# nbip/IWAE

Hardware: AMD Instinct MI355X
Metric: images/sec (train step) IWAE k=50 batch 1024 @1/2/4/8 GPU; test LLH@k=5000 (higher is better)
Workload: dtype bf16; 1 GPU; 1-layer IWAE k=50 batch 1024 per GPU (BASELINE configs[1]; N=8 is configs[4]), objective iwae_elbo, train step = forward + backward + Adam(eps=1e-4); config_id=c1, global_batch=1024, n_samples=50, parallelism=dp1, rccl_ranks=0, settle_steps=100, full=False

## Files before the change

### iwae_amd/csrc/device_helpers.h

```cpp
#pragma once
#include <hip/hip_runtime.h>
#include <stdint.h>
#include "kernels.h"
#include "layout.h"

namespace iwae {

typedef __attribute__((ext_vector_type(8))) __bf16 bf16x8_t;
typedef __attribute__((ext_vector_type(2))) __bf16 bf16x2_t;
typedef __attribute__((ext_vector_type(4))) float f32x4;

#define LOG2PI_F 1.8378770664093453f
#define HALF_LOG_2PI_F 0.9189385332046727f

__device__ __forceinline__ uint32_t pack2(float a, float b) {
    bf16x2_t v;
    v[0] = (__bf16)a;
    v[1] = (__bf16)b;
    return __builtin_bit_cast(uint32_t, v);
}
__device__ __forceinline__ float bflo(uint32_t u) { return __uint_as_float(u << 16); }
__device__ __forceinline__ float bfhi(uint32_t u) { return __uint_as_float(u & 0xffff0000u); }
__device__ __forceinline__ float bf_at(const uint4& u, int j) {
    const uint32_t w = (j < 2) ? u.x : (j < 4) ? u.y : (j < 6) ? u.z : u.w;
    return (j & 1) ? bfhi(w) : bflo(w);
}
__device__ __forceinline__ f32x4 mfma16(const uint4& a, const uint4& b, f32x4 c) {
    return __builtin_amdgcn_mfma_f32_16x16x32_bf16(__builtin_bit_cast(bf16x8_t, a), __builtin_bit_cast(bf16x8_t, b), c, 0, 0, 0);
}
__device__ __forceinline__ float rcp_fast(float x) { return __builtin_amdgcn_rcpf(x); }
#define LOG2E_F 1.4426950408889634f
#define LN2_F 0.6931471805599453f
__device__ __forceinline__ float exp2_raw(float x) { return __builtin_amdgcn_exp2f(x); }
__device__ __forceinline__ float log2_raw(float x) { return __builtin_amdgcn_logf(x); }
__device__ __forceinline__ float tanh_fast(float x) {
    return 1.0f - 2.0f * rcp_fast(exp2_raw(x * (2.0f * LOG2E_F)) + 1.0f);
}
__device__ __forceinline__ float sigmoid_fast(float l) { return rcp_fast(1.0f + exp2_raw(-l * LOG2E_F)); }
__device__ __forceinline__ float tanh_f32(float x) {
    const float t = __expf(2.0f * fabsf(x));
    return __builtin_copysignf(1.0f - 2.0f * __builtin_amdgcn_rcpf(t + 1.0f), x);
}

__device__ __forceinline__ uint32_t lds_addr_of(const char* p) {
    return (uint32_t)(uintptr_t)(const __attribute__((address_space(3))) char*)p;
}
__device__ __forceinline__ void glds16(const char* g, uint32_t lds_wave_base) {
    uint32_t keep;
    asm volatile("s_mov_b32 %0, m0\n\ts_mov_b32 m0, %2\n\ts_nop 0\n\tglobal_load_lds_dwordx4 %1, off\n\ts_mov_b32 m0, %0"
                 : "=&s"(keep) : "v"(g), "s"(lds_wave_base) : "memory");
}

template <int NWAVES>
__device__ __forceinline__ void stage_image(const char* src, char* lds, int bytes, int wave, int lane) {
    const uint32_t base = lds_addr_of(lds);
    for (int off = wave * 1024; off < bytes; off += NWAVES * 1024)
        glds16(src + off + lane * 16, (uint32_t)__builtin_amdgcn_readfirstlane((int)(base + (uint32_t)off)));
}

__device__ __forceinline__ void wait_all_vmem() {
    __builtin_amdgcn_s_waitcnt(0x0F70);
    asm volatile("s_waitcnt vmcnt(0)" ::: "memory");
}

template <int N, int P, class RD, class USE, class SIDE>
__device__ __forceinline__ void lds_pipeline(RD rd, USE use, SIDE side) {
    uint4 av[P];
#pragma unroll
    for (int i = 0; i < P; ++i)
        if (i < N) av[i] = rd(i);
#pragma unroll
    for (int i = 0; i < N; ++i) {
        use(i, av[i % P]);
        if (i + P < N) av[i % P] = rd(i + P);
        side(i);
    }
}
template <int N, int P, class RD, class USE>
__device__ __forceinline__ void lds_pipeline(RD rd, USE use) {
    lds_pipeline<N, P>(rd, use, [](int) {});
}

__device__ __forceinline__ void philox4x32_10(uint32_t c0, uint32_t c1, uint32_t c2, uint32_t c3, uint32_t k0, uint32_t k1, uint32_t out[4]) {
#pragma unroll
    for (int r = 0; r < 10; ++r) {
        unsigned long long p0, p1;
        asm("v_mad_u64_u32 %0, vcc, %1, %2, 0" : "=v"(p0) : "v"(c0), "v"(0xD2511F53u) : "vcc");
        asm("v_mad_u64_u32 %0, vcc, %1, %2, 0" : "=v"(p1) : "v"(c2), "v"(0xCD9E8D57u) : "vcc");
        const uint32_t hi0 = (uint32_t)(p0 >> 32), lo0 = (uint32_t)p0;
        const uint32_t hi1 = (uint32_t)(p1 >> 32), lo1 = (uint32_t)p1;
        const uint32_t n0 = hi1 ^ c1 ^ k0, n1 = lo1, n2 = hi0 ^ c3 ^ k1, n3 = lo0;
        c0 = n0; c1 = n1; c2 = n2; c3 = n3;
        k0 += 0x9E3779B9u; k1 += 0xBB67AE85u;
    }
    out[0] = c0; out[1] = c1; out[2] = c2; out[3] = c3;
}
__device__ __forceinline__ void philox4x32_10_mul(uint32_t c0, uint32_t c1, uint32_t c2, uint32_t c3, uint32_t k0, uint32_t k1, uint32_t out[4]) {
#pragma unroll
    for (int r = 0; r < 10; ++r) {
        const unsigned long long p0 = (unsigned long long)c0 * 0xD2511F53ull, p1 = (unsigned long long)c2 * 0xCD9E8D57ull;
        const uint32_t hi0 = (uint32_t)(p0 >> 32), lo0 = (uint32_t)p0, hi1 = (uint32_t)(p1 >> 32), lo1 = (uint32_t)p1;
        const uint32_t n0 = hi1 ^ c1 ^ k0, n2 = hi0 ^ c3 ^ k1;
        c0 = n0; c1 = lo1; c2 = n2; c3 = lo0;
        k0 += 0x9E3779B9u; k1 += 0xBB67AE85u;
    }
    out[0] = c0; out[1] = c1; out[2] = c2; out[3] = c3;
}
__device__ __forceinline__ void box_muller4(const uint32_t (&r)[4], float n[4]) {
    const float s24 = 5.9604644775390625e-08f;
    const float u0 = ((float)(r[0] >> 8) + 0.5f) * s24, u1 = ((float)(r[1] >> 8) + 0.5f) * s24;
    const float u2 = ((float)(r[2] >> 8) + 0.5f) * s24, u3 = ((float)(r[3] >> 8) + 0.5f) * s24;
    const float ra = __builtin_amdgcn_sqrtf(-2.0f * __logf(u0)), rb = __builtin_amdgcn_sqrtf(-2.0f * __logf(u2));
    n[0] = ra * __builtin_amdgcn_cosf(u1); n[1] = ra * __builtin_amdgcn_sinf(u1);
    n[2] = rb * __builtin_amdgcn_cosf(u3); n[3] = rb * __builtin_amdgcn_sinf(u3);
}
__device__ __forceinline__ void normal4(uint64_t grow, uint32_t d4, uint32_t stream, uint32_t step, uint64_t seed, float n[4]) {
    uint32_t r[4];
    philox4x32_10((uint32_t)grow, (uint32_t)(grow >> 32), (stream << 24) | d4, step, (uint32_t)seed, (uint32_t)(seed >> 32), r);
    box_muller4(r, n);
}
__device__ __forceinline__ void normal4_mul(uint64_t grow, uint32_t d4, uint32_t stream, uint32_t step, uint64_t seed, float n[4]) {
    uint32_t r[4];
    philox4x32_10_mul((uint32_t)grow, (uint32_t)(grow >> 32), (stream << 24) | d4, step, (uint32_t)seed, (uint32_t)(seed >> 32), r);
    box_muller4(r, n);
}

__device__ __forceinline__ float rowsum16(float v) {
    v += __shfl_xor(v, 1); v += __shfl_xor(v, 2); v += __shfl_xor(v, 4); v += __shfl_xor(v, 8);
    return v;
}
__device__ __forceinline__ double rowsum16(double v) {
    v += __shfl_xor(v, 1); v += __shfl_xor(v, 2); v += __shfl_xor(v, 4); v += __shfl_xor(v, 8);
    return v;
}
__device__ __forceinline__ double tree_sum_256(double v, double* sh) {
    sh[threadIdx.x] = v;
    __syncthreads();
#pragma unroll
    for (int w = 256 / 2; w > 0; w >>= 1) {
        if ((int)threadIdx.x < w) sh[threadIdx.x] += sh[threadIdx.x + w];
        __syncthreads();
    }
    const double r = sh[0];
    __syncthreads();
    return r;
}

constexpr int WG_GEMM_THREADS = 256;

__device__ __forceinline__ void wg_gemm_f32(const float* strip, int pa, int nkb, const float* W, int ldw, int cnt, float* slab,
                                            f32x4 (&acc)[AIS_NT], int tid, int n16, int q) {
    const int gpr = 4 * cnt;
    int goff[4], soff[4];
    bool ok[4];
    float4 pre[4];
#pragma unroll
    for (int u = 0; u < 4; ++u) {
        const int g = tid + WG_GEMM_THREADS * u, r = g / gpr, cq = g - r * gpr;
        ok[u] = r < 16;
        goff[u] = r * ldw + 4 * cq;
        soff[u] = r * AIS_SLABP + 4 * cq;
        pre[u] = make_float4(0.f, 0.f, 0.f, 0.f);
        if (ok[u]) pre[u] = *(const float4*)(W + goff[u]);
    }
    for (int kb = 0; kb < nkb; ++kb) {
        __syncthreads();
#pragma unroll
        for (int u = 0; u < 4; ++u)
            if (ok[u]) *(float4*)(slab + soff[u]) = pre[u];
        __syncthreads();
        if (kb + 1 < nkb) {
#pragma unroll
            for (int u = 0; u < 4; ++u)
                if (ok[u]) pre[u] = *(const float4*)(W + (size_t)(kb + 1) * 16 * ldw + goff[u]);
        }
        const float4 av = *(const float4*)(strip + n16 * pa + 16 * kb + 4 * q);
        const float a4[4] = {av.x, av.y, av.z, av.w};
        const float* sl = slab + 4 * q * AIS_SLABP + n16;
#pragma unroll
        for (int j = 0; j < 4; ++j)
#pragma unroll
            for (int t = 0; t < AIS_NT; ++t)
                if (t < cnt) acc[t] = __builtin_amdgcn_mfma_f32_16x16x4f32(a4[j], sl[j * AIS_SLABP + 16 * t], acc[t], 0, 0, 0);
    }
}

template <class Args>
__device__ __forceinline__ void dec_row_tanh_layers(const Args& a, const float* zs, float* g1s, float* g2s, float* slab, int PZ, int PH, int dt, int ht,
                                                    f32x4 (&acc)[AIS_NT], int tid, int n16, int q) {
#pragma unroll
    for (int t = 0; t < AIS_NT; ++t) acc[t] = (f32x4){0.f, 0.f, 0.f, 0.f};
    wg_gemm_f32(zs, PZ, dt, a.W1, a.Hp, ht, slab, acc, tid, n16, q);
#pragma unroll
    for (int t = 0; t < AIS_NT; ++t) {
        if (t < ht) {
            const float b = a.b1[16 * t + n16];
#pragma unroll
            for (int r = 0; r < 4; ++r) g1s[(4 * q + r) * PH + 16 * t + n16] = tanh_f32(acc[t][r] + b);
            acc[t] = (f32x4){0.f, 0.f, 0.f, 0.f};
        }
    }
    wg_gemm_f32(g1s, PH, ht, a.W2, a.Hp, ht, slab, acc, tid, n16, q);
#pragma unroll
    for (int t = 0; t < AIS_NT; ++t) {
        if (t < ht) {
            const float b = a.b2[16 * t + n16];
#pragma unroll
            for (int r = 0; r < 4; ++r) g2s[(4 * q + r) * PH + 16 * t + n16] = tanh_f32(acc[t][r] + b);
        }
    }
}

template <class Args>
__device__ __forceinline__ void dec_row_eval(const Args& a, float* zs, float* g1s, float* g2s, float* slab, int PZ, int PH, int dt, int ht, int xt,
                                             int npass, const float* const (&xrow)[4], f32x4 (&acc)[AIS_NT], float (&lp)[4], int tid, int n16, int q) {
    f32x4 dg2[AIS_NT];
    dec_row_tanh_layers(a, zs, g1s, g2s, slab, PZ, PH, dt, ht, acc, tid, n16, q);
#pragma unroll
    for (int t = 0; t < AIS_NT; ++t) dg2[t] = (f32x4){0.f, 0.f, 0.f, 0.f};
    for (int pass = 0; pass < npass; ++pass) {
        const int c0 = 16 * AIS_TPO * pass, cnt = min(AIS_TPO, xt - AIS_TPO * pass);
#pragma unroll
        for (int t = 0; t < AIS_TPO; ++t) acc[t] = (f32x4){0.f, 0.f, 0.f, 0.f};
        wg_gemm_f32(g2s, PH, ht, a.W3 + c0, a.Xp, cnt, slab, acc, tid, n16, q);
        float s_xl[4] = {0.f, 0.f, 0.f, 0.f}, s_al[4] = {0.f, 0.f, 0.f, 0.f}, prod[4] = {1.f, 1.f, 1.f, 1.f};
#pragma unroll
        for (int t = 0; t < AIS_TPO; ++t) {
            if (t < cnt) {
                const int col = c0 + 16 * t + n16;
                const bool in = col < a.X;
                const float b = a.b3[col];
#pragma unroll
                for (int r = 0; r < 4; ++r) {
// ... 44 lines not shown
```

### iwae_amd/csrc/fp32_kernels.hip

```cpp
#include <hip/hip_runtime.h>
#include <stdint.h>
#include <type_traits>
#include <algorithm>
#include "kernels.h"
#include "device_helpers.h"

namespace iwae {

__device__ __forceinline__ float4 scale_b_quad(const GemmF32Args& a, float4 t, int gk, bool b_nfast) {
    if (b_nfast) { const float w = a.brow_scale[gk]; return make_float4(t.x * w, t.y * w, t.z * w, t.w * w); }
    return make_float4(t.x * a.brow_scale[gk], t.y * a.brow_scale[gk + 1], t.z * a.brow_scale[gk + 2], t.w * a.brow_scale[gk + 3]);
}

template <int KB>
__global__ __launch_bounds__(256) void gemm_f32_kernel(GemmF32Args a) {
    constexpr int BK = 16 * KB;
    __shared__ float sA[64][BK + 1];
    __shared__ float sB[BK][80];
    const int tid = threadIdx.x, lane = tid & 63, wave = tid >> 6;
    const int m0 = blockIdx.y * 64, n0 = blockIdx.x * 64;
    const int k_beg = blockIdx.z * a.kchunk, k_end = min(a.K, k_beg + a.kchunk);
    const int wm = wave >> 1, wn = wave & 1;
    const int r16 = lane & 15, q = lane >> 4;
    f32x4 acc[2][2];
// ... 148 lines not shown
        const float* p = a.B + (size_t)gk * a.sbk + (size_t)gn * a.sbn;
        const int lim = b_nfast ? a.N - gn : k_end - gk;
        const bool outer_ok = b_nfast ? gk < k_end : gn < a.N;
        if (outer_ok && lim >= 4 && a.bvec) { float4 t = *(const float4*)p; if (a.brow_scale) t = scale_b_quad(a, t, gk, b_nfast); return t; }
        if (outer_ok) {
#pragma unroll
            for (int e = 0; e < 4; ++e) if (e < lim) v[e] = p[e * (b_nfast ? a.sbn : a.sbk)] * (a.brow_scale ? a.brow_scale[b_nfast ? gk : gk + e] : 1.0f);
        }
        return make_float4(v[0], v[1], v[2], v[3]);
    };
    auto stash = [&](int buf, const float4 (&ra)[NA], const float4 (&rb)[NB]) {
#pragma unroll
        for (int u = 0; u < NA; ++u) {
            int lm, lk;
            if (!a_pos(u, lm, lk)) continue;
            const float av4[4] = {ra[u].x, ra[u].y, ra[u].z, ra[u].w};
#pragma unroll
            for (int e = 0; e < 4; ++e) { if (a_kfast) sA[buf][lm][lk + e] = av4[e]; else sA[buf][lm + e][lk] = av4[e]; }
        }
#pragma unroll
        for (int u = 0; u < NB; ++u) {
            int ln, lk;
            if (!b_pos(u, ln, lk)) continue;
            const float bv4[4] = {rb[u].x, rb[u].y, rb[u].z, rb[u].w};
#pragma unroll
            for (int e = 0; e < 4; ++e) { if (b_nfast) sB[buf][lk][ln + e] = bv4[e]; else sB[buf][lk + e][ln] = bv4[e]; }
        }
    };
    float4 ra[NA], rb[NB];
#pragma unroll
    for (int u = 0; u < NA; ++u) ra[u] = make_float4(0.f, 0.f, 0.f, 0.f);
#pragma unroll
    for (int u = 0; u < NB; ++u) rb[u] = make_float4(0.f, 0.f, 0.f, 0.f);
    if (k_beg < k_end) {
#pragma unroll
        for (int u = 0; u < NA; ++u) ra[u] = fetch_a(k_beg, u);
#pragma unroll
        for (int u = 0; u < NB; ++u) rb[u] = fetch_b(k_beg, u);
    }
    stash(0, ra, rb);
    __syncthreads();
    int buf = 0;
    for (int k0 = k_beg; k0 < k_end; k0 += 16) {
        const bool more = k0 + 16 < k_end;
        if (more) {
#pragma unroll
            for (int u = 0; u < NA; ++u) ra[u] = fetch_a(k0 + 16, u);
#pragma unroll
            for (int u = 0; u < NB; ++u) rb[u] = fetch_b(k0 + 16, u);
        }
#pragma unroll
        for (int kk = 0; kk < 4; ++kk) {
            float av[TM], bv[TN];
#pragma unroll
            for (int i = 0; i < TM; ++i) av[i] = sA[buf][16 * TM * wm + 16 * i + r16][4 * kk + q];
#pragma unroll
            for (int j = 0; j < TN; ++j) bv[j] = sB[buf][4 * kk + q][16 * TN * wn + 16 * j + r16];
#pragma unroll
            for (int i = 0; i < TM; ++i)
#pragma unroll
                for (int j = 0; j < TN; ++j) acc[i][j] = __builtin_amdgcn_mfma_f32_16x16x4f32(av[i], bv[j], acc[i][j], 0, 0, 0);
        }
        if (more) stash(buf ^ 1, ra, rb);
        __syncthreads();
        buf ^= 1;
    }
    if constexpr (TM == 4 && TN == 4) {
    if (a.epi == GEMM_EPI_BERN) {
        float bias4[4];
        bool nok[4];
#pragma unroll
        for (int j = 0; j < 4; ++j) {
            const int n = n0 + 64 * wn + 16 * j + r16;
            nok[j] = n < a.N;
            bias4[j] = (nok[j] && a.bias) ? a.bias[n] : 0.0f;
        }
#pragma unroll
        for (int i = 0; i < 4; ++i)
#pragma unroll
            for (int r = 0; r < 4; ++r) {
                const int m = m0 + 64 * wm + 16 * i + 4 * q + r;
                const int mc = min(m, a.M - 1);
                const float* xr = a.XB + (size_t)(mc / a.bern_k) * a.bern_X;
                float sum = 0.0f;
#pragma unroll
                for (int j = 0; j < 4; ++j) {
                    if (nok[j]) {
                        const float l = acc[i][j][r] + bias4[j];
                        const float xv = xr[n0 + 64 * wn + 16 * j + r16];
                        const float e = __expf(-fabsf(l)), ope = 1.0f + e;
                        sum += xv * l - (fmaxf(l, 0.0f) + __logf(ope));
                        if (a.C && m < a.M) a.C[(size_t)m * a.ldc + n0 + 64 * wn + 16 * j + r16] = xv - (l >= 0.0f ? 1.0f : e) * __builtin_amdgcn_rcpf(ope);
                    }
                }
                sum += __shfl_xor(sum, 1); sum += __shfl_xor(sum, 2); sum += __shfl_xor(sum, 4); sum += __shfl_xor(sum, 8);
                if (r16 == 0 && m < a.M) a.part[(size_t)(2 * blockIdx.x + wn) * a.part_stride + m] = sum;
            }
        return;
    }
    }
    float* C = a.C + (size_t)blockIdx.z * a.slab_stride;
#pragma unroll
    for (int i = 0; i < TM; ++i)
#pragma unroll
        for (int j = 0; j < TN; ++j) {
            const int n = n0 + 16 * TN * wn + 16 * j + r16;
            if (n >= a.N) continue;
            const float bias = a.bias ? a.bias[n] : 0.0f;
#pragma unroll
            for (int r = 0; r < 4; ++r) {
                const int m = m0 + 16 * TM * wm + 16 * i + 4 * q + r;
                if (m >= a.M) {
                    if (a.Cones && m == a.M) a.Cones[(size_t)blockIdx.z * a.cones_stride + n] = acc[i][j][r];
                    continue;
                }
                float v = acc[i][j][r] + bias;
                if (a.orow_scale) v *= a.orow_scale[m];
                if (a.epi == GEMM_EPI_TANH) v = tanh_f32(v);
                else if (a.epi == GEMM_EPI_EXP) v = expf(v) + 1e-6f;
                else if (a.epi == GEMM_EPI_DTANH) { const float y = a.ACT[(size_t)m * a.ldact + n]; v *= 1.0f - y * y; }
                float* dst = C + (size_t)m * a.ldc + n;
                *dst = a.accumulate ? *dst + v : v;
            }
        }
}

#ifdef IWAE_DENSE_STAMPS
#define GS_STAMP(slot)                                                                 \
    {                                                                                  \
        unsigned long long t_;                                                         \
        __builtin_amdgcn_sched_barrier(0);                                             \
        asm volatile("s_memtime %0\n\ts_waitcnt lgkmcnt(0)" : "=s"(t_)::"memory");     \
        __builtin_amdgcn_sched_barrier(0);                                             \
        gs_sum[slot] += t_ - gs_prev;                                                  \
        gs_prev = t_;                                                                  \
    }
#else
#define GS_STAMP(slot)
#endif
__device__ __forceinline__ int gemm_swz16(int row) { return (0x78 >> (2 * ((row >> 2) & 3))) & 3; }
__device__ __forceinline__ float4 gemm_f32_slow_quad(const float* base, long s_e, long s_k, int e, int k, int Ext, int k_end, bool kfast, bool ones) {
    float v[4];
#pragma unroll
    for (int t = 0; t < 4; ++t) {
        const int ee = kfast ? e : e + t, kk = kfast ? k + t : k;
        float x = 0.0f;
        if (kk < k_end) {
            if (ee < Ext) x = base[(size_t)ee * s_e + (size_t)kk * s_k];
            else if (ones && ee == Ext) x = 1.0f;
        }
        v[t] = x;
    }
    return make_float4(v[0], v[1], v[2], v[3]);
}
__device__ __forceinline__ void quad_transpose(float (&x)[4], int lane) {
    const int p = lane & 3;
    float t[4];
#pragma unroll
    for (int r = 0; r < 4; ++r) {
        const float o = __builtin_bit_cast(float, __builtin_amdgcn_mov_dpp(__builtin_bit_cast(int, x[r ^ 1]), 0xB1, 0xF, 0xF, true));
        t[r] = ((r ^ p) & 1) ? o : x[r];
    }
#pragma unroll
    for (int r = 0; r < 4; ++r) {
        const float o = __builtin_bit_cast(float, __builtin_amdgcn_mov_dpp(__builtin_bit_cast(int, t[r ^ 2]), 0x4E, 0xF, 0xF, true));
        x[r] = ((r ^ p) & 2) ? o : t[r];
    }
}
template <int TM, int TN, int WGM, int WGN, bool AK, bool BNF, int OCC = 4>
__global__ __launch_bounds__(64 * WGM * WGN, OCC) void gemm_f32_v2_kernel(GemmF32Args a) {
    constexpr int NT = 64 * WGM * WGN;
    [[maybe_unused]] constexpr int NW = WGM * WGN;
    constexpr int BM = 16 * TM * WGM, BN = 16 * TN * WGN;
    constexpr int PA = AK ? 16 : BM + 4, PB = BNF ? BN + 4 : 16;
    constexpr int SA = AK ? BM * 16 : 16 * PA, SB = BNF ? 16 * PB : BN * 16;
    constexpr int QM = BM / 4, QN = BN / 4;
    constexpr bool HOLD_A = TM <= TN;
    __shared__ __attribute__((aligned(16))) float sA[2][SA];
    __shared__ __attribute__((aligned(16))) float sB[2][SB];
    const int tid = threadIdx.x, lane = tid & 63, wave = tid >> 6;
#ifdef IWAE_DENSE_STAMPS
    unsigned long long gs_sum[8] = {0, 0, 0, 0, 0, 0, 0, 0}, gs_prev = 0;
    asm volatile("s_memtime %0\n\ts_waitcnt lgkmcnt(0)" : "=s"(gs_prev)::"memory");
#endif
    int bx = blockIdx.x, by = blockIdx.y, bz = blockIdx.z;
    {
        const int nb = gridDim.x * gridDim.y * gridDim.z;
        if (gridDim.z > 1 && (nb & 7) == 0) {
            const int L = bx + gridDim.x * (by + gridDim.y * bz), V = (L & 7) * (nb >> 3) + (L >> 3);
            bx = V % gridDim.x; by = (V / gridDim.x) % gridDim.y; bz = V / (gridDim.x * gridDim.y);
        }
    }
    const int m0 = by * BM, n0 = bx * BN;
    const int k_beg = bz * a.kchunk, k_end = min(a.K, k_beg + a.kchunk);
    const int wm = wave / WGN, wn = wave % WGN;
    const int r16 = lane & 15, q = lane >> 4;
    f32x4 acc[TM][TN];
#pragma unroll
    for (int i = 0; i < TM; ++i)
#pragma unroll
        for (int j = 0; j < TN; ++j) acc[i][j] = (f32x4){0.f, 0.f, 0.f, 0.f};
    constexpr int TPRA = QM > 32 ? 64 : QM > 16 ? 32 : 16, TPRB = QN > 32 ? 64 : QN > 16 ? 32 : 16;
    constexpr int RQ = NT / 4, KRA = NT / TPRA, KRB = NT / TPRB;
    constexpr int NA = AK ? (BM + RQ - 1) / RQ : (16 + KRA - 1) / KRA, NB = BNF ? (16 + KRB - 1) / KRB : (BN + RQ - 1) / RQ;
    const bool ones = a.Cones != nullptr;
    const int eA0 = AK ? tid >> 2 : 4 * (tid % TPRA), kA0 = AK ? 4 * (tid & 3) : tid / TPRA;
    const int eB0 = BNF ? 4 * (tid % TPRB) : tid >> 2, kB0 = BNF ? tid / TPRB : 4 * (tid & 3);
    constexpr int dEA = AK ? RQ : 0, dKA = AK ? 0 : KRA, dEB = BNF ? 0 : RQ, dKB = BNF ? KRB : 0;
    const int oA0 = AK ? eA0 * 16 + (((tid & 3) ^ gemm_swz16(eA0)) << 2) : kA0 * PA + eA0;
    const int oB0 = BNF ? kB0 * PB + eB0 : eB0 * 16 + (((tid & 3) ^ gemm_swz16(eB0)) << 2);
    constexpr int dOA = AK ? RQ * 16 : dKA * PA, dOB = BNF ? dKB * PB : RQ * 16;
    const float* pA = a.A + (size_t)(m0 + eA0) * a.sam + (size_t)(k_beg + kA0) * a.sak;
    const float* pB = a.B + (size_t)(n0 + eB0) * a.sbn + (size_t)(k_beg + kB0) * a.sbk;
    const long dPA = AK ? RQ * a.sam : (long)dKA * a.sak, dPB = BNF ? (long)dKB * a.sbk : RQ * a.sbn;
    unsigned stA = 0, stB = 0;
#pragma unroll
    for (int u = 0; u < NA; ++u) {
        const int le = eA0 + dEA * u, ge = m0 + le;
        const bool exists = AK ? le < BM : le < BM && kA0 + dKA * u < 16;
        const bool inside = AK ? ge < a.M : ge + 3 < a.M, outside = ge >= a.M + (ones ? 1 : 0);
        stA |= (unsigned)(!exists ? 3 : (inside && a.avec) ? 1 : outside ? 0 : 2) << (2 * u);
    }
#pragma unroll
    for (int u = 0; u < NB; ++u) {
        const int le = eB0 + dEB * u, ge = n0 + le;
        const bool exists = BNF ? le < BN && kB0 + dKB * u < 16 : le < BN;
        const bool inside = BNF ? ge + 3 < a.N : ge < a.N, outside = ge >= a.N;
        stB |= (unsigned)(!exists ? 3 : (inside && a.bvec) ? 1 : outside ? 0 : 2) << (2 * u);
    }
    const long stepA = 16 * a.sak, stepB = 16 * a.sbk;
    float4 ra[NA], rb[NB], rw[NB];
    auto fetch = [&](int k0, bool full) {
#pragma unroll
        for (int u = 0; u < NA; ++u) {
            const unsigned st = (stA >> (2 * u)) & 3u;
            float4 t = make_float4(0.f, 0.f, 0.f, 0.f);
            if (st == 1 && full) t = *(const float4*)(pA + u * dPA);
            else if (st == 2 || (st == 1 && !full)) t = gemm_f32_slow_quad(a.A, a.sam, a.sak, m0 + eA0 + dEA * u, k0 + kA0 + dKA * u, a.M, k_end, AK, ones);
            ra[u] = t;
        }
        pA += stepA;
#pragma unroll
        for (int u = 0; u < NB; ++u) {
            const unsigned st = (stB >> (2 * u)) & 3u;
            float4 t = make_float4(0.f, 0.f, 0.f, 0.f);
            if (st == 1 && full) t = *(const float4*)(pB + u * dPB);
            else if (st == 2 || (st == 1 && !full)) t = gemm_f32_slow_quad(a.B, a.sbn, a.sbk, n0 + eB0 + dEB * u, k0 + kB0 + dKB * u, a.N, k_end, !BNF, false);
            rb[u] = t;
            if (a.brow_scale && st != 3) {
                const int gk = k0 + kB0 + dKB * u;
                if (BNF) { const float w = gk < k_end ? a.brow_scale[gk] : 0.0f; rw[u] = make_float4(w, w, w, w); }
                else rw[u] = make_float4(gk < k_end ? a.brow_scale[gk] : 0.0f, gk + 1 < k_end ? a.brow_scale[gk + 1] : 0.0f,
                                         gk + 2 < k_end ? a.brow_scale[gk + 2] : 0.0f, gk + 3 < k_end ? a.brow_scale[gk + 3] : 0.0f);
            }
        }
        pB += stepB;
    };
    auto stash = [&](int buf) {
#pragma unroll
        for (int u = 0; u < NA; ++u) if (((stA >> (2 * u)) & 3u) != 3u) *(float4*)&sA[buf][oA0 + dOA * u] = ra[u];
#pragma unroll
        for (int u = 0; u < NB; ++u)
            if (((stB >> (2 * u)) & 3u) != 3u) {
                float4 t = rb[u];
                if (a.brow_scale) { t.x *= rw[u].x; t.y *= rw[u].y; t.z *= rw[u].z; t.w *= rw[u].w; }
                *(float4*)&sB[buf][oB0 + dOB * u] = t;
            }
    };
    const int arow = 16 * TM * wm + r16, brow = 16 * TN * wn + r16;
    const int afr = AK ? arow * 16 + ((q ^ gemm_swz16(r16)) << 2) : 4 * q * PA + arow;
    const int bfr = BNF ? 4 * q * PB + brow : brow * 16 + ((q ^ gemm_swz16(r16)) << 2);
    auto frag_a = [&](const float* As, int t, float (&v)[4]) {
        if (AK) { const float4 x = *(const float4*)(As + afr + 256 * t); v[0] = x.x; v[1] = x.y; v[2] = x.z; v[3] = x.w; }
        else {
#pragma unroll
            for (int j = 0; j < 4; ++j) v[j] = As[afr + 16 * t + j * PA];
        }
    };
    auto frag_b = [&](const float* Bs, int t, float (&v)[4]) {
        if (BNF) {
#pragma unroll
            for (int j = 0; j < 4; ++j) v[j] = Bs[bfr + 16 * t + j * PB];
        } else { const float4 x = *(const float4*)(Bs + bfr + 256 * t); v[0] = x.x; v[1] = x.y; v[2] = x.z; v[3] = x.w; }
    };
    auto compute = [&](int buf) {
        const float *As = sA[buf], *Bs = sB[buf];
        if constexpr (HOLD_A) {
            float ah[TM][4];
#pragma unroll
            for (int i = 0; i < TM; ++i) frag_a(As, i, ah[i]);
            constexpr int NG = (TN + 1) / 2;
            float cur[2][4], nxt[2][4];
            frag_b(Bs, 0, cur[0]);
            if (TN > 1) frag_b(Bs, 1, cur[1]);
#pragma unroll
            for (int g = 0; g < NG; ++g) {
                if (g + 1 < NG) { frag_b(Bs, 2 * g + 2, nxt[0]); if (2 * g + 3 < TN) frag_b(Bs, 2 * g + 3, nxt[1]); }
#pragma unroll
                for (int j = 0; j < 4; ++j)
#pragma unroll
                    for (int h = 0; h < 2; ++h)
                        if (2 * g + h < TN) {
#pragma unroll
                            for (int i = 0; i < TM; ++i) acc[i][2 * g + h] = __builtin_amdgcn_mfma_f32_16x16x4f32(ah[i][j], cur[h][j], acc[i][2 * g + h], 0, 0, 0);
                        }
#pragma unroll
                for (int h = 0; h < 2; ++h)
#pragma unroll
                    for (int j = 0; j < 4; ++j) cur[h][j] = nxt[h][j];
            }
        } else {
            float bh[TN][4];
#pragma unroll
            for (int j = 0; j < TN; ++j) frag_b(Bs, j, bh[j]);
            constexpr int NG = (TM + 1) / 2;
            float cur[2][4], nxt[2][4];
            frag_a(As, 0, cur[0]);
            if (TM > 1) frag_a(As, 1, cur[1]);
#pragma unroll
            for (int g = 0; g < NG; ++g) {
// ... 652 lines not shown
```

### iwae_amd/csrc/kernels.h

```cpp
#pragma once
#include <hip/hip_runtime.h>
#include <stdint.h>

namespace iwae {

#define IWAE_DENSE_G1_DEFAULT 29u
enum { EPI_TANH = 0, EPI_HEAD = 1, EPI_DX = 2, EPI_F32 = 3, EPI_BERN = 4, EPI_SIGMOID = 5 };
enum { OBJ_VAE_ELBO = 0, OBJ_IWAE_ELBO = 1, OBJ_IWAE_EQ14 = 2, OBJ_VAE_ELBO_KL = 3, OBJ_DREG = 4 };
enum { PB_LME = 0, PB_MEAN, PB_EQ14, PB_KL, PB_PX, PB_T1, PB_T2, PB_DREG, PB_COUNT };
enum { SC_VAE_ELBO = 0, SC_VAE_ELBO_KL, SC_IWAE_ELBO, SC_IWAE_EQ14, SC_INFERENCE_LOSS, SC_MEAN_LPXZ, SC_MEAN_T1, SC_MEAN_T2, SC_KL, SC_COUNT = 16 };


struct EpsSrc {
    const float* user = nullptr;
    const float* cache = nullptr;
    int ldC = 0;
    int B = 0;
    uint64_t seed = 0;
    uint64_t row_offset = 0;
    uint32_t step = 0;
    uint32_t stream = 0;
    int k_total = 0, s_off = 0, kc = 0;
};

// ... 82 lines not shown
    const float* Xf; int Xdim; uint16_t* XPout;
    const char *img0, *img1, *img2;
    int KT0, KT1;
    int NT1, NT2;
    int R;
    uint16_t *H1, *H2; int ldH;
    float* YF; int ldYF; int split;
    int sample; SampleArgs S;
    const char* oimg; int oXdim, oH;
    const uint16_t* oXB; int oldXB; int ok;
    uint16_t* oSP; int oldS; float* olpxz;
};
bool block_fwd_ok(const BlockFwdArgs& a);
bool block_fwd_shape_ok(const BlockFwdArgs& a);
void launch_block_fwd(const BlockFwdArgs& a, hipStream_t st);

struct Chain2FwdArgs {
    uint16_t* Z1P;
    float* lqz1x;
    const char *e_img1, *e_img2, *e_imgh;
    const char *d_img1, *d_img2, *d_imgh;
    int M, k, B, D0, D1;
    uint16_t *EH1, *EH2;
    float* EHEAD;
    uint16_t* Z2P;
    uint16_t *DH1, *DH2;
    float* DHEAD;
    const float* head1; int ldH1;
    EpsSrc eps1, eps2;
    float *lpz1z2, *lpz2, *lqz2z1;
};
bool chain2_fwd_ok(int KT0, int KTH, int KT1, int M);
void launch_chain2_fwd(const Chain2FwdArgs& a, hipStream_t st);

struct DecBwdRowsArgs {
    const uint16_t* SP; int ldS; int KTX;
    const char* imgK3; int MT3;
    const char *imgB2, *imgB1;
    int KT, NT1, NT3;
    int M;
    const uint16_t *G2, *G1; int ldH;
    const float* gx;
    uint16_t *D2P, *D1P;
    float* DZ; uint16_t* DZH; int ldDZ;
    int lse_on;
    LseArgs lse;
};
bool dec_bwd_rows_ok(const DecBwdRowsArgs& a);
void launch_dec_bwd_rows(const DecBwdRowsArgs& a, hipStream_t st, hipEvent_t done = nullptr);

struct LatentBwdArgs {
    const float* dz; int ldDZ;
    const uint16_t* dzh;
    const float* dz2; const float* dz3;
    const float* head; int ldH; int D, Dp;
    const float4* cf;
    EpsSrc eps;
    int B, Bp, k;
    float kmu, ksig;
    uint16_t* DHP;
    float* DHF;
    const float* prior_head;
    uint16_t* DHP2;
    float* DHF2;
};
void launch_latent_bwd(const LatentBwdArgs& a, hipStream_t st);
struct BlockBwdArgs {
    const uint16_t* DH; int ldDH;
    const char *imgH, *imgL2;
    int KTH, KT1, NT1;
    int R;
    const uint16_t *H2, *H1; int ldH;
    uint16_t *D2, *D1;
    int lat_on;
    LatentBwdArgs lat;
    int rows_per_wg;
};
bool block_bwd_ok(const BlockBwdArgs& a);
void launch_block_bwd(const BlockBwdArgs& a, hipStream_t st);

struct OutBwdArgs {
    const uint16_t* G2; int ldG;
    const char* img1;
    const char* img2;
    int Xdim; int Xp32;
    const float* gx;
    const uint16_t* XB; int ldXB; int k;
    int M, KT, NG;
    uint16_t* DLP;
    const uint16_t* SP;
    float* part; int gpb;
    uint16_t* DPP;
    unsigned long long* stamps;
    int dbg;
};
void launch_out_bwd(const OutBwdArgs& a, hipStream_t st, hipEvent_t done = nullptr);

struct DecBwdArgs {
    OutBwdArgs o;
    const char* imgB2;
    const uint16_t* G1;
    uint16_t* D1P;
    const char* imgB1; int MG1;
    float* DZ; int ldDZ;
    uint16_t* DZH;
    int nw;
};
bool out_bwd_has_s_mode(int KT);
void launch_dec_bwd(const DecBwdArgs& d, hipStream_t st, hipEvent_t done = nullptr);

struct GBlockBwdArgs {
    const char* imgH;
    const char *imgBh, *imgB2, *imgB1;
    const uint16_t *H2, *H1;
    const float* gx;
    int M, k, B, D;
    EpsSrc eps;
    const float* head1; int ldH1;
    const float* DZIN;
    uint16_t* DHP;
    uint16_t *D2P, *D1P;
    float* DZ2;
    uint16_t* DZD;
    const float* DZDEC;
    int ldDZDEC;
    uint16_t* DZOUT;
};
bool gblock_bwd_ok(int KT0, int KTH, int KT1, int M);
void launch_gblock_bwd(int mode, const GBlockBwdArgs& a, hipStream_t st, hipEvent_t done = nullptr);

struct GaussBwdArgs {
    int mode;
    const float* G;
    const float* head; int ldH; int D, Dp;
    const float* zhead; int ldZH; int Dzp;
    const float* dz_in; float* dz_direct; int ldDZ;
    EpsSrc eps;
    int M, Mp, k;
    uint16_t* DHP;
    float* DHF;
};
void launch_gauss_bwd(const GaussBwdArgs& a, hipStream_t st);

struct WgradPArgs {
    const uint16_t* X; int ldX; int IT;
    const uint16_t* G; int ldG; int JT;
    int M, rows_per_split;
    float* slabW;
    float* slabB;
    const char* zero;
    const float* rowscale;
    int dbg;
    unsigned long long* stamps;
};
void launch_wgradp(const WgradPArgs& a, int nsplit, int shape, hipStream_t st, hipEvent_t done = nullptr);
int wgradp_strip(int shape);
struct WgradPGroup {
    WgradPArgs a[3];
    int n;
    int gx[3], gy[3];
    int zbeg[4];
};
void launch_wgradp_group(const WgradPGroup& g, hipStream_t st);
void launch_wgradws_group(const WgradPGroup& g, hipStream_t st);

struct LayerDesc {
    int Kin, Nout, joff;
    size_t offW, offb;
    char* imgF; int KT_F;
    char* imgB; int KT_B; int MT_B; int imgB_kmajor;
    const float* slabW; const float* slabB; int nsplit; int slab_ld; size_t slab_stride;
    size_t slabB_stride;
    int block_begin;
    int rblock_begin;
};
void launch_reduce_grads(const LayerDesc* layers, int nlayers, int first_block, int nblocks, float* grad, float* param, float* mom, float* vel,
                         float alpha, float beta1, float beta2, float eps, int fuse_adam, const float* per_b, int B, float beta, float* scalars, hipStream_t st,
                         int first_block2 = 0, int nblocks2 = 0, hipEvent_t done = nullptr);
void launch_scalars(const float* per_b, int B, float beta, float* out, hipStream_t st);
void launch_adam(const LayerDesc* layers, int nlayers, int nblocks, float* param, const float* grad, float* mom, float* vel,
                 float alpha, float gscale, float beta1, float beta2, float eps, int do_update, hipStream_t st, int first_block = 0, hipEvent_t done = nullptr);

#define WGR_MAX_JOBS 6
struct WgradRowsJob {
    const uint16_t* X; int ldX;
    const uint16_t* G; int ldG;
    int R;
    const float* rowscale;
    int sub0, sub1, split;
    int ib, jb, wg_begin;
};
void launch_wgrad_rows(const WgradRowsJob* jobs, int njobs, const LayerDesc* layers, float* grad, float* param, float* mom, float* vel, float alpha,
                       float beta1, float beta2, float eps, int fuse_adam, const float* per_b, int B, float beta, float* scalars, const char* zero, hipStream_t st);

enum { GEMM_EPI_NONE = 0, GEMM_EPI_TANH = 1, GEMM_EPI_EXP = 2, GEMM_EPI_DTANH = 3, GEMM_EPI_BERN = 4 };
struct GemmF32Args {
    const float* A; long sam, sak;
    const float* B; long sbk, sbn;
    float* C; long ldc;
    int M, N, K;
    const float* bias;
    int epi;
    const float* ACT; long ldact;
    int accumulate;
    int kchunk; size_t slab_stride;
    int avec, bvec;
    int cvec;
    const float* XB; int bern_k, bern_X;
    float* part; size_t part_stride;
    const float* brow_scale;
    const float* orow_scale;
    float* Cones; size_t cones_stride;
    unsigned long long* stamps;
    int tile_mode;
    int dbg;
};
struct DecFwdF32Args {
    const float* Z; int ldz; int Din;
    int M, H, X;
    const float *W1, *b1, *W2, *b2, *W3, *b3;
    float *G1, *G2; int ldg;
    float* S; int ldS;
    const float* XB; int k;
    float* lpxz;
    const char* zero;
    unsigned long long* stamps;
};
bool dec_fwd_f32_ok(const DecFwdF32Args& a);
void launch_dec_fwd_f32(const DecFwdF32Args& a, hipStream_t st);
struct GemmF32Opts {
    bool v2 = true;
    bool w8 = true;
    bool v2_small = true;
    bool ksplit = true;
    int ksplit_min_tiles = 1;
    int v2_small_min = 1;
    int dbg = 0;
};
long gemm_f32_tiles(const GemmF32Opts& o, int M, int N, int tile_mode = 0);
bool gemm_f32_takes_big(int M, int N, int nsplit);
void launch_gemm_f32(const GemmF32Opts& o, const GemmF32Args& a, int nsplit, hipStream_t st);
int gemm_f32_fewrows_split(const GemmF32Opts& o, int M, int N, int K);
void launch_gemm_f32_fewrows(const GemmF32Opts& o, const GemmF32Args& a, float* slabs, hipStream_t st);
int gemm_f32_slots(const GemmF32Opts& o, int M, int N, int tile_mode = 0);
void launch_reduce_slabs_f32(const float* slabs, size_t stride, int nsplit, size_t n, float* out, hipStream_t st);
#define REDUCE_SLABS_MAX_JOBS 40
struct ReduceSlabsJob { const float* slabs; size_t stride; size_t n; float* out; int nsplit; int block_begin; };
struct ReduceSlabsJobs { ReduceSlabsJob job[REDUCE_SLABS_MAX_JOBS]; int n; };
void launch_reduce_slabs_multi_f32(ReduceSlabsJobs& jobs, hipStream_t st);
void launch_bern_f32(const float* logits, size_t ld, const float* x, int X, int M, int k, float* lpxz, hipStream_t st);
void launch_dl_f32(float* logits, size_t ld, const float* x, int X, int M, int k, const float* gx, hipStream_t st);
void launch_sigmoid_f32(float* v, size_t n, hipStream_t st);
void launch_export_mat(const float* in, int B, int k, int X, float* out, hipStream_t st);
void launch_concat_f32(const float* a, int na, const float* b, int nb, int rows, float* out, hipStream_t st);

#define GRID_D_MAX 4
#define GRID_XP_MAX 800
#define GRID_RANGE 1024
enum { GRID_ST = 18, GRID_S1 = 2, GRID_S2 = 6, GRID_Q = 16, GRID_A = 17 };
__host__ __device__ inline int grid_tri(int d, int e) { return d * GRID_D_MAX - d * (d - 1) / 2 + (e - d); }
struct GridPrepArgs {
    const float* logits; int ldl;
    const float* z; const float* lw;
    int Gc, Gcp, X, Xp, D;
    uint16_t *Lhi, *Llo;
    float* c; float4* zc; float* w;
};
struct GridScoreArgs {
    const uint16_t* XB; int Xp;
    const uint16_t *Lhi, *Llo; const float* c; const float4* zc; const float* w;
    const float* head; int ldh, soff;
    int N, Gc, nsplit;
    float* part;
    float* log_joint; long ldlj; long lj_col;
};
struct GridMergeArgs {
    const float* part; int nsplit, N, D;
    double* run;
    int first, last;
    const float* head; int ldh;
    double* log_px; float *mean, *cov, *qmass, *kl;
};
void launch_grid_prep_x(const float* x, int N, int X, int Np, int Xp, uint16_t* XB, int* nonbinary, hipStream_t st);
void launch_grid_prep(const GridPrepArgs& a, hipStream_t st);
void launch_grid_score(const GridScoreArgs& a, int D, hipStream_t st);
void launch_grid_merge(const GridMergeArgs& a, hipStream_t st);

#define ACT_BLOCK 128
struct ActChainArgs {
    const char *img1, *img2, *imgh;
    const float* head1; int ldH1;
    EpsSrc eps1;
    int kn, D0, D1;
    float* part; int nblk;
    int img0, blk0;
};
struct ActPartialArgs {
    const float* head; int ldh;
    int nb, kn, D1;
    float* part; int nblk, img0, blk0;
};
struct ActStatsArgs {
    const float* src; long ld_img; int ld_blk, nblk;
    double kdiv;
    int N, D;
    float* post_mean; int ldpm, col;
    double *activity, *data_mean;
// ... 208 lines not shown
```

### iwae_amd/csrc/kernels.hip

```cpp
#include <hip/hip_runtime.h>
#include <hip/hip_ext.h>
#include <stdint.h>
#include <string.h>
#include <type_traits>
#include "kernels.h"
#include "layout.h"
#include "device_helpers.h"
#include "step_helpers.h"

namespace iwae {
template <bool MASKED, bool KEEP>
__device__ __forceinline__ float bern8(const f32x4& a0, const f32x4& a1, const uint4& xb, int f0, int Xdim, uint4& sp) {
    float s_xl = 0.0f, s_al = 0.0f, prod = 1.0f, sv[8];
#pragma unroll
    for (int j = 0; j < 8; ++j) {
        const float l = (j < 4) ? a0[j & 3] : a1[j & 3];
        const float xm = bf_at(xb, j) - 0.5f;
        const float ope = 1.0f + exp2_raw(-fabsf(l * LOG2E_F));
        const bool in = !MASKED || (f0 + 16 * (j >> 2) + (j & 3) < Xdim);
        prod *= in ? ope : 1.0f;
        s_al += fabsf(l);
        s_xl = fmaf(xm, l, s_xl);
        if (KEEP) {
            const float h = __builtin_copysignf(rcp_fast(ope) - 0.5f, l);
// ... 2589 lines not shown
                        dsg[i] += t * e[u][i] + cf[u].w * rsg[i];
                        dpm[i] -= cf[u].y * up * prs[i];
                        dps[i] -= cf[u].y * (up * up - 1.0f) * prs[i];
                    }
                }
            }
        }
    }
#pragma unroll
    for (int i = 0; i < 4; ++i) { red[threadIdx.x][i] = dmu[i]; red[threadIdx.x][4 + i] = dsg[i]; }
    __syncthreads();
    if (sg == 0 && act) {
        for (int g = 1; g < SG; ++g)
#pragma unroll
            for (int i = 0; i < 4; ++i) { dmu[i] += red[g * nf4 + f4][i]; dsg[i] += red[g * nf4 + f4][4 + i]; }
#pragma unroll
        for (int i = 0; i < 4; ++i) {
            if (f0 + i < a.D) {
                dmu[i] += a.kmu * mu[i];
                dsg[i] += a.ksig * (sgm[i] - 1.0f / sgm[i]);
                dsg[i] *= (sgm[i] - 1e-6f);
            } else { dmu[i] = 0.0f; dsg[i] = 0.0f; }
        }
    }
    if (sg == 0 && b < a.B) {
        if (a.DHP) {
            *(uint2*)(a.DHP + (size_t)b * (2 * a.Dp) + p_pos(f0)) = make_uint2(pack2(dmu[0], dmu[1]), pack2(dmu[2], dmu[3]));
            *(uint2*)(a.DHP + (size_t)b * (2 * a.Dp) + p_pos(a.Dp + f0)) = make_uint2(pack2(dsg[0], dsg[1]), pack2(dsg[2], dsg[3]));
        }
        if (a.DHF) {
            *(float4*)(a.DHF + (size_t)b * (2 * a.Dp) + f0) = make_float4(dmu[0], dmu[1], dmu[2], dmu[3]);
            *(float4*)(a.DHF + (size_t)b * (2 * a.Dp) + a.Dp + f0) = make_float4(dsg[0], dsg[1], dsg[2], dsg[3]);
        }
    }
    if (FAST || !a.prior_head) return;
    __syncthreads();
#pragma unroll
    for (int i = 0; i < 4; ++i) { red[threadIdx.x][i] = dpm[i]; red[threadIdx.x][4 + i] = dps[i]; }
    __syncthreads();
    if (sg != 0 || b >= a.B) return;
    if (act) {
        for (int g = 1; g < SG; ++g)
#pragma unroll
            for (int i = 0; i < 4; ++i) { dpm[i] += red[g * nf4 + f4][i]; dps[i] += red[g * nf4 + f4][4 + i]; }
#pragma unroll
        for (int i = 0; i < 4; ++i) {
            if (f0 + i < a.D) dps[i] *= (sigp_of(a, b, f0 + i) - 1e-6f);
            else { dpm[i] = 0.0f; dps[i] = 0.0f; }
        }
    }
    if (a.DHP2) {
        *(uint2*)(a.DHP2 + (size_t)b * (2 * a.Dp) + p_pos(f0)) = make_uint2(pack2(dpm[0], dpm[1]), pack2(dpm[2], dpm[3]));
        *(uint2*)(a.DHP2 + (size_t)b * (2 * a.Dp) + p_pos(a.Dp + f0)) = make_uint2(pack2(dps[0], dps[1]), pack2(dps[2], dps[3]));
    }
    if (a.DHF2) {
        *(float4*)(a.DHF2 + (size_t)b * (2 * a.Dp) + f0) = make_float4(dpm[0], dpm[1], dpm[2], dpm[3]);
        *(float4*)(a.DHF2 + (size_t)b * (2 * a.Dp) + a.Dp + f0) = make_float4(dps[0], dps[1], dps[2], dps[3]);
    }
}

__global__ void gauss_bwd_kernel(GaussBwdArgs a) {
    const int idx = blockIdx.x * blockDim.x + threadIdx.x;
    const int nf4 = a.Dp / 4;
    const int row = idx / nf4, f4 = idx % nf4;
    if (row >= a.Mp) return;
    const bool valid = row < a.M;
    const int f0 = 4 * f4;
    float dm[4] = {0, 0, 0, 0}, ds[4] = {0, 0, 0, 0}, dzd[4] = {0, 0, 0, 0};
    if (valid && f0 < a.D) {
        const int b = row / a.k, s = row - b * a.k;
        const float G = a.G[row];
        const float* hp = a.head + (size_t)row * a.ldH;
        float e[4];
        eps4(a.eps, b, s, row, f4, a.D, e);
        const float4 mu4 = *(const float4*)(hp + f0), sg4 = *(const float4*)(hp + a.Dp + f0);
        const float muv[4] = {mu4.x, mu4.y, mu4.z, mu4.w}, sgv[4] = {sg4.x, sg4.y, sg4.z, sg4.w};
        float4 a4 = make_float4(0.f, 0.f, 0.f, 0.f), b4 = a4;
        if (a.mode == 0) {
            const float* hz = a.zhead + (size_t)b * a.ldZH;
            a4 = *(const float4*)(hz + f0); b4 = *(const float4*)(hz + a.Dzp + f0);
        } else {
            a4 = *(const float4*)(a.dz_in + (size_t)row * a.ldDZ + f0);
        }
        const float av[4] = {a4.x, a4.y, a4.z, a4.w}, bv[4] = {b4.x, b4.y, b4.z, b4.w};
#pragma unroll
        for (int i = 0; i < 4; ++i) {
            if (f0 + i < a.D) {
                const float mu = muv[i], sg = sgv[i], rs = __builtin_amdgcn_rcpf(sg);
                if (a.mode == 0) {
                    const float z = av[i] + bv[i] * e[i];
                    const float u = (z - mu) * rs;
                    dm[i] = G * u * rs;
                    ds[i] = G * (u * u - 1.0f) * rs * (sg - 1e-6f);
                    dzd[i] = -dm[i];
                } else {
                    const float z = mu + sg * e[i];
                    const float d = av[i] - G * z;
                    dm[i] = d;
                    ds[i] = (d * e[i] + G * rs) * (sg - 1e-6f);
                }
            }
        }
    }
    if (valid) {
        if (a.DHP) {
            *(uint2*)(a.DHP + (size_t)row * (2 * a.Dp) + p_pos(f0)) = make_uint2(pack2(dm[0], dm[1]), pack2(dm[2], dm[3]));
            *(uint2*)(a.DHP + (size_t)row * (2 * a.Dp) + p_pos(a.Dp + f0)) = make_uint2(pack2(ds[0], ds[1]), pack2(ds[2], ds[3]));
        }
        if (a.DHF) {
            *(float4*)(a.DHF + (size_t)row * (2 * a.Dp) + f0) = make_float4(dm[0], dm[1], dm[2], dm[3]);
            *(float4*)(a.DHF + (size_t)row * (2 * a.Dp) + a.Dp + f0) = make_float4(ds[0], ds[1], ds[2], ds[3]);
        }
        if (a.mode == 0) *(float4*)(a.dz_direct + (size_t)row * a.ldDZ + f0) = make_float4(dzd[0], dzd[1], dzd[2], dzd[3]);
    }
}


struct AdamCoef { float alpha, gscale, beta1, beta2, eps; int on; };

__device__ __forceinline__ void adam_math(float& w, float& m, float& v, float g, const AdamCoef& c) {
    g *= c.gscale;
    m = __builtin_fmaf(c.beta1, m, (1.0f - c.beta1) * g);
    v = __builtin_fmaf(c.beta2, v, ((1.0f - c.beta2) * g) * g);
    const float q = (c.alpha * m) / (sqrtf(v) + c.eps);
    w = w - q;
}
__device__ __forceinline__ void image_refresh(const LayerDesc& L, bool is_bias, int i, int j, float w) {
    if (is_bias) {
        *(float*)(L.imgF + img_mg_bias_byte(L.joff + j, L.KT_F)) = w;
    } else {
        const uint16_t h = (uint16_t)(pack2(w, 0.0f) & 0xffffu);
        *(uint16_t*)(L.imgF + img_mg_byte(L.joff + j, i, L.KT_F)) = h;
        if (L.imgB) {
            if (L.imgB_kmajor) *(uint16_t*)(L.imgB + img_k_byte(i, L.joff + j, L.MT_B)) = h;
            else *(uint16_t*)(L.imgB + img_mg_byte(i, L.joff + j, L.KT_B)) = h;
        }
    }
}
__device__ __forceinline__ void adam_element(const LayerDesc& L, bool is_bias, int i, int j, size_t idx, float g, bool update,
                                             float* param, float* mom, float* vel, const AdamCoef& c) {
    float w = param[idx];
    if (update) {
        float m = mom[idx], v = vel[idx];
        adam_math(w, m, v, g, c);
        mom[idx] = m;
        vel[idx] = v;
        param[idx] = w;
    }
    image_refresh(L, is_bias, i, j, w);
}

struct MeansArgs { const float* per_b; int B; float beta; float* out; };

__global__ __launch_bounds__(256) void reduce_grads_kernel(const LayerDesc* layers, int nlayers, float* grad, float* param, float* mom,
                                                           float* vel, AdamCoef c, MeansArgs mn, int first_block, int n1, int first_block2) {
    if (mn.per_b && blockIdx.x == gridDim.x - 1) {
        batch_means_block(mn.per_b, mn.B, mn.beta, mn.out);
        return;
    }
    const int bid = (int)blockIdx.x < n1 ? (int)blockIdx.x + first_block : (int)blockIdx.x - n1 + first_block2;
    __shared__ float4 red[4][64];
    int l = 0;
    while (l + 1 < nlayers && bid >= layers[l + 1].rblock_begin) ++l;
    const LayerDesc L = layers[l];
    const int n4 = (L.Nout + 3) >> 2;
    const int g = (bid - L.rblock_begin) * 64 + (threadIdx.x & 63);
    const int sg = threadIdx.x >> 6;
    const int ngroups = (L.Kin + 1) * n4;
    float4 s = make_float4(0.f, 0.f, 0.f, 0.f);
    int i = 0, j = 0;
    const bool ok = g < ngroups;
    if (ok) {
        i = g / n4;
        j = (g - i * n4) * 4;
        const bool is_b = i == L.Kin;
        const float* p = is_b ? (L.slabB + L.joff + j) : (L.slabW + (size_t)i * L.slab_ld + L.joff + j);
        const size_t stride = is_b ? (L.slabB_stride ? L.slabB_stride : (size_t)L.slab_ld) : L.slab_stride;
        if (L.nsplit <= 16) {
#pragma unroll 4
            for (int sp = sg; sp < L.nsplit; sp += 4) {
                const float4 v = *(const float4*)(p + (size_t)sp * stride);
                s.x += v.x; s.y += v.y; s.z += v.z; s.w += v.w;
            }
        } else
        for (int sp0 = sg; sp0 < L.nsplit; sp0 += 32) {
            float4 v[8];
#pragma unroll
            for (int u = 0; u < 8; ++u) {
                const int sp = sp0 + 4 * u;
                v[u] = *(const float4*)(p + (size_t)(sp < L.nsplit ? sp : sg) * stride);
            }
#pragma unroll
            for (int u = 0; u < 8; ++u)
                if (sp0 + 4 * u < L.nsplit) { s.x += v[u].x; s.y += v[u].y; s.z += v[u].z; s.w += v[u].w; }
        }
    }
    red[sg][threadIdx.x & 63] = s;
    __syncthreads();
    if (sg == 0 && ok) {
        const int t = threadIdx.x;
        float r[4] = {red[0][t].x + red[1][t].x + red[2][t].x + red[3][t].x, red[0][t].y + red[1][t].y + red[2][t].y + red[3][t].y,
                      red[0][t].z + red[1][t].z + red[2][t].z + red[3][t].z, red[0][t].w + red[1][t].w + red[2][t].w + red[3][t].w};
        float* dst = (i == L.Kin) ? (grad + L.offb + j) : (grad + L.offW + (size_t)i * L.Nout + j);
#pragma unroll
        for (int e = 0; e < 4; ++e) {
            if (j + e < L.Nout) {
                dst[e] = r[e];
                if (c.on) adam_element(L, i == L.Kin, i, j + e, (size_t)(dst - grad) + e, r[e], true, param, mom, vel, c);
            }
        }
    }
}

__global__ void adam_kernel(const LayerDesc* layers, int nlayers, float* param, const float* grad, float* mom, float* vel, AdamCoef c, int first_block) {
    const int bid = (int)blockIdx.x + first_block;
    int l = 0;
    while (l + 1 < nlayers && bid >= layers[l + 1].block_begin) ++l;
    const LayerDesc L = layers[l];
    const int e = (bid - L.block_begin) * blockDim.x + threadIdx.x;
    const int nW = L.Kin * L.Nout;
    if (e >= nW + L.Nout) return;
    const bool is_b = e >= nW;
    const size_t idx = is_b ? (L.offb + (e - nW)) : (L.offW + e);
    adam_element(L, is_b, is_b ? 0 : e / L.Nout, is_b ? e - nW : e % L.Nout, idx, c.on ? grad[idx] : 0.0f, c.on != 0, param, mom, vel, c);
}
struct WgradRowsArgs {
    WgradRowsJob job[WGR_MAX_JOBS];
    int njobs;
    const LayerDesc* layers;
    float *grad, *param, *mom, *vel;
    AdamCoef c;
    MeansArgs mn;
    const char* zero;
};
#define WGR_NST 4
#define WGR_STAGE 8192
__global__ __launch_bounds__(256, 1) void wgrad_rows_kernel(WgradRowsArgs a) {
    extern __shared__ __attribute__((aligned(1024))) char smem[];
    typedef __attribute__((ext_vector_type(4))) short v4s;
    if (a.mn.per_b && blockIdx.x == gridDim.x - 1) {
        batch_means_block(a.mn.per_b, a.mn.B, a.mn.beta, a.mn.out);
        return;
    }
    int jn = 0;
#pragma unroll
    for (int t = 1; t < WGR_MAX_JOBS; ++t)
        if (t < a.njobs && (int)blockIdx.x >= a.job[t].wg_begin) jn = t;
    const WgradRowsJob J = a.job[jn];
    const int wl = (int)blockIdx.x - J.wg_begin;
    const int bi = wl / J.jb, bj = wl - bi * J.jb;
    const int tid = threadIdx.x, lane = tid & 63, wave = __builtin_amdgcn_readfirstlane(tid >> 6);
    const int q = lane >> 4, l16 = lane & 15, qp = l16 >> 2, p = l16 & 3;
    const int RW = ((J.R + 3) / 4 + 31) & ~31;
    const int rbeg = wave * RW, rend = min(J.R, rbeg + RW);
    const int nstage = rend > rbeg ? (rend - rbeg + 31) / 32 : 0;
    char* ring = smem + wave * (WGR_NST * WGR_STAGE);
    auto swz = [](int r) { return ((r >> 1) & 1) << 2; };
    const int prl = lane >> 3, psl = lane & 7;
    const char* zsrc = a.zero + lane * 16;
    const char* xsrc[4]; const char* gsrc[4]; int xlim[4], glim[4];
#pragma unroll
    for (int pc = 0; pc < 4; ++pc) {
        const int rl = 8 * pc + prl;
        const int cx = bi * 64 + ((psl ^ swz(rl)) * 8), cg = bj * 64 + ((psl ^ swz(rl)) * 8);
        xsrc[pc] = (const char*)J.X + ((size_t)(rbeg + rl) * J.ldX + cx) * 2;
        gsrc[pc] = (const char*)J.G + ((size_t)(rbeg + rl) * J.ldG + cg) * 2;
        xlim[pc] = cx < J.ldX ? rend - rbeg - rl : -(1 << 30);
        glim[pc] = cg < J.ldG ? rend - rbeg - rl : -(1 << 30);
    }
    const size_t xstride = (size_t)32 * J.ldX * 2, gstride = (size_t)32 * J.ldG * 2;
    auto issue = [&](int c) {
        const uint32_t base = lds_addr_of(ring + (c % WGR_NST) * WGR_STAGE);
#pragma unroll
        for (int pc = 0; pc < 4; ++pc)
            glds16(32 * c < xlim[pc] ? xsrc[pc] + (size_t)c * xstride : zsrc, (uint32_t)__builtin_amdgcn_readfirstlane((int)(base + (uint32_t)pc * 1024u)));
#pragma unroll
        for (int pc = 0; pc < 4; ++pc)
            glds16(32 * c < glim[pc] ? gsrc[pc] + (size_t)c * gstride : zsrc, (uint32_t)__builtin_amdgcn_readfirstlane((int)(base + 4096u + (uint32_t)pc * 1024u)));
    };
    f32x4 acc[4][4], accb[4];
#pragma unroll
    for (int u = 0; u < 4; ++u) {
        accb[u] = (f32x4){0.0f, 0.0f, 0.0f, 0.0f};
#pragma unroll
        for (int t = 0; t < 4; ++t) acc[t][u] = (f32x4){0.0f, 0.0f, 0.0f, 0.0f};
    }
    const uint4 ones = make_uint4(0x3F803F80u, 0x3F803F80u, 0x3F803F80u, 0x3F803F80u);
    const bool do_bias = bi == 0;
    for (int c = 0; c < min(nstage, WGR_NST - 1); ++c) issue(c);
    const int row_off = (4 * q + qp) * 128;
    for (int c = 0; c < nstage; ++c) {
        wait_vmem_but_ws(8 * min(WGR_NST - 2, nstage - 1 - c));
        if (c + WGR_NST - 1 < nstage) issue(c + WGR_NST - 1);
        const char* xb = ring + (c % WGR_NST) * WGR_STAGE + row_off;
        const char* gb = xb + 4096;
        auto frag = [&](const char* base, int t) {
            const char* p0 = base + ((((4 * (t >> 1)) ^ swz(qp)) + p) * 16) + 8 * (t & 1);
            const v4s r0 = __builtin_amdgcn_ds_read_tr16_b64_v4i16((__attribute__((address_space(3))) v4s*)p0);
            const v4s r1 = __builtin_amdgcn_ds_read_tr16_b64_v4i16((__attribute__((address_space(3))) v4s*)(p0 + 16 * 128));
            const uint2 lo = __builtin_bit_cast(uint2, r0), hi = __builtin_bit_cast(uint2, r1);
            return make_uint4(lo.x, lo.y, hi.x, hi.y);
        };
        uint4 g[4];
#pragma unroll
        for (int u = 0; u < 4; ++u) g[u] = frag(gb, u);
        if (J.rowscale) {
            const float* rs = J.rowscale + rbeg + 32 * c + 4 * q;
            const float4 s0 = *(const float4*)rs, s1 = *(const float4*)(rs + 16);
#pragma unroll
            for (int u = 0; u < 4; ++u)
                g[u] = make_uint4(pack2(bflo(g[u].x) * s0.x, bfhi(g[u].x) * s0.y), pack2(bflo(g[u].y) * s0.z, bfhi(g[u].y) * s0.w),
                                  pack2(bflo(g[u].z) * s1.x, bfhi(g[u].z) * s1.y), pack2(bflo(g[u].w) * s1.z, bfhi(g[u].w) * s1.w));
        }
#pragma unroll
        for (int t = 0; t < 4; ++t) {
            const uint4 av = frag(xb, t);
#pragma unroll
            for (int u = 0; u < 4; ++u) acc[t][u] = mfma16(av, g[u], acc[t][u]);
        }
        if (do_bias) {
#pragma unroll
            for (int u = 0; u < 4; ++u) accb[u] = mfma16(ones, g[u], accb[u]);
        }
    }
    asm volatile("s_waitcnt vmcnt(0)" ::: "memory");
#pragma unroll
    for (int t = 0; t < 4; ++t)
#pragma unroll
        for (int u = 0; u < 4; ++u) *(f32x4*)(ring + ((t * 4 + u) * 64 + lane) * 16) = acc[t][u];
    if (q == 0) {
#pragma unroll
        for (int u = 0; u < 4; ++u) *(float*)(ring + 16384 + (u * 16 + l16) * 4) = accb[u][0];
    }
    __syncthreads();
    const int jg = bj * 64;
    const LayerDesc L0 = a.layers[J.sub0];
    const LayerDesc L1 = a.layers[J.sub1 >= 0 ? J.sub1 : J.sub0];
    const int s2 = wave >> 1, u0 = 2 * (wave & 1);
    float gsum[16], pw[16], pm[16], pv[16];
    size_t eidx[16];
    bool eok[16];
    char* tileB = smem + 20480;
    constexpr int TB_PITCH = 144;
#pragma unroll
    for (int uu = 0; uu < 2; ++uu) {
        const int u = u0 + uu;
        const bool second = J.sub1 >= 0 && jg + 16 * u >= J.split;
        const int joff = second ? L1.joff : L0.joff, Nout = second ? L1.Nout : L0.Nout, Kin = second ? L1.Kin : L0.Kin;
        const size_t offW = second ? L1.offW : L0.offW;
        const int jj = jg + 16 * u + l16 - joff;
#pragma unroll
        for (int tt = 0; tt < 2; ++tt) {
            const int n = (2 * s2 + tt) * 4 + u;
            f32x4 v = *(const f32x4*)(smem + (n * 64 + lane) * 16);
#pragma unroll
            for (int w = 1; w < 4; ++w) {
// ... 98 lines not shown
    if (a.M < 8192 || !((a.g1_mask >> epi) & 1u)) return false;
    if (a.KT == 7 && epi == EPI_TANH) {
        LAUNCH_EV(done, (dense_kernel<EPI_TANH, 7, 1, 16>), dim3((a.M + 255) / 256, grid.y), dim3(1024), lds, st, a);
        return true;
    }
    if (a.KT == 7) {
        switch (epi) {
            case EPI_DX: LAUNCH_EV(done, (dense_kernel<EPI_DX, 7, 1>), grid, dim3(512), lds, st, a); return true;
            case EPI_F32: LAUNCH_EV(done, (dense_kernel<EPI_F32, 7, 1>), grid, dim3(512), lds, st, a); return true;
            case EPI_BERN: LAUNCH_EV(done, (dense_kernel<EPI_BERN, 7, 1>), grid, dim3(512), lds, st, a); return true;
            default: return false;
        }
    }
    if (a.KT == 4 && epi == EPI_TANH) { LAUNCH_EV(done, (dense_kernel<EPI_TANH, 4, 1>), grid, dim3(512), lds, st, a); return true; }
    return false;
}
bool block_fwd_ok(const BlockFwdArgs& a) {
    if (a.sample && !a.S.ZP) return false;
    if (a.oimg && (!a.oXB || !a.olpxz)) return false;
    return block_fwd_shape_ok(a);
}
bool block_fwd_shape_ok(const BlockFwdArgs& a) {
    if (a.sample && (a.S.Dp != 32 * a.KT0 || a.KT0 > 15 || a.S.ZF || a.S.M != a.R)) return false;
    if (a.oimg && (a.NT2 != 0 || a.oH < 1 || a.ok < 1)) return false;
    return a.R <= 4096 && a.KT1 <= BLOCKFWD_MAX_KT && a.NT1 <= 16 && a.NT2 <= 16 && a.NT1 == 2 * a.KT1 &&
           (size_t)(a.KT0 + 2 * a.KT1) * 1024 <= 150 * 1024;
}
bool dec_bwd_rows_ok(const DecBwdRowsArgs& a) {
    return a.KT <= BLOCKFWD_MAX_KT && a.NT1 <= 16 && a.NT1 == 2 * a.KT && a.NT3 <= 16 && (size_t)(a.KTX + 2 * a.KT) * 1024 <= 150 * 1024;
}
void launch_dec_bwd_rows(const DecBwdRowsArgs& a, hipStream_t st, hipEvent_t done) {
    const size_t lds = (size_t)(a.KTX + 2 * a.KT) * 1024 + 64;
    if (a.M <= 512 && a.KTX > 8) LAUNCH_EV(done, (dec_bwd_rows_kernel<13>), dim3((a.M + 15) / 16), dim3(1024), lds, st, a);
    else LAUNCH_EV(done, (dec_bwd_rows_kernel<6>), dim3((a.M + 15) / 16), dim3(1024), lds, st, a);
}
bool block_bwd_ok(const BlockBwdArgs& a) {
    return a.R <= 4096 && a.KTH <= BLOCKFWD_MAX_KT && a.KT1 <= BLOCKFWD_MAX_KT && a.NT1 <= 16 && a.NT1 == 2 * a.KT1;
}
void launch_block_bwd(const BlockBwdArgs& a, hipStream_t st) {
    if (a.rows_per_wg == 4) hipLaunchKernelGGL(block_bwd_kernel<4>, dim3((a.R + 3) / 4), dim3(1024), (size_t)(a.KTH + a.KT1) * 1024 + 16384, st, a);
    else hipLaunchKernelGGL(block_bwd_kernel<16>, dim3((a.R + 15) / 16), dim3(1024), (size_t)(a.KTH + a.KT1) * 1024, st, a);
}
void launch_block_fwd(const BlockFwdArgs& a, hipStream_t st) {
    const size_t lds = (size_t)(a.KT0 + 2 * a.KT1) * 1024 + (a.sample ? (size_t)a.KT0 * 768 : 0);
    if (a.oimg) { hipLaunchKernelGGL((block_fwd_kernel<6, true>), dim3((a.R + 15) / 16), dim3(1024), lds, st, a); return; }
    if (a.R <= 512 && a.KT0 > 8) hipLaunchKernelGGL((block_fwd_kernel<13>), dim3((a.R + 15) / 16), dim3(1024), lds, st, a);
    else hipLaunchKernelGGL((block_fwd_kernel<6>), dim3((a.R + 15) / 16), dim3(1024), lds, st, a);
}
bool bern_pipe_ok(const DenseArgs& a) {
    if (a.pre_img1 && (a.pre_KT1 < 1 || a.pre_KT1 > 4)) return false;
    return a.KT == 7 && a.M >= 8192 && a.mg_per_block >= a.MG && !a.logits_out && a.lpxz_stride == 0 &&
           (126 + a.k) / a.k + 1 <= BERN_XIMG_MAX && (a.Np32 >> 5) >= 2 && (a.Np32 >> 5) <= 2 * a.MG &&
           2 * (7 * 4096 + 1024) + (size_t)BERN_XIMG_MAX * a.ldXB * 4 + 128 <= 80 * 1024;
}
bool bern_lse_ok(const DenseArgs& a) {
    return bern_pipe_ok(a) && a.pre_img1 && a.pipe >= 2 && (198 + a.k) / a.k + 1 <= 8 && a.k >= 13 && 200 % a.k == 0 &&
           (!a.zhead || (a.lse.term[1] == a.zlp && a.lse.term[2] == a.zlq && (!a.lse.lq_dreg || a.lse.lq_dreg == a.zlq_dreg))) && a.lse.n_px_part <= 1;
}
void launch_dense(int epi, const DenseArgs& a, hipStream_t st, hipEvent_t done) {
    dim3 grid((a.M + 127) / 128, (a.MG + a.mg_per_block - 1) / a.mg_per_block);
    const size_t lds = 2 * DENSE_UNIT;
    if (epi == EPI_BERN && a.pipe && bern_pipe_ok(a)) {
        const size_t ldsb = 2 * (7 * 4096 + 1024) + (size_t)BERN_XIMG_MAX * a.ldXB * 4 + 128;
        if (a.pre_img1 && a.pipe >= 2 && (198 + a.k) / a.k + 1 <= 8) {
            const size_t ldsq = 2 * (7 * 4096 + 1024) + (size_t)8 * a.ldXB * 4 + 128 + 4096 + 2 * 7 * 1024 + 4096 + 1024
                                + (a.zhead ? (size_t)8 * 3 * a.zDp * 4 + 256 : 0);
            if (a.YP) LAUNCH_EV(done, (bern_pipe_kernel<7, true, true, true>), dim3((a.M + 199) / 200), dim3(1024), ldsq, st, a);
            else LAUNCH_EV(done, (bern_pipe_kernel<7, false, true, true>), dim3((a.M + 199) / 200), dim3(1024), ldsq, st, a);
        } else if (a.pre_img1) {
            if (a.YP) LAUNCH_EV(done, (bern_pipe_kernel<7, true, true>), dim3(grid.x), dim3(512), ldsb, st, a);
            else LAUNCH_EV(done, (bern_pipe_kernel<7, false, true>), dim3(grid.x), dim3(512), ldsb, st, a);
        } else if (a.YP) LAUNCH_EV(done, (bern_pipe_kernel<7, true, false>), dim3(grid.x), dim3(512), ldsb, st, a);
        else LAUNCH_EV(done, (bern_pipe_kernel<7, false, false>), dim3(grid.x), dim3(512), ldsb, st, a);
        return;
    }
    if (launch_dense_g1(epi, a, grid, lds, st, done)) return;
    switch (a.KT) {
        case 2: launch_dense_k<2>(epi, a, grid, lds, st, done); break;
        case 4: launch_dense_k<4>(epi, a, grid, lds, st, done); break;
        case 7: launch_dense_k<7>(epi, a, grid, lds, st, done); break;
        case 8: launch_dense_k<8>(epi, a, grid, lds, st, done); break;
        default: launch_dense_k<0>(epi, a, grid, a.stage_all ? 4 * DENSE_UNIT : lds, st, done); break;
    }
}
bool chain2_fwd_ok(int KT0, int KTH, int KT1, int M) { return KT0 == 4 && KTH == 4 && KT1 == 2 && M >= 8192; }
void launch_chain2_fwd(const Chain2FwdArgs& a, hipStream_t st) {
    hipLaunchKernelGGL((chain2_fwd_kernel<4, 4, 2>), dim3((a.M + 127) / 128), dim3(512), 2 * (4 * 4096 + 1024), st, a);
}
bool gblock_bwd_ok(int KT0, int KTH, int KT1, int M) { return KT0 == 4 && KTH == 4 && KT1 == 2 && M >= 8192; }
void launch_gblock_bwd(int mode, const GBlockBwdArgs& a, hipStream_t st, hipEvent_t done) {
    dim3 grid((a.M + 127) / 128);
    if (mode == 0) LAUNCH_EV(done, (gblock_bwd_kernel<0, 2, 4, 4>), grid, dim3(512), 2 * (8 * 4096 + 1024), st, a);
    else LAUNCH_EV(done, (gblock_bwd_kernel<1, 4, 4, 2>), grid, dim3(512), 2 * (4 * 4096 + 1024), st, a);
}
bool out_bwd_has_s_mode(int KT) { return KT == 7 || KT == 4 || KT == 2; }
void launch_dec_bwd(const DecBwdArgs& d, hipStream_t st, hipEvent_t done) {
    const size_t lds = 2 * ((size_t)d.o.KT * 4096 + 1024);
    dim3 grid((d.o.M + 127) / 128);
    if (d.nw == 8 && d.o.KT == 7) { LAUNCH_EV(done, (dec_bwd_kernel<7, 8, 1>), grid, dim3(512), lds, st, d); return; }
    switch (d.o.KT) {
        case 7: LAUNCH_EV(done, dec_bwd_kernel<7>, grid, dim3(256), lds, st, d); break;
        case 4: LAUNCH_EV(done, dec_bwd_kernel<4>, grid, dim3(256), lds, st, d); break;
        case 2: LAUNCH_EV(done, dec_bwd_kernel<2>, grid, dim3(256), lds, st, d); break;
        default: break;
    }
}
void launch_out_bwd(const OutBwdArgs& a, hipStream_t st, hipEvent_t done) {
    if (a.SP) {
        const size_t lds = 2 * ((size_t)a.KT * 4096 + 1024);
        const int nparts = a.part ? (a.NG + a.gpb - 1) / a.gpb : 1;
        dim3 grid((a.M + 127) / 128, nparts);
        const hipEvent_t done_s = a.part ? nullptr : done;
        switch (a.KT) {
            case 7: LAUNCH_EV(done_s, out_bwd_s_kernel<7>, grid, dim3(256), lds, st, a); break;
            case 4: LAUNCH_EV(done_s, out_bwd_s_kernel<4>, grid, dim3(256), lds, st, a); break;
            case 2: LAUNCH_EV(done_s, out_bwd_s_kernel<2>, grid, dim3(256), lds, st, a); break;
            default: return;
        }
        if (a.part) {
            LAUNCH_EV(done, out_bwd_finish_kernel, grid1((size_t)a.M * (a.ldG / 8), 256), dim3(256), 0, st, a, nparts);
        }
        return;
    }
    constexpr int PAIRS = 2;
    const size_t ldsp = 2 * ((size_t)a.KT * 4096 + 1024) + (size_t)PAIRS * 4096;
    dim3 gridp((a.M + PAIRS * 32 - 1) / (PAIRS * 32));
#ifdef IWAE_DIAG
    if (a.stamps) {
        LAUNCH_EV(done, (out_bwd_pair_kernel<7, PAIRS, true>), gridp, dim3(PAIRS * 128), 2 * ((size_t)7 * 4096 + 1024) + (size_t)PAIRS * 4096, st, a);
        return;
    }
#endif
    switch (a.KT) {
        case 7: LAUNCH_EV(done, (out_bwd_pair_kernel<7, PAIRS, false>), gridp, dim3(PAIRS * 128), ldsp, st, a); break;
        case 4: LAUNCH_EV(done, (out_bwd_pair_kernel<4, PAIRS, false>), gridp, dim3(PAIRS * 128), ldsp, st, a); break;
        case 2: LAUNCH_EV(done, (out_bwd_pair_kernel<2, PAIRS, false>), gridp, dim3(PAIRS * 128), ldsp, st, a); break;
        default: {
            const size_t lds = 2 * ((size_t)a.KT * 8192 + 1024);
            LAUNCH_EV(done, (out_bwd_kernel<0, false>), dim3((a.M + 127) / 128), dim3(256), lds, st, a);
        }
    }
}
void launch_latent_bwd(const LatentBwdArgs& a, hipStream_t st) {
    if (a.dzh && !a.dz2 && a.eps.cache && !a.prior_head) hipLaunchKernelGGL(latent_bwd_kernel<1>, dim3(a.Bp), dim3(256), 0, st, a);
    else if (!a.dzh && a.dz && a.dz2 && a.dz3 && a.eps.cache && !a.prior_head) hipLaunchKernelGGL(latent_bwd_kernel<2>, dim3(a.Bp), dim3(256), 0, st, a);
    else hipLaunchKernelGGL(latent_bwd_kernel<0>, dim3(a.Bp), dim3(256), 0, st, a);
}
void launch_gauss_bwd(const GaussBwdArgs& a, hipStream_t st) {
    hipLaunchKernelGGL(gauss_bwd_kernel, grid1((size_t)a.Mp * (a.Dp / 4), 256), dim3(256), 0, st, a);
}
void launch_reduce_grads(const LayerDesc* layers, int nlayers, int first_block, int nblocks, float* grad, float* param, float* mom, float* vel,
                         float alpha, float beta1, float beta2, float eps, int fuse_adam, const float* per_b, int B, float beta, float* scalars, hipStream_t st,
                         int first_block2, int nblocks2, hipEvent_t done) {
    const AdamCoef c = {alpha, 1.0f, beta1, beta2, eps, fuse_adam};
    const MeansArgs mn = {per_b, B, beta, scalars};
    LAUNCH_EV(done, reduce_grads_kernel, dim3(nblocks + nblocks2 + (per_b ? 1 : 0)), dim3(256), 0, st, layers, nlayers, grad, param, mom, vel, c, mn, first_block, nblocks,
              first_block2);
}
void launch_scalars(const float* per_b, int B, float beta, float* out, hipStream_t st) {
    hipLaunchKernelGGL(scalars_kernel, dim3(1), dim3(256), 0, st, per_b, B, beta, out);
}
void launch_adam(const LayerDesc* layers, int nlayers, int nblocks, float* param, const float* grad, float* mom, float* vel,
                 float alpha, float gscale, float beta1, float beta2, float eps, int do_update, hipStream_t st, int first_block, hipEvent_t done) {
    const AdamCoef c = {alpha, gscale, beta1, beta2, eps, do_update};
    LAUNCH_EV(done, adam_kernel, dim3(nblocks), dim3(256), 0, st, layers, nlayers, param, grad, mom, vel, c, first_block);
}
void launch_wgrad_rows(const WgradRowsJob* jobs, int njobs, const LayerDesc* layers, float* grad, float* param, float* mom, float* vel, float alpha,
                       float beta1, float beta2, float eps, int fuse_adam, const float* per_b, int B, float beta, float* scalars, const char* zero, hipStream_t st) {
    WgradRowsArgs a;
    memset(&a, 0, sizeof(a));
    int wgs = 0;
    for (int i = 0; i < njobs && i < WGR_MAX_JOBS; ++i) {
        a.job[i] = jobs[i];
        a.job[i].ib = (jobs[i].ldX + 63) / 64;
        a.job[i].jb = (jobs[i].ldG + 63) / 64;
        a.job[i].wg_begin = wgs;
        wgs += a.job[i].ib * a.job[i].jb;
    }
    a.njobs = njobs;
    a.layers = layers; a.grad = grad; a.param = param; a.mom = mom; a.vel = vel;
    a.c = AdamCoef{alpha, 1.0f, beta1, beta2, eps, fuse_adam};
    a.mn = MeansArgs{per_b, B, beta, scalars};
    a.zero = zero;
    hipLaunchKernelGGL(wgrad_rows_kernel, dim3(wgs + (per_b ? 1 : 0)), dim3(256), (size_t)4 * WGR_NST * WGR_STAGE, st, a);
}

}
```

### iwae_amd/csrc/model.h

```cpp
#pragma once
#include <hip/hip_runtime.h>
#include <stddef.h>
#include <stdint.h>
#include <string>
#include <type_traits>
#include <vector>
#include <rccl/rccl.h>
#include "../../include/iwae_amd.h"
#include "kernels.h"

#pragma GCC visibility push(hidden)

int fail(int code, const std::string& msg);
#define HIPCHK(expr)                                                                                   \
    do {                                                                                               \
        hipError_t e_ = (expr);                                                                        \
        if (e_ != hipSuccess)                                                                          \
            return fail(e_ == hipErrorOutOfMemory ? IWAE_ERR_NOMEM : IWAE_ERR_HIP,                     \
                        std::string(#expr) + ": " + hipGetErrorString(e_));                            \
    } while (0)
#define CHK(expr) do { int rc_ = (expr); if (rc_ != IWAE_OK) return rc_; } while (0)

struct DevBuf { void* p = nullptr; size_t cap = 0; };
struct KerasLayer { std::string name; int Kin, Nout; size_t offW, offb; };

struct Linear {
    int Kin = 0, Nspace = 0;
    int Kp32 = 0, Np32 = 0, KT = 0, MG = 0;
    int nsub = 0, sub[2] = {0, 0}, joff[2] = {0, 0};
    char* imgF = nullptr; size_t imgF_bytes = 0;
    char* imgB = nullptr; size_t imgB_bytes = 0; int KT_B = 0, MG_B = 0, MT_B = 0, kmajor = 0;
    DevBuf slabW, slabB;
    int IT = 0, JT = 0, nsplit = 1;
};

struct BlockWs { DevBuf h1P, h2P, head, dheadP, d2P, d1P, dx; };
struct MlpWs {
    DevBuf g1P, g2P, dlP, d2P, d1P, dz;
    DevBuf g2wP;
};

void free_buf(DevBuf& b);
template <class Ws> void free_all(Ws& ws) {
    static_assert(std::is_standard_layout<Ws>::value && std::is_trivially_destructible<Ws>::value && sizeof(Ws) % sizeof(DevBuf) == 0, "a workspace struct holds DevBufs only");
    DevBuf* b = reinterpret_cast<DevBuf*>(&ws);
    for (size_t i = 0; i < sizeof(Ws) / sizeof(DevBuf); ++i) free_buf(b[i]);
}

enum TimedKernel { T_OUT_BWD = 0, T_DEC_FWD, T_WGRAD_OUT, T_DX_HID, T_DX_LAT, T_WGRAD_HID, T_WGRAD_LAT, T_LATENT_BWD, T_ENC_FWD, T_REDUCE, T_DEC_BWD, T_AR_ENC, T_AR_DEC, T_AIS_CHAIN, T_LOCAL_Q, T_IMPUTE, T_POSTERIOR, T_COUNT };

struct FwdCall {
    uint32_t batch_offset = 0;
    int cond_row0 = 0;
    int k_total = 0, s_off = 0;
    bool log_w_only = false;
    bool no_ksplit = false;
};

struct StepOptions {
    bool allow_s_mode = true;
    bool allow_zin = true;
    bool allow_zin_eval = false;
    bool allow_eps_multi = true;
    int eps_blocks = 512;
    bool allow_block_fused = true;
    bool allow_out_in_block = true;
    bool allow_dec_fused = true;
    bool allow_bern_pipe = true;
    bool bern_qw = true;
    bool bern_qw_force = false;
    bool allow_lse_fused = true;
    bool allow_lse_dup = true;
    bool allow_lse_in_bwd = true;
    bool allow_early_wout = true;
    bool allow_g2w = false;
    bool allow_chain2 = true;
    bool allow_chain2_bwd = true;
    unsigned dense_g1_mask = IWAE_DENSE_G1_DEFAULT;
    bool allow_dec_bwd = true;
    bool small_dec_bwd = true; int small_rows = 8191;
    int dec_rows_max = 1024;
    int dec_bwd_nw = 8;
    bool allow_dz_half = true;
    bool allow_wg3 = true;
    bool allow_dec_rows = true;
    bool allow_wgrad_rows = true;
    bool allow_lat_rows4 = false;
    bool allow_lat_in_block = true;
    bool use_side2 = true;
    bool allow_wg_group = false;
    int wout_split = 0, wout_wg1 = 56, wout_wg2 = 128;
    bool defer_split = false;
    bool allow_defer = true;
    bool allow_defer2 = true;
    bool allow_defer2_split = true;
    int wg_target16 = 0;
    int wg_target16_1 = 64;
    int wg_target8 = 128;
    int wg_target8_few = 32;
    int wg_shape9 = 0;
    bool allow_wg7 = true;
    bool dp_concurrent = false;
    iwae::GemmF32Opts gemm_f32;
    bool allow_f32_multi_reduce = true;
    bool allow_f32_side = true, f32_wout_first = true;
    int f32_dw_last = 0;
    int f32_dw_min_rows = 32;
    int f32_dw_tiles = 1024;
    bool f32_dec_fused_train = false;
    bool allow_f32_dec_fused = true;
    bool allow_f32_bern_fused = true;
    int eval_rows = 0;
    int grid_chunk = 0;
    int ais_t_chunk = 0;
    int local_t_chunk = 0;
    int impute_rows = 0;
};

enum ZFrom { Z_SAMPLE = 0, Z_DENSE_ZIN, Z_DEC_PROLOGUE, Z_BLOCK, Z_CHAIN2 };
enum DecFwd { DEC_DENSE = 0, DEC_BLOCK2, DEC_BLOCK_OUT, DEC_PIPE };
enum LseAt { LSE_FWD = 0, LSE_DECODER, LSE_BWD_ROWS };
enum DxPath { DX_THREE = 0, DX_DEC_BWD, DX_ROWS };
enum OnStream { ON_MAIN = 0, ON_SIDE, ON_SIDE2 };
struct StepPlan {
    bool zin_eval = false;
    bool keep_eps = false;
    bool eps_multi = false;
    bool enc_takes_f32 = false;
    ZFrom z_from = Z_SAMPLE;
    bool chain = false;
    bool chain2_bwd = false;
    DecFwd dec_fwd = DEC_DENSE;
    iwae::DenseArgs bern;
    iwae::BlockFwdArgs dec_blk;
    int px_parts = 1;
    bool s_mode = false;
    bool early_wout = false;
    bool lse_fused = false;
    bool lse_dup = false;
    bool g2w = false;
    LseAt lse_at = LSE_FWD;
    bool want_dreg = false;
    OnStream draw_on = ON_SIDE;
    bool dec_rows = false;
    DxPath dx = DX_THREE;
    iwae::DecBwdRowsArgs rows;
    bool out_parts = false;
    bool dz_half = false;
    bool lat_fuse = false;
    bool rows_enc = false;
    bool group3 = false;
    bool wout_two_part = false;
    bool hid_group = false;
    OnStream hid_on = ON_SIDE;
    OnStream tail = ON_SIDE;
};

enum F32DecFwd { F32_DEC_GEMMS = 0, F32_DEC_ONE_LAUNCH };
enum F32PxFrom { F32_PX_BERN_PASS = 0, F32_PX_GEMM_EPILOGUE, F32_PX_DEC_KERNEL };
enum F32DwOrder {
    F32_DW_ONE_STREAM = 0,
    F32_DW_WOUT_FIRST,
    F32_DW_WOUT_LAST,
    F32_DW_BEHIND_DX
};
struct F32Plan {
    const float* x = nullptr;
    F32DecFwd dec_fwd = F32_DEC_GEMMS;
    F32PxFrom px_from = F32_PX_BERN_PASS;
    int px_parts = 1;
    bool keeps_s = false;
    bool want_dreg = false;
    bool lme_only = false;
    F32DwOrder dw_order = F32_DW_ONE_STREAM;
    int dw_tile_mode = 0;
    bool side() const { return dw_order != F32_DW_ONE_STREAM; }
};

enum StepEnd {
    END_GRAD = 0,
    END_GRAD_SPLIT,
    END_GRAD_SPLIT_HELD,
    END_UPDATE
};
struct BlockRange { int first = 0, count = 0; };
struct TableBounds {
    struct At { int r = 0, e = 0; };
    At enc1_end, enc2, dec2;
    At dec1, dec1_out, dec1_end;
    At end;
};
struct StepLeft {
    bool dec = false;
    bool dec2 = false;
    BlockRange held;
    size_t split_offset = 0;
    OnStream on = ON_SIDE;
    bool z_pending = false;
};
enum EndCase { ENDS_JOINED = 0, ENDS_DEC_ROWS, ENDS_EARLY, ENDS_EARLY_SPLIT, ENDS_EARLY_HELD, ENDS_DEFER, ENDS_SPLIT_UPD, ENDS_DEFER2, ENDS_DEFER2_SPLIT };
enum SideWait { WAIT_NONE = 0, WAIT_FORK2, WAIT_SIDE };
struct SideSum { OnStream on = ON_SIDE; BlockRange a, b; SideWait behind = WAIT_NONE; bool second_event = false; };
struct StepEndPlan {
    EndCase how = ENDS_JOINED;
    bool update = false;
    bool join_both = false;
    BlockRange main_a, main_b;
    int nside = 0;
    SideSum side[2];
    StepLeft left;
};

struct iwae_model {
    iwae_config cfg;
    int X, Xp32;
    int C = 0, Xinp = 0;
    DevBuf cond; int cond_n = 0;
    int H[2], D[2], Hp[2], Dp[2];
    hipStream_t stream = nullptr;
    bool own_stream = false;
    std::vector<KerasLayer> klayers;
    size_t nparam = 0;
    Linear enc1[3], enc2[3], dec2[3], dec1[3];
    Linear prior[3];
    bool has_prior = false;
    DevBuf condP;
    float *param = nullptr, *grad = nullptr, *mom = nullptr, *vel = nullptr;
    int64_t adam_t = 0;
    struct F32Block { DevBuf h1, h2, dhead, d2, d1, dx; };
    struct F32State { F32Block enc1, enc2, dec2, prior; DevBuf z[2], g1, g2, logits, d2, d1, slab, bpart, xcat, kslab; } f32;
    struct F32Pending { size_t off; size_t stride; size_t n; float* out; int nsplit; int seg; };
    std::vector<F32Pending> f32_pending; size_t f32_slab_used = 0;
    bool bf16_side_used = false;
    size_t f32_slab_want = 0, f32_slab_want_step = 0;
    struct EvalWs { DevBuf x, xP, head; } ev;
    DevBuf eval_lme;
    int eval_precision = IWAE_PREC_FP32;
    struct GridWs { DevBuf xb, flag, z, lw, zP, h1, h2, logits, lhi, llo, c, zc, w, part, run, lpx, mean, cov, qmass, kl, lj; } grid;
    struct ActWs { DevBuf eps, z, rows, part, pm, act, dm; BlockWs blk; F32Block f32; } act;
    struct MomWs { DevBuf mean, m2; } mom_ws;
    struct AggWs { DevBuf eps, mu, inv, invd, nls, nls_sum, zT, shT, dim_part, jmax, jsum, lqz, lqzdT, lqzd, part, out; } agg;
    struct AisWs { DevBuf wpad, betas, e, logw, h, nacc, z0, mom, unif, dH, acc, rate, z, lpx, ess; } ais;
    struct LocalWs { DevBuf st, acc, alpha, mu0, sg0, eps, qmu, qsg, mu, sg, elbo, iwae, bound, grad, logw; } loc;
    struct ImputeWs { DevBuf xin, mask, eps, logw, wstat, part, lpx, ess, xhat; } imp;
    struct PosteriorWs { DevBuf part, cdf, unif, mean, cov, idx, z, u; } post;
    bool fwd_was_f32 = false;
    ncclComm_t comm_main = nullptr, comm_side = nullptr;
    int comm_world = 1, comm_rank = 0;
    float adam_b1 = 0.9f, adam_b2 = 0.999f, adam_eps = 1e-4f;
    uint32_t noise_step = 0, batch_offset = 0;
    std::vector<iwae::LayerDesc> descs;
    iwae::LayerDesc* d_descs = nullptr;
    TableBounds tb;
    bool descs_dirty = true;
// ... 113 lines not shown
```

### iwae_amd/csrc/model.hip

```cpp
#include <math.h>
#include <stdio.h>
#include <string.h>
#include <stddef.h>
#include <stdlib.h>
#include <algorithm>
#include <random>
#include <memory>
#include <dlfcn.h>
#include "model.h"
#include "layout.h"

using namespace iwae;

static_assert(sizeof(iwae_config) == 64 && offsetof(iwae_config, struct_size) == 0 && offsetof(iwae_config, seed) == 32 && offsetof(iwae_config, cond_dim) == 48 &&
              offsetof(iwae_config, cond_prior) == 52 && offsetof(iwae_config, precision) == 56, "iwae_config layout is part of the ABI (iwae_amd/_capi.py)");
static_assert(sizeof(iwae_scalars) == 64 && sizeof(iwae_tensors) == 12 * sizeof(void*), "ABI struct layout");
static_assert(sizeof(iwae_ais_options) == 72 && offsetof(iwae_ais_options, betas) == 16 && offsetof(iwae_ais_options, step_size) == 24 && offsetof(iwae_ais_options, z0) == 40 &&
              offsetof(iwae_ais_options, unif) == 64 && sizeof(iwae_ais_outputs) == 10 * sizeof(void*), "iwae_ais_options / iwae_ais_outputs layout is part of the ABI (iwae_amd/_capi.py)");
static_assert(sizeof(iwae_local_options) == 64 && offsetof(iwae_local_options, objective) == 16 && offsetof(iwae_local_options, lr) == 20 && offsetof(iwae_local_options, epsilon) == 32 &&
              offsetof(iwae_local_options, mu0) == 40 && offsetof(iwae_local_options, eps) == 56 && sizeof(iwae_local_outputs) == 9 * sizeof(void*), "iwae_local_options / iwae_local_outputs layout is part of the ABI (iwae_amd/_capi.py)");
static_assert(sizeof(iwae_impute_options) == 24 && offsetof(iwae_impute_options, k) == 4 && offsetof(iwae_impute_options, mask) == 8 && offsetof(iwae_impute_options, eps) == 16 &&
              sizeof(iwae_impute_outputs) == 6 * sizeof(void*), "iwae_impute_options / iwae_impute_outputs layout is part of the ABI (iwae_amd/_capi.py)");
static_assert(sizeof(iwae_posterior_options) == 40 && offsetof(iwae_posterior_options, k) == 4 && offsetof(iwae_posterior_options, R) == 8 && offsetof(iwae_posterior_options, reserved) == 12 &&
              offsetof(iwae_posterior_options, mask) == 16 && offsetof(iwae_posterior_options, eps) == 24 && offsetof(iwae_posterior_options, unif) == 32 &&
// ... 52 lines not shown
void init_linear(Linear& L, int Kin, int Nspace, bool need_B, bool kmajor) {
    L.Kin = Kin;
    L.Nspace = Nspace;
    L.Kp32 = round_up(Kin, 32);
    L.Np32 = round_up(Nspace, 32);
    L.KT = L.Kp32 / 32;
    L.MG = (L.Np32 + 63) / 64;
    L.imgF_bytes = (size_t)L.MG * img_mg_group_bytes(L.KT);
    L.kmajor = kmajor ? 1 : 0;
    if (need_B) {
        if (kmajor) {
            L.MT_B = L.Kp32 / 16;
            L.imgB_bytes = (size_t)L.MG * 2 * L.MT_B * 1024;
        } else {
            L.KT_B = L.Np32 / 32;
            L.MG_B = (L.Kp32 + 63) / 64;
            L.imgB_bytes = (size_t)L.MG_B * img_mg_group_bytes(L.KT_B);
        }
    }
    L.IT = L.Kp32 / 16;
    L.JT = L.Np32 / 16;
}

int alloc_linear(Linear& L) {
    HIPCHK(hipMalloc((void**)&L.imgF, L.imgF_bytes));
    HIPCHK(hipMemset(L.imgF, 0, L.imgF_bytes));
    if (L.imgB_bytes) {
        HIPCHK(hipMalloc((void**)&L.imgB, L.imgB_bytes));
        HIPCHK(hipMemset(L.imgB, 0, L.imgB_bytes));
    }
    return IWAE_OK;
}

void free_linear(Linear& L) {
    if (L.imgF) (void)hipFree(L.imgF);
    if (L.imgB) (void)hipFree(L.imgB);
    free_buf(L.slabW);
    free_buf(L.slabB);
}

void add_block(iwae_model* m, Linear* blk, const char* prefix, int Kin, int H, int D, bool need_dx_first) {
    const int base = (int)m->klayers.size();
    const char* nm[4] = {"l1", "l2", "lmu", "lstd"};
    const int kin[4] = {Kin, H, H, H}, nout[4] = {H, H, D, D};
    for (int i = 0; i < 4; ++i) {
        KerasLayer kl;
        kl.name = std::string(prefix) + "." + nm[i];
        kl.Kin = kin[i];
        kl.Nout = nout[i];
        kl.offW = m->nparam;
        m->nparam += (size_t)kin[i] * nout[i];
        kl.offb = m->nparam;
        m->nparam += nout[i];
        m->klayers.push_back(kl);
    }
    const int Dp = round_up(D, 32);
    init_linear(blk[0], Kin, H, need_dx_first, false);
    blk[0].nsub = 1; blk[0].sub[0] = base;
    init_linear(blk[1], H, H, true, false);
    blk[1].nsub = 1; blk[1].sub[0] = base + 1;
    init_linear(blk[2], H, 2 * Dp, true, false);
    blk[2].nsub = 2; blk[2].sub[0] = base + 2; blk[2].sub[1] = base + 3; blk[2].joff[1] = Dp;
}

void add_mlp3(iwae_model* m, Linear* mlp, const char* prefix, int D, int H, int X) {
    const int base = (int)m->klayers.size();
    const char* nm[3] = {"d1", "d2", "out"};
    const int kin[3] = {D, H, H}, nout[3] = {H, H, X};
    for (int i = 0; i < 3; ++i) {
        KerasLayer kl;
        kl.name = std::string(prefix) + "." + nm[i];
        kl.Kin = kin[i];
        kl.Nout = nout[i];
        kl.offW = m->nparam;
        m->nparam += (size_t)kin[i] * nout[i];
        kl.offb = m->nparam;
        m->nparam += nout[i];
        m->klayers.push_back(kl);
    }
    init_linear(mlp[0], D, H, true, false);
    mlp[0].nsub = 1; mlp[0].sub[0] = base;
    init_linear(mlp[1], H, H, true, false);
    mlp[1].nsub = 1; mlp[1].sub[0] = base + 1;
    init_linear(mlp[2], H, X, true, true);
    mlp[2].nsub = 1; mlp[2].sub[0] = base + 2;
}

std::vector<Linear*> all_linears(iwae_model* m) {
    std::vector<Linear*> v;
    for (int i = 0; i < 3; ++i) v.push_back(&m->enc1[i]);
    if (m->cfg.n_layers == 2) {
        for (int i = 0; i < 3; ++i) v.push_back(&m->enc2[i]);
        for (int i = 0; i < 3; ++i) v.push_back(&m->dec2[i]);
    }
    for (int i = 0; i < 3; ++i) v.push_back(&m->dec1[i]);
    if (m->has_prior) for (int i = 0; i < 3; ++i) v.push_back(&m->prior[i]);
    return v;
}

bool dec_layers_last(const iwae_model* m) {
    const int d0 = m->dec1[0].sub[0];
    return m->dec1[0].nsub == 1 && m->dec1[1].nsub == 1 && m->dec1[2].nsub == 1 && m->dec1[1].sub[0] == d0 + 1 && m->dec1[2].sub[0] == d0 + 2 && d0 + 3 == (int)m->klayers.size();
}
bool side_layers_from_enc2(const iwae_model* m) { return m->cfg.n_layers == 2 && m->enc2[0].nsub >= 1; }

}
int build_descs(iwae_model* m) {
    m->descs.assign(m->klayers.size(), LayerDesc());
    for (Linear* L : all_linears(m)) {
        for (int s = 0; s < L->nsub; ++s) {
            const KerasLayer& kl = m->klayers[L->sub[s]];
            LayerDesc& d = m->descs[L->sub[s]];
            d.Kin = kl.Kin; d.Nout = kl.Nout; d.joff = L->joff[s];
            d.offW = kl.offW; d.offb = kl.offb;
            d.imgF = L->imgF; d.KT_F = L->KT;
            d.imgB = L->imgB; d.KT_B = L->KT_B; d.MT_B = L->MT_B; d.imgB_kmajor = L->kmajor;
            d.slabW = ptr<float>(L->slabW); d.slabB = ptr<float>(L->slabB);
            d.nsplit = L->nsplit; d.slab_ld = L->JT * 16; d.slab_stride = (size_t)L->IT * 16 * L->JT * 16;
            d.slabB_stride = 0;
            if (m->plan.g2w && L == &m->dec1[2]) {
                d.slabB = ptr<float>(L->slabW) + (size_t)kl.Kin * d.slab_ld;
                d.slabB_stride = d.slab_stride;
            }
        }
    }
    int blocks = 0, rblocks = 0;
    for (auto& d : m->descs) {
        d.block_begin = blocks;
        d.rblock_begin = rblocks;
        blocks += (d.Kin * d.Nout + d.Nout + 255) / 256;
        rblocks += ((d.Kin + 1) * ((d.Nout + 3) / 4) + 63) / 64;
    }
    auto at = [&](int i) { return i < (int)m->descs.size() ? TableBounds::At{m->descs[i].rblock_begin, m->descs[i].block_begin} : TableBounds::At{rblocks, blocks}; };
    const bool two = m->cfg.n_layers == 2;
    TableBounds& t = m->tb;
    t.enc1_end = at(m->enc1[2].sub[m->enc1[2].nsub - 1] + 1);
    t.enc2 = two ? at(m->enc2[0].sub[0]) : t.enc1_end;
    t.dec2 = two ? at(m->dec2[0].sub[0]) : t.enc1_end;
    t.dec1 = at(m->dec1[0].sub[0]); t.dec1_out = at(m->dec1[2].sub[0]); t.dec1_end = at(m->dec1[2].sub[0] + 1);
    t.end = at((int)m->descs.size());
    if (!m->d_descs) HIPCHK(hipMalloc((void**)&m->d_descs, sizeof(LayerDesc) * m->descs.size()));
    HIPCHK(hipMemcpyAsync(m->d_descs, m->descs.data(), sizeof(LayerDesc) * m->descs.size(), hipMemcpyHostToDevice, m->stream));
    HIPCHK(hipStreamSynchronize(m->stream));
    if (m->side) HIPCHK(hipStreamSynchronize(m->side));
    if (m->side2) HIPCHK(hipStreamSynchronize(m->side2));
    m->descs_dirty = false;
    m->g2w_descs = m->plan.g2w;
    return IWAE_OK;
}
namespace {

void reduce_blocks(iwae_model* m, hipStream_t st, BlockRange a, BlockRange b, float alpha, bool update, hipEvent_t done, bool with_means) {
    const float* per_b = with_means ? ptr<float>(m->per_b) : nullptr;
    launch_reduce_grads(m->d_descs, (int)m->descs.size(), a.first, a.count, m->grad, m->param, m->mom, m->vel, alpha, m->adam_b1, m->adam_b2, m->adam_eps, update ? 1 : 0,
                        per_b, per_b ? m->B : 0, !per_b ? 0.f : m->cfg.n_layers == 2 ? 1.f : m->beta, per_b ? m->d_scalars : nullptr, st, b.first, b.count, done);
}
}
void adam_blocks(iwae_model* m, hipStream_t st, int first, int count, float alpha, float grad_scale, hipEvent_t done, bool update) {
    launch_adam(m->d_descs, (int)m->descs.size(), count, m->param, m->grad, m->mom, m->vel, alpha, grad_scale, m->adam_b1, m->adam_b2, m->adam_eps, update ? 1 : 0, st, first, done);
}
namespace {

int refresh_images(iwae_model* m) {
    if (m->descs_dirty) CHK(build_descs(m));
    adam_blocks(m, m->stream, 0, m->tb.end.e, 0.f, 1.f, nullptr, false);
    HIPCHK(hipGetLastError());
    return IWAE_OK;
}

static inline int eps_ld(const iwae_model* m, int layer) { return 4 * ((m->D[layer] + 3) / 4); }
}
EpsSrc eps_src(iwae_model* m, int layer) {
    EpsSrc e;
    e.user = nullptr;
    e.cache = m->epsc_ptr[layer];
    e.ldC = eps_ld(m, layer);
    if (m->user_eps) e.user = ptr<float>(m->epsbuf) + (layer == 0 ? 0 : (size_t)m->k * m->B * m->D[0]);
    e.B = m->B;
    e.seed = m->cfg.seed;
    e.row_offset = (uint64_t)m->call.batch_offset * (uint64_t)m->k;
    e.step = m->noise_step;
    e.stream = (uint32_t)layer;
    if (m->call.k_total > 0) {
        e.k_total = m->call.k_total; e.s_off = m->call.s_off; e.kc = m->k;
        e.row_offset = (uint64_t)m->call.batch_offset * (uint64_t)m->call.k_total;
    }
    return e;
}
namespace {

int attach_dense_stamps(iwae_model* m, int epi, DenseArgs& a) {
    if (m->dstamp_epi != epi || m->dstamp_kt != a.KT || (a.M < 4096 && a.KT <= 8)) return IWAE_OK;
    m->dstamp_waves = std::max(((a.M + 127) / 128) * ((a.MG + a.mg_per_block - 1) / a.mg_per_block) * 4, epi == EPI_BERN ? ((a.M + 127) / 128) * 16 : 0);
    CHK(ensure(m->dstamps, (size_t)m->dstamp_waves * 64, m->stream));
    a.stamps = ptr<unsigned long long>(m->dstamps);
    return IWAE_OK;
}

bool block_fwd_shape(const iwae_model* m, const Linear* blk, int R, BlockFwdArgs& a) {
    memset(&a, 0, sizeof(a));
    a.ldX = blk[0].Kp32; a.img0 = blk[0].imgF; a.img1 = blk[1].imgF; a.img2 = blk[2].imgF;
    a.KT0 = blk[0].KT; a.KT1 = blk[1].KT; a.NT1 = blk[0].Np32 / 16; a.NT2 = blk[2].Np32 / 16; a.R = R;
    a.ldH = blk[0].Np32; a.ldYF = blk[2].Np32; a.split = (blk[2].nsub == 2) ? blk[2].joff[1] : (1 << 30);
    return m->opt.allow_block_fused && blk[1].Np32 == blk[0].Np32 && blk[2].KT == blk[1].KT && blk[1].Kp32 == blk[0].Np32 && block_fwd_ok(a);
}

void wgradp_shape(const iwae_model* m, const Linear& L, int rows, int& nsplit, int& nw, int& cps) {
    const int chunks = (rows + 63) / 64;
    nw = (L.JT > 8 && chunks >= 128) ? 16 : 8;
    if (nw == 16 && L.IT <= 14 && m->opt.allow_wg7) nw = (m->opt.wg_shape9 & (L.JT > 16 ? 1 : 2)) ? 9 : 7;
    const int blocks = ((L.JT + wgradp_strip(nw) - 1) / wgradp_strip(nw)) * ((L.IT + 15) / 16);
    const int target16 = m->opt.wg_target16 > 0 ? m->opt.wg_target16 : (m->cfg.n_layers == 2 ? 64 : 96);
    const int target = (nw != 8) ? (blocks == 1 ? m->opt.wg_target16_1 : target16) : (chunks < 128 ? m->opt.wg_target8_few : m->opt.wg_target8);
    nsplit = std::max(1, std::min(chunks, target / std::max(1, blocks)));
    cps = (chunks + nsplit - 1) / nsplit;
    nsplit = (chunks + cps - 1) / cps;
}
int wgradp_plan(iwae_model* m, Linear& L, const uint16_t* XP, const uint16_t* GP, int rows, WgradPArgs& a, int& nsplit, int& nw) {
    int cps;
    wgradp_shape(m, L, rows, nsplit, nw, cps);
    const size_t needW = (size_t)nsplit * L.IT * 16 * L.JT * 16 * 4, needB = (size_t)nsplit * L.JT * 16 * 4;
    void* oldW = L.slabW.p; void* oldB = L.slabB.p;
    CHK(ensure(L.slabW, needW, m->stream));
    CHK(ensure(L.slabB, needB, m->stream));
    if (oldW != L.slabW.p || oldB != L.slabB.p || nsplit != L.nsplit) { L.nsplit = nsplit; m->descs_dirty = true; }
    a.X = XP; a.ldX = L.Kp32; a.IT = L.IT; a.G = GP; a.ldG = L.Np32; a.JT = L.JT; a.M = rows; a.rows_per_split = cps * 64;
    a.slabW = ptr<float>(L.slabW); a.slabB = ptr<float>(L.slabB); a.zero = m->d_zero; a.rowscale = nullptr;
    a.dbg = m->wg_debug;
    a.stamps = nullptr;
    return IWAE_OK;
}

int wgradp(iwae_model* m, Linear& L, const uint16_t* XP, const uint16_t* GP, int rows, hipStream_t st = nullptr,
           const float* rowscale = nullptr, hipEvent_t done = nullptr) {
    WgradPArgs a;
    int nsplit = 1, nw = 8;
    CHK(wgradp_plan(m, L, XP, GP, rows, a, nsplit, nw));
    a.rowscale = rowscale;
    if (rowscale && (m->fake_s & 2)) a.dbg |= 32;
#ifdef IWAE_DENSE_STAMPS
    if (m->dstamp_epi == 10 && rowscale && nw == 7) {
        m->dstamp_waves = ((L.JT + 15) / 16) * nsplit * 12;
        CHK(ensure(m->dstamps, (size_t)m->dstamp_waves * 64, m->stream));
        a.stamps = ptr<unsigned long long>(m->dstamps);
    }
#endif
    launch_wgradp(a, nsplit, nw, st ? st : m->stream, done);
    HIPCHK(hipGetLastError());
    return IWAE_OK;
}

int wgradp_two_plan(iwae_model* m, Linear& L, const uint16_t* XP, const uint16_t* GP, int rows, const float* rowscale, WgradPArgs& a1, int& n1, WgradPArgs& a2, int& n2) {
    const int blocks = (L.JT + 15) / 16;
    const int chunks = (rows + 63) / 64;
    const int c1 = std::min(chunks - 1, std::max(1, (int)((long)chunks * m->opt.wout_split / 100)));
    const int c2 = chunks - c1;
    auto split = [&](int ch, int target, int& n, int& cps) { n = std::max(1, std::min(ch, target / std::max(1, blocks))); cps = (ch + n - 1) / n; n = (ch + cps - 1) / cps; };
    int cps1, cps2;
    split(c1, m->opt.wout_wg1, n1, cps1);
    split(c2, m->opt.wout_wg2, n2, cps2);
    const int ns = n1 + n2;
    const size_t stride = (size_t)L.IT * 16 * L.JT * 16;
    void* oldW = L.slabW.p; void* oldB = L.slabB.p;
    CHK(ensure(L.slabW, (size_t)ns * stride * 4, m->stream));
    CHK(ensure(L.slabB, (size_t)ns * L.JT * 16 * 4, m->stream));
    if (oldW != L.slabW.p || oldB != L.slabB.p || ns != L.nsplit) { L.nsplit = ns; m->descs_dirty = true; }
    const int R1 = c1 * 64;
    memset(&a1, 0, sizeof(a1));
    a1.X = XP; a1.ldX = L.Kp32; a1.IT = L.IT; a1.G = GP; a1.ldG = L.Np32; a1.JT = L.JT; a1.M = R1; a1.rows_per_split = cps1 * 64;
    a1.slabW = ptr<float>(L.slabW); a1.slabB = ptr<float>(L.slabB); a1.zero = m->d_zero; a1.rowscale = rowscale;
    a2 = a1;
    a2.X = XP + (size_t)R1 * L.Kp32; a2.G = GP + (size_t)R1 * L.Np32; a2.M = rows - R1; a2.rows_per_split = cps2 * 64;
    a2.slabW = a1.slabW + (size_t)n1 * stride; a2.slabB = a1.slabB + (size_t)n1 * L.JT * 16; a2.rowscale = rowscale + R1;
    return IWAE_OK;
}

int dense_dx(iwae_model* m, Linear& L, const uint16_t* GP, int rows, const uint16_t* ACT, uint16_t* YP, float* YF, hipEvent_t done = nullptr) {
    DenseArgs a;
    memset(&a, 0, sizeof(a));
    a.X = GP; a.ldX = L.Np32; a.img = L.imgB;
    a.split = 1 << 30;
    a.M = rows; a.KT = L.KT_B; a.MG = L.MG_B; a.mg_per_block = (rows <= 8192) ? 1 : L.MG_B; a.Np32 = L.Kp32; a.g1_mask = m->opt.dense_g1_mask;
    a.YP = YP; a.ldYP = L.Kp32; a.YF = YF; a.ldYF = L.Kp32;
    a.ACT = ACT; a.ldACT = L.Kp32;
    CHK(attach_dense_stamps(m, ACT ? EPI_DX : EPI_F32, a));
    launch_dense(ACT ? EPI_DX : EPI_F32, a, m->stream, done);
    HIPCHK(hipGetLastError());
    return IWAE_OK;
}

bool block_bwd_shape(const iwae_model* m, const Linear* blk, int R, BlockBwdArgs& b) {
    memset(&b, 0, sizeof(b));
    b.ldDH = blk[2].Np32; b.imgH = blk[2].imgB; b.imgL2 = blk[1].imgB;
    b.KTH = blk[2].KT_B; b.KT1 = blk[1].KT_B; b.NT1 = blk[0].Np32 / 16; b.R = R; b.ldH = blk[0].Np32;
    return m->opt.allow_block_fused && !blk[2].kmajor && !blk[1].kmajor && blk[1].Np32 == blk[0].Np32 && blk[1].Kp32 == blk[0].Np32 && blk[2].Kp32 == blk[0].Np32 && block_bwd_ok(b);
}
bool lat_in_block_ok(const Linear* blk, int Dp, bool prior, bool f32_rows) { return Dp <= 128 && Dp == blk[2].Np32 / 2 && !prior && !f32_rows; }
int block_bwd(iwae_model* m, Linear* blk, BlockWs& w, const uint16_t* inP, int R, bool need_dx, bool wgrad_on_side, bool dx_done = false, hipStream_t side_st = nullptr,
              bool skip_wgrad = false, const LatentBwdArgs* lat = nullptr) {
    bool chain_fused = dx_done;
    if (dx_done) need_dx = false;
    BlockBwdArgs b;
    if (!dx_done && block_bwd_shape(m, blk, R, b)) {
        b.DH = ptr<uint16_t>(w.dheadP); b.H2 = ptr<uint16_t>(w.h2P); b.H1 = ptr<uint16_t>(w.h1P);
        b.D2 = ptr<uint16_t>(w.d2P); b.D1 = ptr<uint16_t>(w.d1P);
        if (lat) {
            if (!lat_in_block_ok(blk, lat->Dp, lat->prior_head != nullptr, lat->DHF != nullptr)) return fail(IWAE_ERR_STATE, "block_bwd: latent sums on a shape block_bwd_kernel does not cover");
            b.lat_on = 1; b.lat = *lat;
            b.rows_per_wg = lat->k > 16 ? 4 : 16;
        }
        launch_block_bwd(b, m->stream); chain_fused = true;
    } else if (lat) return fail(IWAE_ERR_STATE, "block_bwd: latent sums on a shape block_bwd_kernel does not cover");
    if (!chain_fused) {
        CHK(dense_dx(m, blk[2], ptr<uint16_t>(w.dheadP), R, ptr<uint16_t>(w.h2P), ptr<uint16_t>(w.d2P), nullptr));
        CHK(dense_dx(m, blk[1], ptr<uint16_t>(w.d2P), R, ptr<uint16_t>(w.h1P), ptr<uint16_t>(w.d1P), nullptr));
    }
    if (need_dx) CHK(dense_dx(m, blk[0], ptr<uint16_t>(w.d1P), R, nullptr, nullptr, ptr<float>(w.dx)));
    if (skip_wgrad) { HIPCHK(hipGetLastError()); return IWAE_OK; }
    const uint16_t* xs[3] = {ptr<uint16_t>(w.h2P), ptr<uint16_t>(w.h1P), inP};
    const uint16_t* gs[3] = {ptr<uint16_t>(w.dheadP), ptr<uint16_t>(w.d2P), ptr<uint16_t>(w.d1P)};
    Linear* ls[3] = {&blk[2], &blk[1], &blk[0]};
    hipStream_t ws = m->stream;
    if (wgrad_on_side) {
        ws = side_st ? side_st : m->side;
        if (!dx_done) HIPCHK(hipEventRecord(m->ev_blk, m->stream));
        HIPCHK(hipStreamWaitEvent(ws, m->ev_blk, 0));
    }
    WgradPGroup g;
    memset(&g, 0, sizeof(g));
    int nsplit[3], nw[3];
    bool small = true;
    for (int i = 0; i < 3; ++i) {
        CHK(wgradp_plan(m, *ls[i], xs[i], gs[i], R, g.a[i], nsplit[i], nw[i]));
        small = small && nw[i] == 8;
    }
    if (small) {
        g.n = 3;
        for (int i = 0; i < 3; ++i) {
            g.gx[i] = (ls[i]->JT + 7) / 8; g.gy[i] = (ls[i]->IT + 15) / 16;
            g.zbeg[i + 1] = g.zbeg[i] + nsplit[i];
        }
        launch_wgradp_group(g, ws);
    } else {
        for (int i = 0; i < 3; ++i) launch_wgradp(g.a[i], nsplit[i], nw[i], ws);
    }
    HIPCHK(hipGetLastError());
    return IWAE_OK;
}

bool wgrad_rows_ok(const iwae_model* m, const Linear* blk, int R) {
    return m->opt.allow_wgrad_rows && R <= 2048 && blk[0].nsub == 1 && blk[1].nsub == 1 && blk[2].nsub <= 2 && !blk[0].kmajor && !blk[1].kmajor && !blk[2].kmajor;
}
bool dec_rows_step(const iwae_model* m, int M, int B) {
    return m->opt.allow_dec_rows && m->cfg.n_layers == 1 && M <= 2048 && wgrad_rows_ok(m, m->enc1, B) && m->dec1[0].nsub == 1 && m->dec1[1].nsub == 1 &&
           m->dec1[2].nsub == 1 && !m->dec1[0].kmajor && !m->dec1[1].kmajor;
}
int block_wgrad_rows(iwae_model* m, Linear* blk, BlockWs& w, const uint16_t* inP, int R, float alpha, bool fuse, bool with_means, bool with_decoder = false) {
    if (m->descs_dirty) CHK(build_descs(m));
    const uint16_t* xs[6] = {ptr<uint16_t>(w.h2P), ptr<uint16_t>(w.h1P), inP, ptr<uint16_t>(m->wdec1.g2P), ptr<uint16_t>(m->wdec1.g1P), ptr<uint16_t>(m->zP[0])};
    const uint16_t* gs[6] = {ptr<uint16_t>(w.dheadP), ptr<uint16_t>(w.d2P), ptr<uint16_t>(w.d1P), ptr<uint16_t>(m->wdec1.dlP), ptr<uint16_t>(m->wdec1.d2P), ptr<uint16_t>(m->wdec1.d1P)};
    Linear* ls[6] = {&blk[2], &blk[1], &blk[0], &m->dec1[2], &m->dec1[1], &m->dec1[0]};
    const int njobs = with_decoder ? 6 : 3;
    WgradRowsJob jobs[6];
    memset(jobs, 0, sizeof(jobs));
    for (int i = 0; i < njobs; ++i) {
        jobs[i].X = xs[i]; jobs[i].ldX = ls[i]->Kp32; jobs[i].G = gs[i]; jobs[i].ldG = ls[i]->Np32; jobs[i].R = i < 3 ? R : m->M;
        jobs[i].sub0 = ls[i]->sub[0];
        jobs[i].sub1 = ls[i]->nsub == 2 ? ls[i]->sub[1] : -1;
        jobs[i].split = ls[i]->nsub == 2 ? ls[i]->joff[1] : (1 << 30);
    }
    if (with_decoder && m->plan.s_mode) jobs[3].rowscale = ptr<float>(m->gx);
    const bool two = m->cfg.n_layers == 2;
    launch_wgrad_rows(jobs, njobs, m->d_descs, m->grad, m->param, m->mom, m->vel, alpha, m->adam_b1, m->adam_b2, m->adam_eps, fuse ? 1 : 0,
                      with_means ? ptr<float>(m->per_b) : nullptr, m->B, two ? 1.f : m->beta, m->d_scalars, m->d_zero, m->stream);
    HIPCHK(hipGetLastError());
    return IWAE_OK;
}

}
int draw_eps(iwae_model* m, int par, uint32_t step, int M, hipStream_t gs, int max_blocks) {
    const int Mp = round_up(M, 128);
    iwae_model::EpsTag& tg = m->eps_tag[par];
    tg.valid = false;
    for (int l = 0; l < m->cfg.n_layers; ++l) {
        CHK(ensure(m->epsc[par][l], (size_t)Mp * m->Dp[l] * 4, m->stream));
        EpsSrc e = eps_src(m, l);
        e.user = nullptr; e.cache = nullptr; e.step = step;
        if (!(m->abl_skip & 16)) launch_eps_gen(e, M, m->D[l], eps_ld(m, l), ptr<float>(m->epsc[par][l]), gs, max_blocks);
    }
    HIPCHK(hipGetLastError());
    tg.valid = true; tg.step = step; tg.row_offset = (uint64_t)m->call.batch_offset * (uint64_t)m->k; tg.M = M;
    return IWAE_OK;
}
namespace {

#define EPSM_STEPS 8
int draw_eps_multi(iwae_model* m, int buf, uint32_t step0, int M, hipStream_t gs) {
    const int Mp = round_up(M, 128);
    iwae_model::EpsMTag& tg = m->epsm_tag[buf];
    tg.valid = false;
    for (int l = 0; l < m->cfg.n_layers; ++l) {
        const size_t stride = (size_t)Mp * eps_ld(m, l);
        CHK(ensure(m->epsm[buf][l], (size_t)EPSM_STEPS * stride * 4, m->stream));
        EpsSrc e = eps_src(m, l);
        e.user = nullptr; e.cache = nullptr; e.step = step0;
        launch_eps_gen_multi(e, M, m->D[l], eps_ld(m, l), ptr<float>(m->epsm[buf][l]), EPSM_STEPS, stride, gs);
    }
    HIPCHK(hipGetLastError());
    tg.valid = true; tg.step0 = step0; tg.row_offset = (uint64_t)m->call.batch_offset * (uint64_t)m->k; tg.M = M;
    return IWAE_OK;
}
int epsm_find(const iwae_model* m, uint32_t step, int M) {
    const uint64_t ro = (uint64_t)m->call.batch_offset * (uint64_t)m->k;
    for (int i = 0; i < 2; ++i) {
        const iwae_model::EpsMTag& t = m->epsm_tag[i];
        if (t.valid && t.M == M && t.row_offset == ro && step - t.step0 < (uint32_t)EPSM_STEPS) return i;
    }
    return -1;
}

inline hipStream_t on_stream(const iwae_model* m, OnStream s) { return s == ON_SIDE2 ? m->side2 : s == ON_SIDE ? m->side : m->stream; }

StepPlan plan_step(const iwae_model* m, int B, int k, int objective, bool bwd, const FwdCall& call, const iwae_tensors* want, bool host_eps) {
    const StepOptions& o = m->opt;
    StepPlan p = StepPlan();
    const bool two = m->cfg.n_layers == 2;
    const int M = B * k, Mp = round_up(M, 128), X = m->X, Xp = m->Xp32;
    const Linear* d1 = m->dec1;
    const Linear& L = m->dec1[2];
    BlockFwdArgs bf;
    p.enc_takes_f32 = m->C == 0 && block_fwd_shape(m, m->enc1, B, bf);
    p.dec_rows = bwd && dec_rows_step(m, M, B);
    p.want_dreg = !two && (objective == OBJ_DREG || (!bwd && !call.log_w_only));
    p.zin_eval = !bwd && !two && m->C == 0 && o.allow_zin && o.allow_zin_eval && (int64_t)B * k >= 8192 && o.allow_dec_fused && o.allow_bern_pipe;
    p.keep_eps = !host_eps && (bwd || two || p.zin_eval);
    p.eps_multi = p.keep_eps && bwd && !two && o.allow_eps_multi && call.k_total == 0 && p.dec_rows;
    const bool fuse_z = o.allow_zin && !two && m->C == 0 && (bwd || p.zin_eval) && p.keep_eps && M >= 8192 && (d1[0].KT == 4 || d1[0].KT == 2) && d1[0].Kp32 == m->Dp[0];
    const bool sample_in_block = o.allow_block_fused && o.allow_zin && !two && !fuse_z && M <= 4096 && d1[0].Kp32 == m->Dp[0];
    if (two) {
        const Linear *e2 = m->enc2, *d2 = m->dec2;
        p.chain = o.allow_chain2 && chain2_fwd_ok(e2[0].KT, e2[1].KT, d2[0].KT, M) && e2[0].Kp32 == m->Dp[0] && e2[0].Np32 == 32 * e2[1].KT &&
                  e2[1].Np32 == e2[0].Np32 && e2[2].KT == e2[1].KT && e2[2].Np32 == 2 * m->Dp[1] && d2[0].Kp32 == m->Dp[1] && d2[0].Np32 == e2[0].Np32 &&
                  d2[1].KT == e2[1].KT && d2[1].Np32 == d2[0].Np32 && d2[2].KT == e2[1].KT && d2[2].Np32 == 2 * m->Dp[0];
        p.chain2_bwd = p.chain && bwd && o.allow_chain2_bwd && gblock_bwd_ok(e2[0].KT, e2[1].KT, d2[0].KT, M) && e2[0].imgB && d2[0].imgB;
    }
    DenseArgs& a = p.bern;
    a.ldX = L.Kp32; a.img = L.imgF;
    a.split = 1 << 30;
    a.M = M; a.KT = L.KT; a.MG = L.MG; a.mg_per_block = L.MG; a.Np32 = L.Np32; a.g1_mask = o.dense_g1_mask;
    const bool out_in_block = o.allow_block_fused && o.allow_out_in_block && !fuse_z && M <= 4096 && !(want && want->logits) && !m->want_stamps &&
                              d1[1].Np32 == d1[0].Np32 && d1[1].Kp32 == d1[0].Np32 && L.Kp32 == d1[1].Np32 && L.KT == d1[1].KT && L.KT <= 8;
    if (M < 8192 && L.MG > 1 && !out_in_block) { a.mg_per_block = 1; p.px_parts = L.MG; }
    a.ldXB = m->Xinp; a.k = k; a.B = B; a.Xdim = X;
    a.lpxz_stride = p.px_parts > 1 ? (size_t)Mp : 0;
    p.s_mode = bwd && o.allow_s_mode && out_bwd_has_s_mode(L.KT);
    if (p.s_mode) {
        a.ldYP = Xp;
        if (m->fake_s & 4) a.dbg = 32;
        if (m->fake_s & 16) a.dbg |= 64;
        if (m->fake_s & 32) a.dbg |= 128;
        if (m->fake_s & 64) a.dbg |= 256;
        if (m->fake_s & 128) a.dbg |= 512;
    }
    a.pipe = o.allow_bern_pipe ? 1 : 0;
    if (a.pipe && o.bern_qw) {
        const int nwg = (M + 199) / 200, ncu = std::max(1, m->num_cus);
        const int rounds = (nwg + ncu - 1) / ncu;
        if ((double)nwg >= 0.9 * (double)rounds * ncu || o.bern_qw_force) a.pipe = 2;
    }
    if (o.allow_dec_fused && a.pipe && m->C == 0 && d1[0].KT <= 4 && d1[0].Kp32 == m->Dp[0] && d1[0].Np32 == L.Kp32 && d1[1].Kp32 == L.Kp32 && d1[1].Np32 == L.Kp32) {
        DenseArgs pre = a;
        pre.pre_img1 = d1[0].imgF; pre.pre_KT1 = d1[0].KT; pre.pre_img2 = d1[1].imgF;
        pre.logits_out = want ? want->logits : nullptr;
        if (bern_pipe_ok(pre)) { a = pre; p.dec_fwd = DEC_PIPE; }
    }
    if (p.dec_fwd != DEC_PIPE && o.allow_block_fused && !fuse_z && M <= 4096 && d1[1].Np32 == d1[0].Np32 && d1[1].Kp32 == d1[0].Np32) {
        BlockFwdArgs& b = p.dec_blk;
        b.ldX = d1[0].Kp32; b.img0 = d1[0].imgF; b.img1 = d1[1].imgF; b.img2 = d1[1].imgF;
        b.KT0 = d1[0].KT; b.KT1 = d1[1].KT; b.NT1 = d1[0].Np32 / 16; b.NT2 = 0; b.R = M;
        b.ldH = d1[0].Np32; b.split = 1 << 30;
        if (sample_in_block) { b.sample = 1; b.S.Dp = m->Dp[0]; b.S.M = M; }
        if (out_in_block) { b.oimg = L.imgF; b.oXdim = X; b.oH = L.Np32 >> 5; b.oldXB = m->Xinp; b.ok = k; b.oldS = Xp; }
        if (block_fwd_shape_ok(b)) p.dec_fwd = out_in_block ? DEC_BLOCK_OUT : DEC_BLOCK2;
    }
    const bool in_block = p.dec_fwd == DEC_BLOCK2 || p.dec_fwd == DEC_BLOCK_OUT;
    p.z_from = p.chain ? Z_CHAIN2 : (fuse_z && p.dec_fwd == DEC_PIPE) ? Z_DEC_PROLOGUE : (fuse_z && !p.want_dreg) ? Z_DENSE_ZIN : (sample_in_block && in_block) ? Z_BLOCK : Z_SAMPLE;
    p.early_wout = bwd && p.s_mode && o.allow_early_wout && !p.dec_rows;
    if (p.dec_fwd == DEC_PIPE && o.allow_lse_fused && !m->want_stamps) {
        DenseArgs lse = a;
        lse.lse_on = 1; lse.lse.n_px_part = 1;
        if (bern_lse_ok(lse)) { a.lse_on = 1; p.lse_fused = true; }
    }
    p.g2w = p.lse_fused && p.early_wout && o.allow_g2w && p.s_mode && L.Kin < L.Kp32 && !two;
    if (p.g2w) a.g2w_feat = L.Kin;
    p.lse_dup = p.early_wout && o.allow_lse_dup && p.px_parts == 1 && p.dec_fwd != DEC_BLOCK_OUT && !p.lse_fused;
    if (p.lse_fused) p.lse_at = LSE_DECODER;
    if (!bwd) return p;

    const bool small_fused = o.small_dec_bwd && o.allow_dec_bwd && p.s_mode && M <= o.small_rows && out_bwd_has_s_mode(L.KT) && !m->want_stamps;
    p.out_parts = p.s_mode && M < 8192 && L.MG > 1 && !small_fused;
    const bool fused_dx = o.allow_dec_bwd && p.s_mode && !p.out_parts && (M >= 8192 || small_fused) && !(m->want_stamps && L.KT == 7) && L.kmajor && L.imgB &&
                          d1[1].KT_B == L.KT && d1[1].MG_B == (L.KT + 1) / 2 && d1[0].KT_B == L.KT && d1[1].Kp32 == L.Kp32 && d1[0].Np32 == L.Kp32;
    p.dz_half = fused_dx && !two && o.allow_dz_half;
    DecBwdRowsArgs& r = p.rows;
    r.ldS = Xp; r.KTX = Xp / 32; r.imgK3 = L.imgB; r.MT3 = L.MT_B;
    r.imgB2 = d1[1].imgB; r.imgB1 = d1[0].imgB; r.KT = L.KT; r.NT1 = L.Kp32 / 16; r.NT3 = d1[0].Kp32 / 16; r.M = M;
    r.ldH = L.Kp32; r.ldDZ = d1[0].Kp32;
    p.dx = !fused_dx ? DX_THREE : (M <= o.dec_rows_max && o.allow_block_fused && dec_bwd_rows_ok(r)) ? DX_ROWS : DX_DEC_BWD;
    if (!p.lse_fused && o.allow_lse_in_bwd && !p.lse_dup && !p.early_wout && p.dx == DX_ROWS && small_fused && !two) { p.lse_at = LSE_BWD_ROWS; r.lse_on = 1; }
    const bool few_side2 = p.early_wout && o.allow_wg3 && o.use_side2 && M <= 4096;
    int ns[3], nw[3], cps;
    for (int i = 0; i < 3; ++i) wgradp_shape(m, d1[i], M, ns[i], nw[i], cps);
    p.group3 = few_side2 && fused_dx && nw[0] == 8 && nw[1] == 8 && nw[2] == 8;
    p.wout_two_part = !p.dec_rows && !p.group3 && o.wout_split > 0 && p.s_mode && !p.g2w && p.early_wout && o.use_side2 && fused_dx && M >= 8192 && L.IT <= 14 && o.allow_wg7 && !(m->abl_skip & 1);
    p.hid_on = p.dec_rows ? ON_MAIN : (p.group3 || (p.early_wout && o.use_side2)) ? ON_SIDE2 : ON_SIDE;
    p.hid_group = nw[1] == 7 && nw[0] == 7 && o.allow_wg_group && (p.early_wout || fused_dx);
    p.tail = p.dec_rows ? ON_SIDE : p.hid_on;
    p.draw_on = p.dec_rows ? ON_MAIN : few_side2 ? ON_SIDE2 : ON_SIDE;
    BlockBwdArgs bb;
    p.lat_fuse = o.allow_lat_in_block && B <= 1024 && (k <= 16 || (o.allow_lat_rows4 && B >= 64)) && block_bwd_shape(m, m->enc1, B, bb) &&
                 lat_in_block_ok(m->enc1, m->Dp[0], m->has_prior, false);
    p.rows_enc = wgrad_rows_ok(m, m->enc1, B);
    return p;
}

void plan_step_end(const iwae_model* m, const StepPlan& p, StepEnd mode, StepEndPlan& e) {
    const StepOptions& o = m->opt;
    const TableBounds& t = m->tb;
    const bool two = m->cfg.n_layers == 2;
    const bool fuse = mode == END_UPDATE, split = mode == END_GRAD_SPLIT || mode == END_GRAD_SPLIT_HELD;
    const bool dec_own = !two && !p.dec_rows && dec_layers_last(m);
    const bool defer = fuse && o.allow_defer && dec_own;
    const bool split_upd = defer && o.defer_split && p.hid_on == ON_SIDE2 && !p.group3 && p.early_wout;
    const bool early = !fuse && dec_own;
    const bool defer2 = fuse && two && o.allow_defer && o.allow_defer2 && side_layers_from_enc2(m) && p.chain2_bwd && p.early_wout && o.use_side2 && !split;
    const bool defer2_split = defer2 && p.tail == ON_SIDE2 && o.allow_defer2_split && m->dec2[0].nsub == 1 && m->dec1[0].nsub == 1 && m->dec1[2].nsub == 1;
    e = StepEndPlan();
    e.update = fuse;
    e.how = early ? (mode == END_GRAD_SPLIT_HELD ? ENDS_EARLY_HELD : split ? ENDS_EARLY_SPLIT : ENDS_EARLY) : defer2 ? (defer2_split ? ENDS_DEFER2_SPLIT : ENDS_DEFER2) :
            p.dec_rows ? ENDS_DEC_ROWS : defer ? (split_upd ? ENDS_SPLIT_UPD : ENDS_DEFER) : ENDS_JOINED;
    e.join_both = e.how == ENDS_JOINED && two && p.tail != ON_SIDE;
    const int lo = p.rows_enc ? t.enc1_end.r : 0, hi = (defer || early) ? t.dec1.r : defer2 ? t.enc2.r : t.end.r;
    const int d0 = p.dec_rows ? t.dec1.r : hi, d1 = p.dec_rows ? t.dec1_end.r : hi;
    e.main_a = BlockRange{lo, std::max(0, std::min(d0, hi) - lo)};
    e.main_b = BlockRange{d1, std::max(0, hi - d1)};
    e.left.split_offset = early && split ? m->klayers[m->dec1[0].sub[0]].offW : m->nparam;
    e.left.on = p.tail;
    if (e.how == ENDS_JOINED || e.how == ENDS_DEC_ROWS) return;
    auto sum = [&](OnStream on, TableBounds::At a0, TableBounds::At a1, TableBounds::At b0, TableBounds::At b1, SideWait behind = WAIT_NONE, bool second = false) {
        e.side[e.nside++] = SideSum{on, BlockRange{a0.r, a1.r - a0.r}, BlockRange{b0.r, b1.r - b0.r}, behind, second};
    };
    if (e.how == ENDS_DEFER2_SPLIT) {
        sum(ON_SIDE2, t.enc2, t.dec2, t.dec1, t.dec1_out);
        sum(ON_SIDE, t.dec2, t.dec1, t.dec1_out, t.end, WAIT_NONE, true);
    } else if (e.how == ENDS_DEFER2) {
        sum(p.tail, t.enc2, t.end, t.end, t.end, p.tail != ON_SIDE ? WAIT_SIDE : WAIT_NONE);
    } else if (e.how == ENDS_SPLIT_UPD) {
        sum(ON_SIDE, t.dec1_out, t.end, t.end, t.end, WAIT_FORK2, true);
        sum(ON_SIDE2, t.dec1, t.dec1_out, t.end, t.end);
    } else {
        sum(p.tail, t.dec1, t.end, t.end, t.end);
        if (e.how == ENDS_EARLY_HELD) e.left.held = e.side[0].a;
    }
    e.left.dec = e.how != ENDS_EARLY;
    e.left.dec2 = e.nside == 2;
}

void lse_args(iwae_model* m, int objective, bool bwd, const iwae_tensors* want, LseArgs& a) {
    const bool two = m->cfg.n_layers == 2;
    float* lpxz = ptr<float>(m->rows[0]);
    memset(&a, 0, sizeof(a));
    if (!two) {
        a.term[0] = lpxz; a.coef[0] = 1.f;
        a.term[1] = ptr<float>(m->rows[1]); a.coef[1] = m->beta;
        a.term[2] = ptr<float>(m->rows[2]); a.coef[2] = -m->beta;
        a.head = ptr<float>(m->wenc1.head); a.ldH = 2 * m->Dp[0]; a.D = m->D[0]; a.Dp = m->Dp[0];
        a.cz_on = 1.f;
    } else {
        a.term[0] = lpxz; a.coef[0] = 1.f;
        a.term[1] = ptr<float>(m->rows[1]); a.coef[1] = 1.f;
        a.term[2] = ptr<float>(m->rows[2]); a.coef[2] = 1.f;
        a.term[3] = ptr<float>(m->rows[3]); a.coef[3] = -1.f;
        a.term[4] = ptr<float>(m->rows[4]); a.coef[4] = -1.f;
        a.head = nullptr;
        a.cz_on = 0.f;
    }
    a.lq_dreg = m->plan.want_dreg ? ptr<float>(m->rows[5]) : nullptr;
    a.B = m->B; a.k = m->k; a.beta = two ? 1.f : m->beta; a.objective = objective;
    a.lme_only = (!bwd && m->call.log_w_only && !want) ? 1 : 0;
    a.logw = ptr<float>(m->logw); a.wn = ptr<float>(m->wn); a.gx = ptr<float>(m->gx);
    a.cf = ptr<float4>(m->cf); a.per_b = ptr<float>(m->per_b);
    a.n_px_part = 1; a.px_stride = (size_t)m->Mp; a.term0_out = lpxz;
}
void lse_args_parts(iwae_model* m, int objective, bool bwd, const iwae_tensors* want, LseArgs& a) {
    lse_args(m, objective, bwd, want, a);
    if (m->plan.px_parts > 1) a.term[0] = ptr<float>(m->px_part);
    a.n_px_part = m->plan.px_parts;
}
int lse_alloc(iwae_model* m) {
    hipStream_t st = m->stream;
    CHK(ensure(m->logw, (size_t)m->Mp * 4, st));
    CHK(ensure(m->wn, (size_t)m->Mp * 4, st));
    {
        const void* before = m->gx.p;
        CHK(ensure(m->gx, (size_t)m->Mp * 4, st));
        if (m->gx.p != before) HIPCHK(hipMemsetAsync(m->gx.p, 0, m->gx.cap, st));
    }
    CHK(ensure(m->cf, (size_t)m->Mp * 16, st));
    CHK(ensure(m->per_b, (size_t)PB_COUNT * m->B * 4, st));
    return IWAE_OK;
}

}
int begin_forward(iwae_model* m, const float* x, int B, int k, float beta, const FwdCall& call, const float** cond) {
    const bool from_ds = m->ds_start >= 0;
    if ((!x && !from_ds) || B <= 0 || k <= 0) return fail(IWAE_ERR_ARG, "forward: need x, B > 0, k > 0");
    if ((int64_t)B * k > (int64_t)1 << 30) return fail(IWAE_ERR_ARG, "forward: B*k too large");
    const int row0 = from_ds ? 0 : call.cond_row0;
    *cond = nullptr;
    if (m->C > 0) {
        if (from_ds) {
            if (!m->ds_has_labels) return fail(IWAE_ERR_STATE, "conditional model on the resident dataset: call iwae_dataset_set_labels first");
            CHK(ensure(m->cond, (size_t)B * m->C * 4, m->stream));
            m->cond_n = B;
        }
        if (row0 + B > m->cond_n) return fail(IWAE_ERR_STATE, "conditional model: call iwae_set_condition with y for these images first");
        *cond = ptr<float>(m->cond) + (size_t)row0 * m->C;
    }
    m->call = call; m->call.cond_row0 = row0;
    m->B = B; m->k = k; m->M = B * k; m->beta = beta;
    m->Mp = round_up(m->M, 128); m->Bp = round_up(B, 128);
    return IWAE_OK;
}

int stage_input(iwae_model* m, const float* x, int B, bool keep_f32, const float** xd) {
    *xd = x;
    if (m->ds_start >= 0) {
        CHK(ensure(m->xP, (size_t)m->Bp * m->Xinp * 2, m->stream));
        if (keep_f32) CHK(ensure(m->xin, (size_t)B * m->X * 4, m->stream));
        float* xf = keep_f32 ? ptr<float>(m->xin) : nullptr;
        launch_gather_binarize(ptr<uint8_t>(m->ds_data), ptr<int32_t>(m->ds_order), m->ds_start, m->ds_N, B, m->X, m->Xinp, m->Bp, m->cfg.seed, m->ds_epoch,
                               ptr<uint16_t>(m->xP), xf, m->stream, m->C > 0 ? ptr<uint8_t>(m->ds_labels) : nullptr, m->C, m->C > 0 ? ptr<float>(m->cond) : nullptr);
        m->ds_start = -1;
        *xd = xf;
    } else CHK(staged_in(m, x, m->xin, (size_t)B * m->X * 4, xd));
    return IWAE_OK;
}
namespace {

int forward_impl(iwae_model* m, const float* x, int B, int k, float beta, const float* eps, int objective, bool bwd,
                 const iwae_tensors* want, const FwdCall& call) {
    const float* cond;
    CHK(begin_forward(m, x, B, k, beta, call, &cond));
    m->plan = plan_step(m, B, k, objective, bwd, call, want, eps != nullptr);
    const StepPlan& p = m->plan;
    const bool two = m->cfg.n_layers == 2;
    m->bf16_side_used = true;
    if (m->left.z_pending) { HIPCHK(hipStreamWaitEvent(m->stream, m->ev_join, 0)); m->left.z_pending = false; }
    m->time_this = m->timing > 0 && (m->timing_calls++ % m->timing) == 0;
    const int M = m->M, Mp = m->Mp, Bp = m->Bp, X = m->X, Xp = m->Xp32, Xinp = m->Xinp;
    hipStream_t st = m->stream;
    m->user_eps = eps != nullptr;
    m->epsc_ptr[0] = m->epsc_ptr[1] = nullptr;
    if (p.eps_multi) {
        int bi = epsm_find(m, m->noise_step, M);
        if (bi < 0) {
            bi = (m->epsm_tag[0].valid && !m->epsm_tag[1].valid) ? 1 : 0;
            CHK(draw_eps_multi(m, bi, m->noise_step, M, st));
        }
// ... 868 lines not shown
}
int iwae_set_output_bias(iwae_handle m, const float* bias, size_t n) {
    if (!m || !bias || n != (size_t)m->X) return fail(IWAE_ERR_ARG, "set_output_bias: need x_dim values");
    CHK(join_side(m));
    HIPCHK(hipMemcpyAsync(m->param + m->klayers[m->dec1[2].sub[0]].offb, bias, n * 4, hipMemcpyDefault, m->stream));
    CHK(refresh_images(m));
    HIPCHK(hipStreamSynchronize(m->stream));
    return IWAE_OK;
}
int iwae_get_grads(iwae_handle m, float* flat, size_t n) {
    if (!m || !flat || n != m->nparam) return fail(IWAE_ERR_ARG, "get_grads: size mismatch");
    CHK(join_side(m));
    HIPCHK(hipMemcpyAsync(flat, m->grad, n * 4, hipMemcpyDefault, m->stream));
    HIPCHK(hipStreamSynchronize(m->stream));
    return IWAE_OK;
}
int iwae_get_adam_state(iwae_handle m, float* mo, float* ve, size_t n, int64_t* step) {
    if (!m || n != m->nparam) return fail(IWAE_ERR_ARG, "get_adam_state: size mismatch");
    CHK(join_side(m));
    if (mo) HIPCHK(hipMemcpyAsync(mo, m->mom, n * 4, hipMemcpyDefault, m->stream));
    if (ve) HIPCHK(hipMemcpyAsync(ve, m->vel, n * 4, hipMemcpyDefault, m->stream));
    HIPCHK(hipStreamSynchronize(m->stream));
    if (step) *step = m->adam_t;
    return IWAE_OK;
}
int iwae_set_adam_state(iwae_handle m, const float* mo, const float* ve, size_t n, int64_t step) {
    if (!m || !mo || !ve || n != m->nparam || step < 0) return fail(IWAE_ERR_ARG, "set_adam_state: bad argument");
    CHK(join_side(m));
    HIPCHK(hipMemcpyAsync(m->mom, mo, n * 4, hipMemcpyDefault, m->stream));
    HIPCHK(hipMemcpyAsync(m->vel, ve, n * 4, hipMemcpyDefault, m->stream));
    HIPCHK(hipStreamSynchronize(m->stream));
    m->adam_t = step;
    return IWAE_OK;
}

int iwae_forward(iwae_handle m, const float* x, int32_t B, int32_t k, float beta, const float* eps, iwae_scalars* scalars,
                 const iwae_tensors* want) {
    if (!m) return fail(IWAE_ERR_ARG, "null handle");
    HIPCHK(hipSetDevice(m->cfg.device));
    if (m->cfg.precision == IWAE_PREC_FP32) CHK(forward_f32(m, x, B, k, beta, eps, OBJ_IWAE_ELBO, false, want, FwdCall{m->batch_offset}));
    else CHK(forward_impl(m, x, B, k, beta, eps, OBJ_IWAE_ELBO, false, want, FwdCall{m->batch_offset}));
    CHK(fetch_outputs(m, scalars, want));
    m->noise_step += 1;
    return IWAE_OK;
}

int iwae_forward_backward(iwae_handle m, const float* x, int32_t B, int32_t k, float beta, int32_t objective, const float* eps,
                          iwae_scalars* scalars, const iwae_tensors* want) {
    if (!m) return fail(IWAE_ERR_ARG, "null handle");
    HIPCHK(hipSetDevice(m->cfg.device));
    CHK(check_objective(m, objective));
    if (m->cfg.precision == IWAE_PREC_FP32) {
        CHK(forward_f32(m, x, B, k, beta, eps, objective, true, want, FwdCall{m->batch_offset}));
        CHK(backward_f32(m, objective, END_GRAD));
    } else {
        CHK(forward_impl(m, x, B, k, beta, eps, objective, true, want, FwdCall{m->batch_offset}));
        CHK(backward_impl(m, objective, END_GRAD));
    }
    CHK(fetch_outputs(m, scalars, want));
    m->noise_step += 1;
    return IWAE_OK;
}

int iwae_forward_backward_split(iwae_handle m, const float* x, int32_t B, int32_t k, float beta, int32_t objective, const float* eps,
                                void** side_stream, size_t* side_offset) {
    if (!m || !side_stream || !side_offset) return fail(IWAE_ERR_ARG, "null argument");
    HIPCHK(hipSetDevice(m->cfg.device));
    CHK(check_objective(m, objective));
    if (m->cfg.precision == IWAE_PREC_FP32) {
        CHK(forward_f32(m, x, B, k, beta, eps, objective, true, nullptr, FwdCall{m->batch_offset}));
        CHK(backward_f32(m, objective, END_GRAD_SPLIT));
        CHK(join_side(m));
    } else {
        CHK(forward_impl(m, x, B, k, beta, eps, objective, true, nullptr, FwdCall{m->batch_offset}));
        CHK(backward_impl(m, objective, END_GRAD_SPLIT));
    }
    *side_stream = (void*)on_stream(m, m->left.on);
    *side_offset = m->left.split_offset;
    m->noise_step += 1;
    return IWAE_OK;
}

int iwae_grad_devptr(iwae_handle m, void** p, size_t* n) {
    if (!m || !p || !n) return fail(IWAE_ERR_ARG, "null argument");
    CHK(join_side(m));
    *p = m->grad;
    *n = m->nparam;
    return IWAE_OK;
}

int iwae_adam_step(iwae_handle m, float lr, float grad_scale) {
    if (!m) return fail(IWAE_ERR_ARG, "null handle");
    HIPCHK(hipSetDevice(m->cfg.device));
    CHK(join_side(m));
    return adam_impl(m, lr, grad_scale);
}

int iwae_set_option(iwae_handle m, const char* name, int64_t value) {
    if (!m || !name) return fail(IWAE_ERR_ARG, "set_option: null argument");
    HIPCHK(hipSetDevice(m->cfg.device));
    CHK(join_side(m));
    HIPCHK(hipStreamSynchronize(m->stream));
    if (m->side) HIPCHK(hipStreamSynchronize(m->side));
    if (m->side2) HIPCHK(hipStreamSynchronize(m->side2));
    m->have_forward = false;
    const bool on = value != 0;
    const int iv = (int)value;
    const std::string n(name);
    if (n == "out_recompute") m->opt.allow_s_mode = !on;
    else if (n == "no_defer") m->opt.allow_defer = !on;
    else if (n == "wout_split") m->opt.wout_split = std::max(0, std::min(95, iv));
    else if (n == "wout_wg1") m->opt.wout_wg1 = std::max(1, iv);
    else if (n == "wout_wg2") m->opt.wout_wg2 = std::max(1, iv);
    else if (n == "defer_split") m->opt.defer_split = on;
    else if (n == "no_eps_multi") m->opt.allow_eps_multi = !on;
    else if (n == "no_zin") m->opt.allow_zin = !on;
    else if (n == "zin_eval") m->opt.allow_zin_eval = on;
    else if (n == "no_chain2_bwd") m->opt.allow_chain2_bwd = !on;
    else if (n == "no_chain2") m->opt.allow_chain2 = !on;
    else if (n == "no_dec_bwd") m->opt.allow_dec_bwd = !on;
    else if (n == "no_defer2_split") m->opt.allow_defer2_split = !on;
    else if (n == "no_defer2") m->opt.allow_defer2 = !on;
    else if (n == "f32_dw_tiles") m->opt.f32_dw_tiles = std::max(1, iv);
    else if (n == "f32_dw_min_rows") m->opt.f32_dw_min_rows = std::max(16, iv);
    else if (n == "f32_gemm_dbg") m->opt.gemm_f32.dbg = iv;
    else if (n == "f32_gemm_small_min") m->opt.gemm_f32.v2_small_min = std::max(1, iv);
    else if (n == "f32_ksplit_min_tiles") m->opt.gemm_f32.ksplit_min_tiles = std::max(1, iv);
    else if (n == "f32_no_ksplit") m->opt.gemm_f32.ksplit = !on;
    else if (n == "f32_gemm_small_v1") m->opt.gemm_f32.v2_small = !on;
    else if (n == "f32_gemm_w4") m->opt.gemm_f32.w8 = !on;
    else if (n == "f32_gemm_v1") m->opt.gemm_f32.v2 = !on;
    else if (n == "no_f32_side") m->opt.allow_f32_side = !on;
    else if (n == "f32_dw_last") m->opt.f32_dw_last = iv;
    else if (n == "f32_wout_last") m->opt.f32_wout_first = !on;
    else if (n == "no_f32_multi_reduce") m->opt.allow_f32_multi_reduce = !on;
    else if (n == "f32_dec_fused_train") m->opt.f32_dec_fused_train = on;
    else if (n == "no_f32_dec_fused") m->opt.allow_f32_dec_fused = !on;
    else if (n == "no_f32_bern_fused") m->opt.allow_f32_bern_fused = !on;
    else if (n == "no_dec_rows") m->opt.allow_dec_rows = !on;
    else if (n == "no_wgrad_rows") m->opt.allow_wgrad_rows = !on;
    else if (n == "no_wg3") m->opt.allow_wg3 = !on;
    else if (n == "g2w") m->opt.allow_g2w = on;
    else if (n == "lat_rows4") m->opt.allow_lat_rows4 = on;
    else if (n == "no_lat_in_block") m->opt.allow_lat_in_block = !on;
    else if (n == "no_lse_in_bwd") m->opt.allow_lse_in_bwd = !on;
    else if (n == "no_lse_fused") m->opt.allow_lse_fused = !on;
    else if (n == "no_lse_dup") m->opt.allow_lse_dup = !on;
    else if (n == "dz_f32") m->opt.allow_dz_half = !on;
    else if (n == "no_small_dec_bwd") m->opt.small_dec_bwd = !on;
    else if (n == "small_rows") m->opt.small_rows = iv;
    else if (n == "dec_rows") m->opt.dec_rows_max = iv;
    else if (n == "no_wg7") m->opt.allow_wg7 = !on;
    else if (n == "wg9") m->opt.wg_shape9 = iv;
    else if (n == "grid_chunk") m->opt.grid_chunk = iv > 0 ? std::max(16, iv) : 0;
    else if (n == "ais_t_chunk") m->opt.ais_t_chunk = iv > 0 ? iv : 0;
    else if (n == "local_t_chunk") m->opt.local_t_chunk = iv > 0 ? iv : 0;
    else if (n == "impute_rows") m->opt.impute_rows = iv > 0 ? iv : 0;
    else if (n == "eval_rows") m->opt.eval_rows = iv > 0 ? std::max(64, iv) : 0;
    else if (n == "no_bern_pipe") m->opt.allow_bern_pipe = !on;
    else if (n == "no_block_fused") m->opt.allow_block_fused = !on;
    else if (n == "no_out_in_block") m->opt.allow_out_in_block = !on;
    else if (n == "no_dec_fused") m->opt.allow_dec_fused = !on;
    else if (n == "no_bern_qw") m->opt.bern_qw = !on;
    else if (n == "bern_qw_force") m->opt.bern_qw_force = on;
    else if (n == "dense_g1") m->opt.dense_g1_mask = (unsigned)iv;
    else if (n == "wg8") m->opt.wg_target8 = std::max(1, iv);
    else if (n == "wg8_few") m->opt.wg_target8_few = std::max(1, iv);
    else if (n == "wg16") m->opt.wg_target16 = std::max(1, iv);
    else if (n == "wg16_1") m->opt.wg_target16_1 = std::max(1, iv);
    else if (n == "eps_blocks") m->opt.eps_blocks = std::max(0, iv);
    else if (n == "dec_bwd_nw") m->opt.dec_bwd_nw = iv == 8 ? 8 : 4;
    else if (n == "no_side2") m->opt.use_side2 = !on;
    else if (n == "wg_group") m->opt.allow_wg_group = on;
    else if (n == "no_early_wout") m->opt.allow_early_wout = !on;
    else if (n == "dp_concurrent") m->opt.dp_concurrent = on;
#ifdef IWAE_DIAG
    else if (n == "stamps") { m->want_stamps = on; if (on) { m->opt.allow_s_mode = false; m->opt.allow_bern_pipe = false; m->opt.allow_block_fused = false; m->opt.allow_dec_fused = false; } }
    else if (n == "dense_stamps_epi") m->dstamp_epi = iv;
    else if (n == "dense_stamps_kt") m->dstamp_kt = iv;
    else if (n == "wg_debug") m->wg_debug = iv;
    else if (n == "abl_skip") m->abl_skip = iv;
    else if (n == "fake_s") m->fake_s = iv;
#endif
    else return fail(IWAE_ERR_ARG, "set_option: unknown option '" + n + "'");
    return IWAE_OK;
}

int iwae_set_eval_precision(iwae_handle m, int32_t precision) {
    if (!m) return fail(IWAE_ERR_ARG, "null handle");
    if (precision != IWAE_PREC_BF16 && precision != IWAE_PREC_FP32) return fail(IWAE_ERR_ARG, "precision must be IWAE_PREC_BF16 or IWAE_PREC_FP32");
    m->eval_precision = precision;
    return IWAE_OK;
}

int iwae_set_adam(iwae_handle m, float beta1, float beta2, float epsilon) {
    if (!m) return fail(IWAE_ERR_ARG, "null handle");
    if (!(beta1 >= 0.f && beta1 < 1.f) || !(beta2 >= 0.f && beta2 < 1.f) || !(epsilon > 0.f)) return fail(IWAE_ERR_ARG, "set_adam: need 0 <= beta < 1, epsilon > 0");
    m->adam_b1 = beta1; m->adam_b2 = beta2; m->adam_eps = epsilon;
    return IWAE_OK;
}

int iwae_train_step(iwae_handle m, const float* x, int32_t B, int32_t k, float beta, float lr, int32_t objective, const float* eps,
                    iwae_scalars* scalars, const iwae_tensors* want) {
    if (!m) return fail(IWAE_ERR_ARG, "null handle");
    HIPCHK(hipSetDevice(m->cfg.device));
    CHK(check_objective(m, objective));
    if (m->cfg.precision == IWAE_PREC_FP32) {
        CHK(forward_f32(m, x, B, k, beta, eps, objective, true, want, FwdCall{m->batch_offset}));
        if (m->comm_main || want) {
            CHK(backward_f32(m, objective, m->comm_main ? END_GRAD_SPLIT_HELD : END_GRAD));
            if (want) CHK(fetch_outputs(m, nullptr, want));
            if (m->comm_main) CHK(dp_finish(m, lr));
            else { CHK(join_side(m)); CHK(adam_impl(m, lr, 1.0f)); }
        } else {
            CHK(backward_f32(m, objective, END_UPDATE, lr));
        }
        CHK(fetch_outputs(m, scalars, nullptr));
        m->noise_step += 1;
        return IWAE_OK;
    }
    CHK(forward_impl(m, x, B, k, beta, eps, objective, true, want, FwdCall{m->batch_offset}));
    if (m->comm_main) {
        CHK(backward_impl(m, objective, END_GRAD_SPLIT_HELD));
        if (want) CHK(fetch_outputs(m, nullptr, want));
        CHK(dp_finish(m, lr));
    } else if (want) {
        CHK(backward_impl(m, objective, END_GRAD));
        CHK(fetch_outputs(m, nullptr, want));
        CHK(adam_impl(m, lr, 1.0f));
    } else {
        CHK(backward_impl(m, objective, END_UPDATE, lr));
    }
    CHK(fetch_outputs(m, scalars, nullptr));
    m->noise_step += 1;
    return IWAE_OK;
}

int iwae_comm_unique_id(void* id_out, size_t cap, size_t* id_bytes) {
    if (!id_out || !id_bytes || cap < 2 * sizeof(ncclUniqueId)) return fail(IWAE_ERR_ARG, "comm_unique_id: need a buffer of >= 256 bytes");
    CHK(load_rccl());
    ncclUniqueId ids[2];
    NCCLCHK(g_rccl.GetUniqueId(&ids[0]));
    NCCLCHK(g_rccl.GetUniqueId(&ids[1]));
    memcpy(id_out, ids, sizeof(ids));
    *id_bytes = sizeof(ids);
    return IWAE_OK;
}

int iwae_comm_preflight(iwae_handle m, const void* unique_id, size_t id_bytes, int32_t world_size, int32_t rank) {
    if (!m || !unique_id || id_bytes != 2 * sizeof(ncclUniqueId)) return fail(IWAE_ERR_ARG, "comm_init: bad id blob (iwae_comm_unique_id makes it)");
    if (world_size < 1 || rank < 0 || rank >= world_size) return fail(IWAE_ERR_ARG, "comm_init: need 0 <= rank < world_size");
    if (world_size != m->cfg.world_size || rank != m->cfg.rank)
        return fail(IWAE_ERR_ARG, "comm_init: world_size / rank differ from the iwae_config this handle was created with");
    if (m->comm_main) return fail(IWAE_ERR_STATE, "comm_init: communicators already exist (iwae_comm_destroy first)");
    CHK(load_rccl());
    return IWAE_OK;
}

int iwae_comm_init(iwae_handle m, const void* unique_id, size_t id_bytes, int32_t world_size, int32_t rank) {
    CHK(iwae_comm_preflight(m, unique_id, id_bytes, world_size, rank));
    HIPCHK(hipSetDevice(m->cfg.device));
    CHK(join_side(m));
    HIPCHK(hipStreamSynchronize(m->stream));
    ncclUniqueId ids[2];
    memcpy(ids, unique_id, sizeof(ids));
    if (!m->ev_ar) HIPCHK(hipEventCreateWithFlags(&m->ev_ar, hipEventDisableTiming));
    ncclComm_t cm = nullptr, cs = nullptr;
    ncclResult_t r1 = g_rccl.CommInitRank(&cm, world_size, ids[0], rank);
    ncclResult_t r2 = r1 == ncclSuccess ? g_rccl.CommInitRank(&cs, world_size, ids[1], rank) : r1;
    if (r1 != ncclSuccess || r2 != ncclSuccess) {
        if (r1 == ncclSuccess && cm) (void)g_rccl.CommDestroy(cm);
        return fail(IWAE_ERR_HIP, std::string("ncclCommInitRank: ") + g_rccl.GetErrorString(r1 != ncclSuccess ? r1 : r2));
    }
    m->comm_main = cm; m->comm_side = cs;
    m->comm_world = world_size; m->comm_rank = rank;
    return IWAE_OK;
}

int iwae_comm_destroy(iwae_handle m) {
    if (!m) return fail(IWAE_ERR_ARG, "null handle");
    CHK(join_side(m));
    HIPCHK(hipStreamSynchronize(m->stream));
    if (m->side) HIPCHK(hipStreamSynchronize(m->side));
    if (m->side2) HIPCHK(hipStreamSynchronize(m->side2));
    if (m->comm_main) { NCCLCHK(g_rccl.CommDestroy(m->comm_main)); m->comm_main = nullptr; }
    if (m->comm_side) { NCCLCHK(g_rccl.CommDestroy(m->comm_side)); m->comm_side = nullptr; }
    m->comm_world = 1; m->comm_rank = 0;
    return IWAE_OK;
}

int iwae_comm_info(iwae_handle m, int32_t* world_size, int32_t* rank) {
    if (!m || !world_size || !rank) return fail(IWAE_ERR_ARG, "comm_info: null argument");
    *world_size = 0; *rank = -1;
    if (!m->comm_main) return IWAE_OK;
    int n = 0, r = -1, n2 = 0;
    NCCLCHK(g_rccl.CommCount(m->comm_main, &n));
    NCCLCHK(g_rccl.CommUserRank(m->comm_main, &r));
    NCCLCHK(g_rccl.CommCount(m->comm_side, &n2));
    if (n2 != n) return fail(IWAE_ERR_STATE, "comm_info: the two communicators disagree about the world size");
    *world_size = n; *rank = r;
    return IWAE_OK;
}

int iwae_set_condition(iwae_handle m, const float* y, int32_t n) {
    if (!m || !y || n <= 0) return fail(IWAE_ERR_ARG, "set_condition: bad argument");
    if (m->C <= 0) return fail(IWAE_ERR_STATE, "set_condition: the model was created with cond_dim = 0");
// ... 386 lines not shown
```

### iwae_amd/csrc/wgrad_kernels.hip

```cpp
#include <hip/hip_runtime.h>
#include <hip/hip_ext.h>
#include <stdint.h>
#include <algorithm>
#include "kernels.h"
#include "layout.h"
#include "device_helpers.h"
#include "step_helpers.h"

namespace iwae {
__device__ __forceinline__ void wait_vmem_but(int n) {
    switch (n) {
        case 0: asm volatile("s_waitcnt vmcnt(0)" ::: "memory"); break;
        case 1: asm volatile("s_waitcnt vmcnt(1)" ::: "memory"); break;
        case 2: asm volatile("s_waitcnt vmcnt(2)" ::: "memory"); break;
        case 3: asm volatile("s_waitcnt vmcnt(3)" ::: "memory"); break;
        case 4: asm volatile("s_waitcnt vmcnt(4)" ::: "memory"); break;
        case 5: asm volatile("s_waitcnt vmcnt(5)" ::: "memory"); break;
        case 6: asm volatile("s_waitcnt vmcnt(6)" ::: "memory"); break;
        case 7: asm volatile("s_waitcnt vmcnt(7)" ::: "memory"); break;
        case 8: asm volatile("s_waitcnt vmcnt(8)" ::: "memory"); break;
        case 9: asm volatile("s_waitcnt vmcnt(9)" ::: "memory"); break;
        case 10: asm volatile("s_waitcnt vmcnt(10)" ::: "memory"); break;
        case 11: asm volatile("s_waitcnt vmcnt(11)" ::: "memory"); break;
        default: asm volatile("s_waitcnt vmcnt(12)" ::: "memory"); break;
// ... 43 lines not shown
        } else if (SC && pc == XP + GP) {
            pbase[idx] = (const char*)(a.rowscale + rbeg) + (lane & 7) * 16;
            plim[idx] = lane < WG_SR / 4 ? (1 << 30) : -(1 << 30);
            pstride[idx] = WG_SR * 4;
        } else if (pc < NPC) {
            constexpr int SPR = GROW / 16, RPP = 1024 / GROW;
            const int rl = RPP * (pc - XP) + lane / SPR, sl = lane % SPR;
            const int col = gcol0 + (sl ^ ((rl & 3) << 2)) * 8;
            pbase[idx] = (const char*)a.G + ((size_t)(rbeg + rl) * a.ldG + col) * 2;
            plim[idx] = col < a.ldG ? rend - rbeg - rl : -(1 << 30);
            pstride[idx] = WG_SR * a.ldG * 2;
        }
    }
    auto dma_piece = [&](int c, int idx) {
        const int pc = wave + NW * idx;
        if (pc >= NPC) return;
        const char* src = (c * WG_SR < plim[idx]) ? pbase[idx] + (size_t)c * (size_t)pstride[idx] : zsrc;
        glds16(src, (uint32_t)__builtin_amdgcn_readfirstlane((int)(lds_addr_of(smem + (c % WG_NST) * BUF) + (uint32_t)pc * 1024u)));
    };

    f32x4 acc[AI][BJ];
#pragma unroll
    for (int t = 0; t < AI; ++t)
#pragma unroll
        for (int u = 0; u < BJ; ++u) acc[t][u] = (f32x4){0.0f, 0.0f, 0.0f, 0.0f};
    float bsum[BJ];
#pragma unroll
    for (int u = 0; u < BJ; ++u) bsum[u] = 0.0f;
    for (int c = 0; c < min(nstage, WG_NST - 1); ++c) {
#pragma unroll
        for (int idx = 0; idx < NIDX; ++idx) dma_piece(c, idx);
    }
    const int xrow_off = (4 * q + qp) * 512, grow_off = (4 * q + qp) * GROW;

    for (int c = 0; c < nstage; ++c) {
        const int buf = c % WG_NST;
        wait_vmem_but(my_pieces * min(WG_NST - 2, nstage - 1 - c));
        __syncthreads();
        const bool more = c + WG_NST - 1 < nstage && !WG_DBG(a, 1);
        int dma_idx = 0;
        auto dma_next = [&]() {
            if (more && dma_idx < NIDX) dma_piece(c + WG_NST - 1, dma_idx);
            ++dma_idx;
        };
        const char* xb = smem + buf * BUF + xrow_off + p * 16;
        const char* gbase = smem + buf * BUF + XT_BYTES + grow_off;
        {
            uint4 g[BJ];
#pragma unroll
            for (int u = 0; u < BJ; ++u) {
                const int jl = jg * BJ + u;
                const char* gb = gbase + ((((4 * (jl >> 1)) ^ (qp << 2)) + p) * 16) + 8 * (jl & 1);
                const v4s g0 = __builtin_amdgcn_ds_read_tr16_b64_v4i16((__attribute__((address_space(3))) v4s*)gb);
                const v4s g1 = __builtin_amdgcn_ds_read_tr16_b64_v4i16((__attribute__((address_space(3))) v4s*)(gb + 16 * GROW));
                const uint2 glo = __builtin_bit_cast(uint2, g0), ghi = __builtin_bit_cast(uint2, g1);
                g[u] = make_uint4(glo.x, glo.y, ghi.x, ghi.y);
            }
            if (SC && !WG_DBG(a, 8)) {
                const float* scl = (const float*)(smem + buf * BUF + XT_BYTES + GT_BYTES) + 4 * q;
                const float4 s0 = *(const float4*)scl, s1 = *(const float4*)(scl + 16);
#pragma unroll
                for (int u = 0; u < BJ; ++u)
                    g[u] = make_uint4(pack2(bflo(g[u].x) * s0.x, bfhi(g[u].x) * s0.y), pack2(bflo(g[u].y) * s0.z, bfhi(g[u].y) * s0.w),
                                      pack2(bflo(g[u].z) * s1.x, bfhi(g[u].z) * s1.y), pack2(bflo(g[u].w) * s1.z, bfhi(g[u].w) * s1.w));
            }
            if (ig == 0 && !WG_DBG(a, 4)) {
#pragma unroll
                for (int u = 0; u < BJ; ++u)
                    bsum[u] += bflo(g[u].x) + bfhi(g[u].x) + bflo(g[u].y) + bfhi(g[u].y) + bflo(g[u].z) + bfhi(g[u].z) + bflo(g[u].w) + bfhi(g[u].w);
            }
            if (!WG_DBG(a, 2)) lds_pipeline<AI, (AI < 3 ? AI : 3)>(
                [&](int t) {
                    const int i = ig * AI + t;
                    const char* p0 = xb + ((((4 * (i >> 1)) ^ (qp << 2))) * 16) + 8 * (i & 1);
                    const v4s r0 = __builtin_amdgcn_ds_read_tr16_b64_v4i16((__attribute__((address_space(3))) v4s*)p0);
                    const v4s r1 = __builtin_amdgcn_ds_read_tr16_b64_v4i16((__attribute__((address_space(3))) v4s*)(p0 + 16 * 512));
                    const uint2 lo = __builtin_bit_cast(uint2, r0), hi = __builtin_bit_cast(uint2, r1);
                    return make_uint4(lo.x, lo.y, hi.x, hi.y);
                },
                [&](int t, const uint4& av) {
                    if (ig * AI + t < nit) {
#pragma unroll
                        for (int u = 0; u < BJ; ++u) acc[t][u] = mfma16(av, g[u], acc[t][u]);
                    }
                },
                [&](int t) { if (t == 0 || (AI > 1 && t == AI / 2) || (AI > 3 && t == AI - 1)) dma_next(); });
        }
        while (dma_idx < NIDX) dma_next();
    }

    float* slab = a.slabW + (size_t)split * a.IT * 16 * a.JT * 16;
    if (WG_DBG(a, 16)) return;
#pragma unroll
    for (int u = 0; u < BJ; ++u) {
        const int jt = bx * STRIP + jg * BJ + u;
        if (jt < a.JT) {
#pragma unroll
            for (int t = 0; t < AI; ++t) {
                const int it = ig * AI + t;
                if (it < nit) {
#pragma unroll
                    for (int ii = 0; ii < 4; ++ii)
                        slab[(size_t)((it0 + it) * 16 + 4 * q + ii) * (a.JT * 16) + jt * 16 + l16] = acc[t][u][ii];
                }
            }
            if (by == 0 && ig == 0) {
                float v = bsum[u];
                v += __shfl_xor(v, 16);
                v += __shfl_xor(v, 32);
                if (q == 0) a.slabB[(size_t)split * a.JT * 16 + jt * 16 + l16] = v;
            }
        }
    }
}

template <int NW, int IGC, int AI, int BJ, bool SC>
__global__ __launch_bounds__(NW * 64, (AI * BJ > 16) ? 2 : NW / 4) void wgradp_kernel(WgradPArgs a) {
    int bx = blockIdx.x, by = blockIdx.y, bz = blockIdx.z;
    const int gx = gridDim.x, gy = gridDim.y, nb = gx * gy * (int)gridDim.z;
    if ((nb & 7) == 0) {
        const int L = bx + gx * (by + gy * bz);
        const int V = (L & 7) * (nb >> 3) + (L >> 3);
        bx = V % gx; by = (V / gx) % gy; bz = V / (gx * gy);
    }
    wgradp_body<NW, IGC, AI, BJ, SC>(a, bx, by, bz);
}

#ifdef IWAE_DENSE_STAMPS
#define WS_STAMP(slot)                                                                 \
    {                                                                                  \
        unsigned long long t_;                                                         \
        __builtin_amdgcn_sched_barrier(0);                                             \
        asm volatile("s_memtime %0\n\ts_waitcnt lgkmcnt(0)" : "=s"(t_)::"memory");     \
        __builtin_amdgcn_sched_barrier(0);                                             \
        ws_sum[slot] += t_ - ws_prev;                                                  \
        ws_prev = t_;                                                                  \
    }
#define WS_STAMP_OUT()                                                                                                         \
    if (a.stamps && lane == 0) {                                                                                               \
        for (int i_ = 0; i_ < 8; ++i_) a.stamps[((size_t)sid * (NCW + NLW) + wave) * 8 + i_] = ws_sum[i_];                     \
    }
#else
#define WS_STAMP(slot)
#define WS_STAMP_OUT()
#endif
__device__ __forceinline__ void wgradws_block(int& bx, int& bz, const int gx, const int nz) {
    const int nb = gx * nz;
    if ((nb & 7) == 0) {
        const int L = bx + gx * bz;
        const int V = (L & 7) * (nb >> 3) + (L >> 3);
        bx = V % gx; bz = V / gx;
    }
}
template <bool SC, int BJ, int NLW>
__device__ __forceinline__ void wgradws_body(const WgradPArgs& a, const int jt0, const int bz, const int sid) {
    extern __shared__ __attribute__((aligned(1024))) char smem[];
#ifdef IWAE_DENSE_STAMPS
    unsigned long long ws_sum[8] = {0, 0, 0, 0, 0, 0, 0, 0}, ws_prev = 0;
    asm volatile("s_memtime %0\n\ts_waitcnt lgkmcnt(0)" : "=s"(ws_prev)::"memory");
#endif
    constexpr int AI = 7, IGC = 2, NCW = 8, STRIP = 4 * BJ;
    constexpr int XT_BYTES = WG_SR * 512, GROW = STRIP * 32, GT_BYTES = WG_SR * GROW, BUF = XT_BYTES + GT_BYTES;
    constexpr int XP = XT_BYTES / 1024, GP = GT_BYTES / 1024, XPL = XP / NLW, GPL = GP / NLW, PPL = XPL + GPL;
    constexpr int SPR = GROW / 16, RPP = 1024 / GROW;
    static_assert(XP % NLW == 0 && GP % NLW == 0 && GPL >= 1 && GPL <= 4, "loader split");
    typedef __attribute__((ext_vector_type(4))) short v4s;
    auto gswz = [](int r) { return SPR >= 16 ? ((r & 3) << 2) : (((r >> 1) & 1) << 2); };
    const int tid = threadIdx.x, lane = tid & 63, wave = __builtin_amdgcn_readfirstlane(tid >> 6);
    const int rbeg = bz * a.rows_per_split;
    const int rend = min(a.M, rbeg + a.rows_per_split);
    const int nstage = (rend - rbeg + WG_SR - 1) / WG_SR;
    const int gcol0 = jt0 * 16;

    if (SC && wave >= NCW) {
        typedef __attribute__((ext_vector_type(4))) uint32_t u32x4;
        __builtin_amdgcn_s_setprio(3);
        const int lw = wave - NCW;
        const char* zsrc = a.zero + (lane & 31) * 16;
        const int xstride = WG_SR * a.ldX * 2, gstride = WG_DBG(a, 32) ? 0 : WG_SR * a.ldG * 2;
        const char* xbase[XPL]; int xlim[XPL];
#pragma unroll
        for (int i = 0; i < XPL; ++i) {
            const int pc = lw * XPL + i, rl = 2 * pc + (lane >> 5);
            const int col = ((lane & 31) ^ ((rl & 3) << 2)) * 8;
            xbase[i] = (const char*)a.X + ((size_t)(rbeg + rl) * a.ldX + col) * 2;
            xlim[i] = col < a.ldX ? rend - rbeg - rl : -(1 << 30);
        }
        const char* gbase[GPL]; int glim[GPL];
#pragma unroll
        for (int i = 0; i < GPL; ++i) {
            const int pc = lw * GPL + i, rl = RPP * pc + lane / SPR;
            const int col = gcol0 + ((lane % SPR) ^ gswz(rl)) * 8;
            const bool ok = col < a.ldG;
            gbase[i] = (const char*)a.G + ((size_t)(rbeg + rl) * a.ldG + (ok ? col : 0)) * 2;
            glim[i] = ok ? rend - rbeg - rl : -(1 << 30);
        }
        constexpr int NR = RPP * GPL;
        static_assert(NR == 8 || NR == 4, "row weights of a loader and stage are one s_load_dwordx8 / x4");
        typedef __attribute__((ext_vector_type(NR))) float wvec_t;
        auto load_w = [&](int st, wvec_t& w) {
            const uint64_t ad = (uint64_t)(a.rowscale + (rbeg + st * WG_SR + NR * lw));
            const uint64_t au = ((uint64_t)(uint32_t)__builtin_amdgcn_readfirstlane((int)(uint32_t)(ad >> 32)) << 32) |
                                (uint64_t)(uint32_t)__builtin_amdgcn_readfirstlane((int)(uint32_t)ad);
            if constexpr (NR == 8) asm volatile("s_load_dwordx8 %0, %1, 0x0" : "=s"(w) : "s"(au) : "memory");
            else asm volatile("s_load_dwordx4 %0, %1, 0x0" : "=s"(w) : "s"(au) : "memory");
        };
        auto wsel = [&](const wvec_t& w, int i) {
            float f = w[RPP * i];
#pragma unroll
            for (int r = 1; r < RPP; ++r) f = (lane / SPR == r) ? w[RPP * i + r] : f;
            return f;
        };
        constexpr int PER = GPL + XPL;
        u32x4 gq0[GPL], gq1[GPL], gq2[GPL], gq3[GPL];
        auto issue_g = [&](int st, int i, u32x4& dst) {
            const char* pg = (st * WG_SR < glim[i]) ? gbase[i] + (size_t)st * (size_t)gstride : (const char*)a.G;
            asm volatile("global_load_dwordx4 %0, %1, off" : "=v"(dst) : "v"(pg) : "memory");
        };
        auto issue_x = [&](int st, int i) {
            if (WG_DBG(a, 1)) return;
            const char* src = (st * WG_SR < xlim[i]) ? xbase[i] + (size_t)st * (size_t)xstride : zsrc;
            glds16(src, (uint32_t)__builtin_amdgcn_readfirstlane((int)(lds_addr_of(smem + (st % WG_NST) * BUF) + (uint32_t)(lw * XPL + i) * 1024u)));
        };
        auto put_piece = [&](int st, int i, const u32x4& v, const wvec_t& w) {
            const float f = (st * WG_SR < glim[i]) ? (WG_DBG(a, 8) ? 1.0f : wsel(w, i)) : 0.0f;
            *(uint4*)(smem + (st % WG_NST) * BUF + (XP + lw * GPL + i) * 1024 + lane * 16) =
                make_uint4(pack2(bflo(v.x) * f, bfhi(v.x) * f), pack2(bflo(v.y) * f, bfhi(v.y) * f),
                           pack2(bflo(v.z) * f, bfhi(v.z) * f), pack2(bflo(v.w) * f, bfhi(v.w) * f));
        };
        constexpr int XDMA = XPL;
        auto per_stage = [&](int st) { return (st < nstage) ? (WG_DBG(a, 1) ? PER - XDMA : PER) : 0; };
        wvec_t wcur;
        load_w(0, wcur);
        auto issue_all = [&](int st, u32x4 (&gs)[GPL]) {
#pragma unroll
            for (int i = 0; i < GPL; ++i) issue_g(st, i, gs[i]);
#pragma unroll
            for (int i = 0; i < XPL; ++i) issue_x(st, i);
        };
        if (0 < nstage) issue_all(0, gq0);
        if (1 < nstage) issue_all(1, gq1);
        if (2 < nstage) issue_all(2, gq2);
        wait_vmem_but_ws(per_stage(1) + per_stage(2));
        asm volatile("s_waitcnt lgkmcnt(0)" : "+s"(wcur) : : "memory");
        if (0 < nstage) {
#pragma unroll
            for (int i = 0; i < GPL; ++i) { asm volatile("" : "+v"(gq0[i])); put_piece(0, i, gq0[i], wcur); }
        }
        __syncthreads();
        WS_STAMP(0)
        auto iter = [&](int c, u32x4 (&gn)[GPL], u32x4 (&gc)[GPL]) {
            const bool next = c + 1 < nstage;
            if (next) load_w(c + 1, wcur);
            if (c + 3 < nstage) issue_all(c + 3, gn);
            WS_STAMP(1)
            if (next) {
                wait_vmem_but_ws(per_stage(c + 2) + per_stage(c + 3));
                asm volatile("s_waitcnt lgkmcnt(0)" : "+s"(wcur) : : "memory");
            }
            WS_STAMP(2)
            if (next) {
#pragma unroll
                for (int i = 0; i < GPL; ++i) { asm volatile("" : "+v"(gc[i])); put_piece(c + 1, i, gc[i], wcur); }
            }
            WS_STAMP(3)
            __syncthreads();
            WS_STAMP(4)
        };
        for (int c = 0; c < nstage; c += 4) {
            iter(c, gq3, gq1);
            if (c + 1 < nstage) iter(c + 1, gq0, gq2);
            if (c + 2 < nstage) iter(c + 2, gq1, gq3);
            if (c + 3 < nstage) iter(c + 3, gq2, gq0);
        }
        asm volatile("s_waitcnt vmcnt(0)" ::: "memory");
        WS_STAMP_OUT()
        return;
    }
    if (wave >= NCW) {
        const int lw = wave - NCW;
        const char* zsrc = a.zero + (lane & 31) * 16;
        const char* pbase[PPL];
        int plim[PPL];
        const int xstride = WG_SR * a.ldX * 2, gstride = WG_SR * a.ldG * 2;
#pragma unroll
        for (int i = 0; i < PPL; ++i) {
            const bool isx = i < XPL;
            int rl, col, ld;
            if (isx) {
                const int pc = lw * XPL + i;
                rl = 2 * pc + (lane >> 5);
                col = ((lane & 31) ^ ((rl & 3) << 2)) * 8;
                ld = a.ldX;
            } else {
                const int pc = lw * GPL + (i - XPL);
                rl = RPP * pc + lane / SPR;
                col = gcol0 + ((lane % SPR) ^ gswz(rl)) * 8;
                ld = a.ldG;
            }
            pbase[i] = (const char*)(isx ? a.X : a.G) + ((size_t)(rbeg + rl) * ld + col) * 2;
            plim[i] = col < ld ? rend - rbeg - rl : -(1 << 30);
        }
        auto issue = [&](int st) {
#pragma unroll
            for (int i = 0; i < PPL; ++i) {
                const bool isx = i < XPL;
                const int pc = isx ? lw * XPL + i : XP + lw * GPL + (i - XPL);
                const char* src = (st * WG_SR < plim[i]) ? pbase[i] + (size_t)st * (size_t)(isx ? xstride : gstride) : zsrc;
                glds16(src, (uint32_t)__builtin_amdgcn_readfirstlane((int)(lds_addr_of(smem + (st % WG_NST) * BUF) + (uint32_t)pc * 1024u)));
            }
        };
        if (0 < nstage) issue(0);
        if (1 < nstage) issue(1);
        if (2 < nstage) issue(2);
        wait_vmem_but_ws((1 < nstage ? PPL : 0) + (2 < nstage ? PPL : 0));
        __syncthreads();
        for (int c = 0; c < nstage; ++c) {
            const bool refill = c + 3 < nstage && !WG_DBG(a, 1);
            if (refill) issue(c + 3);
            if (c + 1 < nstage) wait_vmem_but_ws((c + 2 < nstage ? PPL : 0) + (refill ? PPL : 0));
            __syncthreads();
        }
        asm volatile("s_waitcnt vmcnt(0)" ::: "memory");
        return;
    }

    const int q = lane >> 4, l16 = lane & 15, qp = l16 >> 2, p = l16 & 3;
    const int ig = wave % IGC, jg = wave / IGC;
    f32x4 acc[AI][BJ], accb[BJ];
#pragma unroll
    for (int u = 0; u < BJ; ++u) {
        accb[u] = (f32x4){0.0f, 0.0f, 0.0f, 0.0f};
#pragma unroll
        for (int t = 0; t < AI; ++t) acc[t][u] = (f32x4){0.0f, 0.0f, 0.0f, 0.0f};
    }
    const int xrow_off = (4 * q + qp) * 512, grow_off = (4 * q + qp) * GROW;
    const uint4 ones = make_uint4(0x3F803F80u, 0x3F803F80u, 0x3F803F80u, 0x3F803F80u);
    const bool do_bias = ig == 0 && !WG_DBG(a, 4);
    __syncthreads();
    WS_STAMP(0)
    for (int c = 0; c < nstage; ++c) {
        const int buf = c % WG_NST;
        const char* xb = smem + buf * BUF + xrow_off + p * 16;
        const char* gbase = smem + buf * BUF + XT_BYTES + grow_off;
        uint4 g[BJ];
#pragma unroll
        for (int u = 0; u < BJ; ++u) {
            const int jl = jg * BJ + u;
            const char* gb = gbase + ((((4 * (jl >> 1)) ^ gswz(qp)) + p) * 16) + 8 * (jl & 1);
            const v4s g0 = __builtin_amdgcn_ds_read_tr16_b64_v4i16((__attribute__((address_space(3))) v4s*)gb);
            const v4s g1 = __builtin_amdgcn_ds_read_tr16_b64_v4i16((__attribute__((address_space(3))) v4s*)(gb + 16 * GROW));
            const uint2 glo = __builtin_bit_cast(uint2, g0), ghi = __builtin_bit_cast(uint2, g1);
            g[u] = make_uint4(glo.x, glo.y, ghi.x, ghi.y);
        }
        WS_STAMP(1)
        if (!WG_DBG(a, 2)) {
            lds_pipeline<AI, 3>(
                [&](int t) {
                    const int i = ig * AI + t;
                    const char* p0 = xb + ((((4 * (i >> 1)) ^ (qp << 2))) * 16) + 8 * (i & 1);
                    const v4s r0 = __builtin_amdgcn_ds_read_tr16_b64_v4i16((__attribute__((address_space(3))) v4s*)p0);
                    const v4s r1 = __builtin_amdgcn_ds_read_tr16_b64_v4i16((__attribute__((address_space(3))) v4s*)(p0 + 16 * 512));
                    const uint2 lo = __builtin_bit_cast(uint2, r0), hi = __builtin_bit_cast(uint2, r1);
                    return make_uint4(lo.x, lo.y, hi.x, hi.y);
                },
                [&](int t, const uint4& av) {
#pragma unroll
                    for (int u = 0; u < BJ; ++u) acc[t][u] = mfma16(av, g[u], acc[t][u]);
                });
        }
        if (do_bias) {
#pragma unroll
            for (int u = 0; u < BJ; ++u) accb[u] = mfma16(ones, g[u], accb[u]);
        }
        WS_STAMP(2)
        __syncthreads();
        WS_STAMP(3)
    }
    if (WG_DBG(a, 16)) return;
    float* slab = a.slabW + (size_t)bz * a.IT * 16 * a.JT * 16;
#pragma unroll
    for (int u = 0; u < BJ; ++u) {
        const int jt = jt0 + jg * BJ + u;
        if (jt < a.JT) {
#pragma unroll
            for (int t = 0; t < AI; ++t) {
                const int it = ig * AI + t;
                if (it < a.IT) {
#pragma unroll
                    for (int ii = 0; ii < 4; ++ii)
                        slab[(size_t)(it * 16 + 4 * q + ii) * (a.JT * 16) + jt * 16 + l16] = acc[t][u][ii];
                }
            }
            if (ig == 0 && q == 0) a.slabB[(size_t)bz * a.JT * 16 + jt * 16 + l16] = accb[u][0];
        }
    }
    WS_STAMP(4)
    WS_STAMP_OUT()
}

template <bool SC, int BJ, int NLW>
__global__ __launch_bounds__((8 + NLW) * 64, NLW == 8 ? 4 : 3) void wgradws_kernel(WgradPArgs a) {
    int bx = blockIdx.x, bz = blockIdx.z;
    wgradws_block(bx, bz, gridDim.x, gridDim.z);
    const int sid = bz * (int)gridDim.x + bx;
    if constexpr (BJ == 4) {
        if (bx == (int)gridDim.x - 1 && a.JT - bx * 16 <= 4 && (SC || gridDim.x > 1)) { wgradws_body<SC, 1, NLW>(a, bx * 16, bz, sid); return; }
    }
    wgradws_body<SC, BJ, NLW>(a, bx * 4 * BJ, bz, sid);
}
__global__ __launch_bounds__(768, 3) void wgradws_group_kernel(WgradPGroup g) {
    int l = 0;
    while (l + 1 < g.n && (int)blockIdx.z >= g.zbeg[l + 1]) ++l;
    if ((int)blockIdx.x >= g.gx[l]) return;
    int bx = blockIdx.x, bz = blockIdx.z - g.zbeg[l];
    wgradws_block(bx, bz, g.gx[l], g.zbeg[l + 1] - g.zbeg[l]);
    wgradws_body<false, 4, 4>(g.a[l], bx * 16, bz, 0);
}

__global__ __launch_bounds__(512, 2) void wgradp_group_kernel(WgradPGroup g) {
    int l = 0;
    while (l + 1 < g.n && (int)blockIdx.z >= g.zbeg[l + 1]) ++l;
    if ((int)blockIdx.x >= g.gx[l] || (int)blockIdx.y >= g.gy[l]) return;
    wgradp_body<8, 4, 4, 4, false>(g.a[l], blockIdx.x, blockIdx.y, blockIdx.z - g.zbeg[l]);
}
__global__ __launch_bounds__(512, 2) void wgradp_group_sc_kernel(WgradPGroup g) {
    int l = 0;
    while (l + 1 < g.n && (int)blockIdx.z >= g.zbeg[l + 1]) ++l;
    if ((int)blockIdx.x >= g.gx[l] || (int)blockIdx.y >= g.gy[l]) return;
    if (l == 0) wgradp_body<8, 4, 4, 4, true>(g.a[0], blockIdx.x, blockIdx.y, blockIdx.z);
    else wgradp_body<8, 4, 4, 4, false>(g.a[l], blockIdx.x, blockIdx.y, blockIdx.z - g.zbeg[l]);
}

void launch_wgradws_group(const WgradPGroup& g, hipStream_t st) {
    int mx = 0;
    for (int l = 0; l < g.n; ++l) mx = std::max(mx, g.gx[l]);
    hipLaunchKernelGGL(wgradws_group_kernel, dim3(mx, 1, g.zbeg[g.n]), dim3(768), WG_NST * (WG_SR * 512 + WG_SR * 512), st, g);
}
void launch_wgradp_group(const WgradPGroup& g, hipStream_t st) {
    int mx = 0, my = 0;
    for (int l = 0; l < g.n; ++l) { mx = std::max(mx, g.gx[l]); my = std::max(my, g.gy[l]); }
    if (g.a[0].rowscale) hipLaunchKernelGGL(wgradp_group_sc_kernel, dim3(mx, my, g.zbeg[g.n]), dim3(512), WG_NST * (WG_SR * 512 + WG_SR * 256 + 1024), st, g);
    else hipLaunchKernelGGL(wgradp_group_kernel, dim3(mx, my, g.zbeg[g.n]), dim3(512), WG_NST * (WG_SR * 512 + WG_SR * 256), st, g);
}
int wgradp_strip(int shape) { return (shape == 8 || shape == 9) ? 8 : 16; }
void launch_wgradp(const WgradPArgs& a, int nsplit, int shape, hipStream_t st, hipEvent_t done) {
    dim3 grid((a.JT + wgradp_strip(shape) - 1) / wgradp_strip(shape), (a.IT + 15) / 16, nsplit);
    const size_t sc = a.rowscale ? 1024 : 0;
    if (shape == 7) {
        const size_t lds = WG_NST * (WG_SR * 512 + WG_SR * 512);
        if (a.rowscale) LAUNCH_EV(done, (wgradws_kernel<true, 4, 4>), grid, dim3(768), lds, st, a);
        else LAUNCH_EV(done, (wgradws_kernel<false, 4, 4>), grid, dim3(768), lds, st, a);
    } else if (shape == 9) {
        const size_t lds = WG_NST * (WG_SR * 512 + WG_SR * 256);
        if (a.rowscale) LAUNCH_EV(done, (wgradws_kernel<true, 2, 8>), grid, dim3(1024), lds, st, a);
        else LAUNCH_EV(done, (wgradws_kernel<false, 2, 8>), grid, dim3(1024), lds, st, a);
    } else if (shape == 16) {
        const size_t lds = WG_NST * (WG_SR * 512 + WG_SR * 512 + sc);
        if (a.rowscale) LAUNCH_EV(done, (wgradp_kernel<16, 2, 8, 2, true>), grid, dim3(1024), lds, st, a);
        else LAUNCH_EV(done, (wgradp_kernel<16, 4, 4, 4, false>), grid, dim3(1024), lds, st, a);
    } else {
        const size_t lds = WG_NST * (WG_SR * 512 + WG_SR * 256 + sc);
        if (a.rowscale) LAUNCH_EV(done, (wgradp_kernel<8, 4, 4, 4, true>), grid, dim3(512), lds, st, a);
        else LAUNCH_EV(done, (wgradp_kernel<8, 4, 4, 4, false>), grid, dim3(512), lds, st, a);
    }
}

}
```

Measured before the change: 5.257 million images/s.

## Add narrow wgrad shape, split bias MFMA, and vectorize fused Adam reduce

Adds a narrower weight-gradient kernel variant (AI=4, half-width X tile) chosen when the input tile count is small, so less LDS is used and less work is wasted on empty rows. The bias accumulation MFMA work is split across the two wave groups to balance load. Gradient reduction with fused Adam now uses float4 loads and stores and writes packed bf16 weight images. An optional epilogue that transposes through DPP for vectorized slab stores is added but off by default. Together these widen the template space and the number of code paths.

```diff
diff --git a/iwae_amd/csrc/device_helpers.h b/iwae_amd/csrc/device_helpers.h
--- a/iwae_amd/csrc/device_helpers.h
+++ b/iwae_amd/csrc/device_helpers.h
@@ -79,6 +79,21 @@
 template <int N, int P, class RD, class USE>
 __device__ __forceinline__ void lds_pipeline(RD rd, USE use) {
     lds_pipeline<N, P>(rd, use, [](int) {});
+}
+
+__device__ __forceinline__ void quad_transpose(float (&x)[4], int lane) {
+    const int p = lane & 3;
+    float t[4];
+#pragma unroll
+    for (int r = 0; r < 4; ++r) {
+        const float o = __builtin_bit_cast(float, __builtin_amdgcn_mov_dpp(__builtin_bit_cast(int, x[r ^ 1]), 0xB1, 0xF, 0xF, true));
+        t[r] = ((r ^ p) & 1) ? o : x[r];
+    }
+#pragma unroll
+    for (int r = 0; r < 4; ++r) {
+        const float o = __builtin_bit_cast(float, __builtin_amdgcn_mov_dpp(__builtin_bit_cast(int, t[r ^ 2]), 0x4E, 0xF, 0xF, true));
+        x[r] = ((r ^ p) & 2) ? o : t[r];
+    }
 }
 
 __device__ __forceinline__ void philox4x32_10(uint32_t c0, uint32_t c1, uint32_t c2, uint32_t c3, uint32_t k0, uint32_t k1, uint32_t out[4]) {
diff --git a/iwae_amd/csrc/fp32_kernels.hip b/iwae_amd/csrc/fp32_kernels.hip
--- a/iwae_amd/csrc/fp32_kernels.hip
+++ b/iwae_amd/csrc/fp32_kernels.hip
@@ -324,20 +324,6 @@
         v[t] = x;
     }
     return make_float4(v[0], v[1], v[2], v[3]);
-}
-__device__ __forceinline__ void quad_transpose(float (&x)[4], int lane) {
-    const int p = lane & 3;
-    float t[4];
-#pragma unroll
-    for (int r = 0; r < 4; ++r) {
-        const float o = __builtin_bit_cast(float, __builtin_amdgcn_mov_dpp(__builtin_bit_cast(int, x[r ^ 1]), 0xB1, 0xF, 0xF, true));
-        t[r] = ((r ^ p) & 1) ? o : x[r];
-    }
-#pragma unroll
-    for (int r = 0; r < 4; ++r) {
-        const float o = __builtin_bit_cast(float, __builtin_amdgcn_mov_dpp(__builtin_bit_cast(int, t[r ^ 2]), 0x4E, 0xF, 0xF, true));
-        x[r] = ((r ^ p) & 2) ? o : t[r];
-    }
 }
 template <int TM, int TN, int WGM, int WGN, bool AK, bool BNF, int OCC = 4>
 __global__ __launch_bounds__(64 * WGM * WGN, OCC) void gemm_f32_v2_kernel(GemmF32Args a) {
diff --git a/iwae_amd/csrc/kernels.h b/iwae_amd/csrc/kernels.h
--- a/iwae_amd/csrc/kernels.h
+++ b/iwae_amd/csrc/kernels.h
@@ -258,7 +258,10 @@
     const float* rowscale;
     int dbg;
     unsigned long long* stamps;
-};
+    int opt;
+};
+enum { WGO_EPI16 = 1,
+       WGO_BIAS_SPLIT = 2 };
 void launch_wgradp(const WgradPArgs& a, int nsplit, int shape, hipStream_t st, hipEvent_t done = nullptr);
 int wgradp_strip(int shape);
 struct WgradPGroup {
diff --git a/iwae_amd/csrc/kernels.hip b/iwae_amd/csrc/kernels.hip
--- a/iwae_amd/csrc/kernels.hip
+++ b/iwae_amd/csrc/kernels.hip
@@ -2765,6 +2765,7 @@
 
 struct MeansArgs { const float* per_b; int B; float beta; float* out; };
 
+template <bool VEC>
 __global__ __launch_bounds__(256) void reduce_grads_kernel(const LayerDesc* layers, int nlayers, float* grad, float* param, float* mom,
                                                            float* vel, AdamCoef c, MeansArgs mn, int first_block, int n1, int first_block2) {
     if (mn.per_b && blockIdx.x == gridDim.x - 1) {
@@ -2815,6 +2816,63 @@
         float r[4] = {red[0][t].x + red[1][t].x + red[2][t].x + red[3][t].x, red[0][t].y + red[1][t].y + red[2][t].y + red[3][t].y,
                       red[0][t].z + red[1][t].z + red[2][t].z + red[3][t].z, red[0][t].w + red[1][t].w + red[2][t].w + red[3][t].w};
         float* dst = (i == L.Kin) ? (grad + L.offb + j) : (grad + L.offW + (size_t)i * L.Nout + j);
+        if (VEC && c.on) {
+            const bool is_b = i == L.Kin;
+            const size_t idx0 = (size_t)(dst - grad);
+            float* pw = param + idx0; float* pm = mom + idx0; float* pv = vel + idx0;
+            const int ne = min(4, L.Nout - j);
+            const bool wide = ne == 4 && ((((uintptr_t)dst | (uintptr_t)pw | (uintptr_t)pm | (uintptr_t)pv) & 15) == 0);
+            float w[4] = {0.f, 0.f, 0.f, 0.f}, mo[4] = {0.f, 0.f, 0.f, 0.f}, ve[4] = {0.f, 0.f, 0.f, 0.f};
+            if (wide) {
+                const float4 w4 = *(const float4*)pw, m4 = *(const float4*)pm, v4 = *(const float4*)pv;
+                w[0] = w4.x; w[1] = w4.y; w[2] = w4.z; w[3] = w4.w;
+                mo[0] = m4.x; mo[1] = m4.y; mo[2] = m4.z; mo[3] = m4.w;
+                ve[0] = v4.x; ve[1] = v4.y; ve[2] = v4.z; ve[3] = v4.w;
+            } else {
+#pragma unroll
+                for (int e = 0; e < 4; ++e)
+                    if (e < ne) { w[e] = pw[e]; mo[e] = pm[e]; ve[e] = pv[e]; }
+            }
+#pragma unroll
+            for (int e = 0; e < 4; ++e)
+                if (e < ne) adam_math(w[e], mo[e], ve[e], r[e], c);
+            if (wide) {
+                *(float4*)dst = make_float4(r[0], r[1], r[2], r[3]);
+                *(float4*)pm = make_float4(mo[0], mo[1], mo[2], mo[3]);
+                *(float4*)pv = make_float4(ve[0], ve[1], ve[2], ve[3]);
+                *(float4*)pw = make_float4(w[0], w[1], w[2], w[3]);
+            } else {
+#pragma unroll
+                for (int e = 0; e < 4; ++e)
+                    if (e < ne) { dst[e] = r[e]; pm[e] = mo[e]; pv[e] = ve[e]; pw[e] = w[e]; }
+            }
+            const int jj = L.joff + j;
+            const bool quad = ne == 4 && (jj & 3) == 0;
+            if (is_b) {
+                if (quad) *(float4*)(L.imgF + img_mg_bias_byte(jj, L.KT_F)) = make_float4(w[0], w[1], w[2], w[3]);
+                else {
+#pragma unroll
+                    for (int e = 0; e < 4; ++e)
+                        if (e < ne) *(float*)(L.imgF + img_mg_bias_byte(jj + e, L.KT_F)) = w[e];
+                }
+            } else {
+                const uint32_t h01 = pack2(w[0], w[1]), h23 = pack2(w[2], w[3]);
+                const uint16_t h[4] = {(uint16_t)(h01 & 0xffffu), (uint16_t)(h01 >> 16), (uint16_t)(h23 & 0xffffu), (uint16_t)(h23 >> 16)};
+#pragma unroll
+                for (int e = 0; e < 4; ++e)
+                    if (e < ne) *(uint16_t*)(L.imgF + img_mg_byte(jj + e, i, L.KT_F)) = h[e];
+                if (L.imgB) {
+                    if (quad) {
+                        *(uint2*)(L.imgB + (L.imgB_kmajor ? img_k_byte(i, jj, L.MT_B) : img_mg_byte(i, jj, L.KT_B))) = make_uint2(h01, h23);
+                    } else {
+#pragma unroll
+                        for (int e = 0; e < 4; ++e)
+                            if (e < ne) *(uint16_t*)(L.imgB + (L.imgB_kmajor ? img_k_byte(i, jj + e, L.MT_B) : img_mg_byte(i, jj + e, L.KT_B))) = h[e];
+                    }
+                }
+            }
+            return;
+        }
 #pragma unroll
         for (int e = 0; e < 4; ++e) {
             if (j + e < L.Nout) {
@@ -3219,10 +3277,11 @@
 void launch_reduce_grads(const LayerDesc* layers, int nlayers, int first_block, int nblocks, float* grad, float* param, float* mom, float* vel,
                          float alpha, float beta1, float beta2, float eps, int fuse_adam, const float* per_b, int B, float beta, float* scalars, hipStream_t st,
                          int first_block2, int nblocks2, hipEvent_t done) {
-    const AdamCoef c = {alpha, 1.0f, beta1, beta2, eps, fuse_adam};
+    const AdamCoef c = {alpha, 1.0f, beta1, beta2, eps, fuse_adam & 1};
     const MeansArgs mn = {per_b, B, beta, scalars};
-    LAUNCH_EV(done, reduce_grads_kernel, dim3(nblocks + nblocks2 + (per_b ? 1 : 0)), dim3(256), 0, st, layers, nlayers, grad, param, mom, vel, c, mn, first_block, nblocks,
-              first_block2);
+    const dim3 grid(nblocks + nblocks2 + (per_b ? 1 : 0));
+    if (fuse_adam & 2) LAUNCH_EV(done, reduce_grads_kernel<true>, grid, dim3(256), 0, st, layers, nlayers, grad, param, mom, vel, c, mn, first_block, nblocks, first_block2);
+    else LAUNCH_EV(done, reduce_grads_kernel<false>, grid, dim3(256), 0, st, layers, nlayers, grad, param, mom, vel, c, mn, first_block, nblocks, first_block2);
 }
 void launch_scalars(const float* per_b, int B, float beta, float* out, hipStream_t st) {
     hipLaunchKernelGGL(scalars_kernel, dim3(1), dim3(256), 0, st, per_b, B, beta, out);
diff --git a/iwae_amd/csrc/model.h b/iwae_amd/csrc/model.h
--- a/iwae_amd/csrc/model.h
+++ b/iwae_amd/csrc/model.h
@@ -100,6 +100,10 @@
     int wg_target8_few = 32;
     int wg_shape9 = 0;
     bool allow_wg7 = true;
+    bool wg_narrow = true;
+    bool wg_epi16 = false;
+    bool wg_bias_split = true;
+    bool reduce_vec = true;
     bool dp_concurrent = false;
     iwae::GemmF32Opts gemm_f32;
     bool allow_f32_multi_reduce = true;
diff --git a/iwae_amd/csrc/model.hip b/iwae_amd/csrc/model.hip
--- a/iwae_amd/csrc/model.hip
+++ b/iwae_amd/csrc/model.hip
@@ -228,7 +228,7 @@
 
 void reduce_blocks(iwae_model* m, hipStream_t st, BlockRange a, BlockRange b, float alpha, bool update, hipEvent_t done, bool with_means) {
     const float* per_b = with_means ? ptr<float>(m->per_b) : nullptr;
-    launch_reduce_grads(m->d_descs, (int)m->descs.size(), a.first, a.count, m->grad, m->param, m->mom, m->vel, alpha, m->adam_b1, m->adam_b2, m->adam_eps, update ? 1 : 0,
+    launch_reduce_grads(m->d_descs, (int)m->descs.size(), a.first, a.count, m->grad, m->param, m->mom, m->vel, alpha, m->adam_b1, m->adam_b2, m->adam_eps, (update ? 1 : 0) | (m->opt.reduce_vec ? 2 : 0),
                         per_b, per_b ? m->B : 0, !per_b ? 0.f : m->cfg.n_layers == 2 ? 1.f : m->beta, per_b ? m->d_scalars : nullptr, st, b.first, b.count, done);
 }
 }
@@ -285,6 +285,7 @@
     const int chunks = (rows + 63) / 64;
     nw = (L.JT > 8 && chunks >= 128) ? 16 : 8;
     if (nw == 16 && L.IT <= 14 && m->opt.allow_wg7) nw = (m->opt.wg_shape9 & (L.JT > 16 ? 1 : 2)) ? 9 : 7;
+    if (nw == 7 && L.IT <= 8 && m->opt.wg_narrow) nw = 4;
     const int blocks = ((L.JT + wgradp_strip(nw) - 1) / wgradp_strip(nw)) * ((L.IT + 15) / 16);
     const int target16 = m->opt.wg_target16 > 0 ? m->opt.wg_target16 : (m->cfg.n_layers == 2 ? 64 : 96);
     const int target = (nw != 8) ? (blocks == 1 ? m->opt.wg_target16_1 : target16) : (chunks < 128 ? m->opt.wg_target8_few : m->opt.wg_target8);
@@ -304,6 +305,7 @@
     a.slabW = ptr<float>(L.slabW); a.slabB = ptr<float>(L.slabB); a.zero = m->d_zero; a.rowscale = nullptr;
     a.dbg = m->wg_debug;
     a.stamps = nullptr;
+    a.opt = (m->opt.wg_epi16 ? WGO_EPI16 : 0) | (m->opt.wg_bias_split ? WGO_BIAS_SPLIT : 0);
     return IWAE_OK;
 }
 
@@ -345,6 +347,7 @@
     memset(&a1, 0, sizeof(a1));
     a1.X = XP; a1.ldX = L.Kp32; a1.IT = L.IT; a1.G = GP; a1.ldG = L.Np32; a1.JT = L.JT; a1.M = R1; a1.rows_per_split = cps1 * 64;
     a1.slabW = ptr<float>(L.slabW); a1.slabB = ptr<float>(L.slabB); a1.zero = m->d_zero; a1.rowscale = rowscale;
+    a1.opt = (m->opt.wg_epi16 ? WGO_EPI16 : 0) | (m->opt.wg_bias_split ? WGO_BIAS_SPLIT : 0);
     a2 = a1;
     a2.X = XP + (size_t)R1 * L.Kp32; a2.G = GP + (size_t)R1 * L.Np32; a2.M = rows - R1; a2.rows_per_split = cps2 * 64;
     a2.slabW = a1.slabW + (size_t)n1 * stride; a2.slabB = a1.slabB + (size_t)n1 * L.JT * 16; a2.rowscale = rowscale + R1;
@@ -590,7 +593,7 @@
     p.group3 = few_side2 && fused_dx && nw[0] == 8 && nw[1] == 8 && nw[2] == 8;
     p.wout_two_part = !p.dec_rows && !p.group3 && o.wout_split > 0 && p.s_mode && !p.g2w && p.early_wout && o.use_side2 && fused_dx && M >= 8192 && L.IT <= 14 && o.allow_wg7 && !(m->abl_skip & 1);
     p.hid_on = p.dec_rows ? ON_MAIN : (p.group3 || (p.early_wout && o.use_side2)) ? ON_SIDE2 : ON_SIDE;
-    p.hid_group = nw[1] == 7 && nw[0] == 7 && o.allow_wg_group && (p.early_wout || fused_dx);
+    p.hid_group = (nw[1] == 7 || nw[1] == 4) && (nw[0] == 7 || nw[0] == 4) && o.allow_wg_group && (p.early_wout || fused_dx);
     p.tail = p.dec_rows ? ON_SIDE : p.hid_on;
     p.draw_on = p.dec_rows ? ON_MAIN : few_side2 ? ON_SIDE2 : ON_SIDE;
     BlockBwdArgs bb;
@@ -1765,6 +1768,10 @@
     else if (n == "dec_rows") m->opt.dec_rows_max = iv;
     else if (n == "no_wg7") m->opt.allow_wg7 = !on;
     else if (n == "wg9") m->opt.wg_shape9 = iv;
+    else if (n == "wg_narrow") m->opt.wg_narrow = on;
+    else if (n == "wg_epi16") m->opt.wg_epi16 = on;
+    else if (n == "wg_bias_split") m->opt.wg_bias_split = on;
+    else if (n == "reduce_vec") m->opt.reduce_vec = on;
     else if (n == "grid_chunk") m->opt.grid_chunk = iv > 0 ? std::max(16, iv) : 0;
     else if (n == "ais_t_chunk") m->opt.ais_t_chunk = iv > 0 ? iv : 0;
     else if (n == "local_t_chunk") m->opt.local_t_chunk = iv > 0 ? iv : 0;
diff --git a/iwae_amd/csrc/wgrad_kernels.hip b/iwae_amd/csrc/wgrad_kernels.hip
--- a/iwae_amd/csrc/wgrad_kernels.hip
+++ b/iwae_amd/csrc/wgrad_kernels.hip
@@ -219,15 +219,18 @@
         bx = V % gx; bz = V / gx;
     }
 }
-template <bool SC, int BJ, int NLW>
+template <bool SC, int BJ, int NLW, int AI, int OPT>
 __device__ __forceinline__ void wgradws_body(const WgradPArgs& a, const int jt0, const int bz, const int sid) {
     extern __shared__ __attribute__((aligned(1024))) char smem[];
 #ifdef IWAE_DENSE_STAMPS
     unsigned long long ws_sum[8] = {0, 0, 0, 0, 0, 0, 0, 0}, ws_prev = 0;
     asm volatile("s_memtime %0\n\ts_waitcnt lgkmcnt(0)" : "=s"(ws_prev)::"memory");
 #endif
-    constexpr int AI = 7, IGC = 2, NCW = 8, STRIP = 4 * BJ;
-    constexpr int XT_BYTES = WG_SR * 512, GROW = STRIP * 32, GT_BYTES = WG_SR * GROW, BUF = XT_BYTES + GT_BYTES;
+    constexpr int IGC = 2, NCW = 8, STRIP = 4 * BJ;
+    constexpr int XROW = AI <= 4 ? 256 : 512;
+    constexpr int XSPR = XROW / 16, XRPP = 1024 / XROW;
+    static_assert(2 * AI * 32 <= XROW, "X tile row");
+    constexpr int XT_BYTES = WG_SR * XROW, GROW = STRIP * 32, GT_BYTES = WG_SR * GROW, BUF = XT_BYTES + GT_BYTES;
     constexpr int XP = XT_BYTES / 1024, GP = GT_BYTES / 1024, XPL = XP / NLW, GPL = GP / NLW, PPL = XPL + GPL;
     constexpr int SPR = GROW / 16, RPP = 1024 / GROW;
     static_assert(XP % NLW == 0 && GP % NLW == 0 && GPL >= 1 && GPL <= 4, "loader split");
@@ -248,8 +251,8 @@
         const char* xbase[XPL]; int xlim[XPL];
 #pragma unroll
         for (int i = 0; i < XPL; ++i) {
-            const int pc = lw * XPL + i, rl = 2 * pc + (lane >> 5);
-            const int col = ((lane & 31) ^ ((rl & 3) << 2)) * 8;
+            const int pc = lw * XPL + i, rl = XRPP * pc + lane / XSPR;
+            const int col = ((lane % XSPR) ^ ((rl & 3) << 2)) * 8;
             xbase[i] = (const char*)a.X + ((size_t)(rbeg + rl) * a.ldX + col) * 2;
             xlim[i] = col < a.ldX ? rend - rbeg - rl : -(1 << 30);
         }
@@ -356,8 +359,8 @@
             int rl, col, ld;
             if (isx) {
                 const int pc = lw * XPL + i;
-                rl = 2 * pc + (lane >> 5);
-                col = ((lane & 31) ^ ((rl & 3) << 2)) * 8;
+                rl = XRPP * pc + lane / XSPR;
+                col = ((lane % XSPR) ^ ((rl & 3) << 2)) * 8;
                 ld = a.ldX;
             } else {
                 const int pc = lw * GPL + (i - XPL);
@@ -401,9 +404,12 @@
 #pragma unroll
         for (int t = 0; t < AI; ++t) acc[t][u] = (f32x4){0.0f, 0.0f, 0.0f, 0.0f};
     }
-    const int xrow_off = (4 * q + qp) * 512, grow_off = (4 * q + qp) * GROW;
+    const int xrow_off = (4 * q + qp) * XROW, grow_off = (4 * q + qp) * GROW;
     const uint4 ones = make_uint4(0x3F803F80u, 0x3F803F80u, 0x3F803F80u, 0x3F803F80u);
-    const bool do_bias = ig == 0 && !WG_DBG(a, 4);
+    constexpr int HB = BJ >= 2 ? BJ / 2 : BJ;
+    constexpr bool SPLIT = BJ >= 2 && (OPT & WGO_BIAS_SPLIT);
+    const bool hi_own = SPLIT ? ig == 1 : ig == 0;
+    const bool do_bias = ig == 0 && !WG_DBG(a, 4), bias_hi = hi_own && !WG_DBG(a, 4);
     __syncthreads();
     WS_STAMP(0)
     for (int c = 0; c < nstage; ++c) {
@@ -427,7 +433,7 @@
                     const int i = ig * AI + t;
                     const char* p0 = xb + ((((4 * (i >> 1)) ^ (qp << 2))) * 16) + 8 * (i & 1);
                     const v4s r0 = __builtin_amdgcn_ds_read_tr16_b64_v4i16((__attribute__((address_space(3))) v4s*)p0);
-                    const v4s r1 = __builtin_amdgcn_ds_read_tr16_b64_v4i16((__attribute__((address_space(3))) v4s*)(p0 + 16 * 512));
+                    const v4s r1 = __builtin_amdgcn_ds_read_tr16_b64_v4i16((__attribute__((address_space(3))) v4s*)(p0 + 16 * XROW));
                     const uint2 lo = __builtin_bit_cast(uint2, r0), hi = __builtin_bit_cast(uint2, r1);
                     return make_uint4(lo.x, lo.y, hi.x, hi.y);
                 },
@@ -438,7 +444,13 @@
         }
         if (do_bias) {
 #pragma unroll
-            for (int u = 0; u < BJ; ++u) accb[u] = mfma16(ones, g[u], accb[u]);
+            for (int u = 0; u < (SPLIT ? HB : BJ); ++u) accb[u] = mfma16(ones, g[u], accb[u]);
+        }
+        if constexpr (SPLIT) {
+            if (bias_hi) {
+#pragma unroll
+                for (int u = HB; u < BJ; ++u) accb[u] = mfma16(ones, g[u], accb[u]);
+            }
         }
         WS_STAMP(2)
         __syncthreads();
@@ -454,27 +466,33 @@
             for (int t = 0; t < AI; ++t) {
                 const int it = ig * AI + t;
                 if (it < a.IT) {
-#pragma unroll
-                    for (int ii = 0; ii < 4; ++ii)
-                        slab[(size_t)(it * 16 + 4 * q + ii) * (a.JT * 16) + jt * 16 + l16] = acc[t][u][ii];
+                    if constexpr ((OPT & WGO_EPI16) != 0) {
+                        float x[4] = {acc[t][u][0], acc[t][u][1], acc[t][u][2], acc[t][u][3]};
+                        quad_transpose(x, lane);
+                        *(float4*)(slab + (size_t)(it * 16 + 4 * q + p) * (a.JT * 16) + jt * 16 + 4 * qp) = make_float4(x[0], x[1], x[2], x[3]);
+                    } else {
+#pragma unroll
+                        for (int ii = 0; ii < 4; ++ii)
+                            slab[(size_t)(it * 16 + 4 * q + ii) * (a.JT * 16) + jt * 16 + l16] = acc[t][u][ii];
+                    }
                 }
             }
-            if (ig == 0 && q == 0) a.slabB[(size_t)bz * a.JT * 16 + jt * 16 + l16] = accb[u][0];
+            if ((u < HB ? ig == 0 : hi_own) && q == 0) a.slabB[(size_t)bz * a.JT * 16 + jt * 16 + l16] = accb[u][0];
         }
     }
     WS_STAMP(4)
     WS_STAMP_OUT()
 }
 
-template <bool SC, int BJ, int NLW>
+template <bool SC, int BJ, int NLW, int AI, int OPT>
 __global__ __launch_bounds__((8 + NLW) * 64, NLW == 8 ? 4 : 3) void wgradws_kernel(WgradPArgs a) {
     int bx = blockIdx.x, bz = blockIdx.z;
     wgradws_block(bx, bz, gridDim.x, gridDim.z);
     const int sid = bz * (int)gridDim.x + bx;
     if constexpr (BJ == 4) {
-        if (bx == (int)gridDim.x - 1 && a.JT - bx * 16 <= 4 && (SC || gridDim.x > 1)) { wgradws_body<SC, 1, NLW>(a, bx * 16, bz, sid); return; }
-    }
-    wgradws_body<SC, BJ, NLW>(a, bx * 4 * BJ, bz, sid);
+        if (bx == (int)gridDim.x - 1 && a.JT - bx * 16 <= 4 && (SC || gridDim.x > 1)) { wgradws_body<SC, 1, NLW, AI, OPT>(a, bx * 16, bz, sid); return; }
+    }
+    wgradws_body<SC, BJ, NLW, AI, OPT>(a, bx * 4 * BJ, bz, sid);
 }
 __global__ __launch_bounds__(768, 3) void wgradws_group_kernel(WgradPGroup g) {
     int l = 0;
@@ -482,7 +500,7 @@
     if ((int)blockIdx.x >= g.gx[l]) return;
     int bx = blockIdx.x, bz = blockIdx.z - g.zbeg[l];
     wgradws_block(bx, bz, g.gx[l], g.zbeg[l + 1] - g.zbeg[l]);
-    wgradws_body<false, 4, 4>(g.a[l], bx * 16, bz, 0);
+    wgradws_body<false, 4, 4, 7, 0>(g.a[l], bx * 16, bz, 0);
 }
 
 __global__ __launch_bounds__(512, 2) void wgradp_group_kernel(WgradPGroup g) {
@@ -511,17 +529,28 @@
     else hipLaunchKernelGGL(wgradp_group_kernel, dim3(mx, my, g.zbeg[g.n]), dim3(512), WG_NST * (WG_SR * 512 + WG_SR * 256), st, g);
 }
 int wgradp_strip(int shape) { return (shape == 8 || shape == 9) ? 8 : 16; }
+template <int BJ, int NLW, int AI>
+static void launch_wgradws(const WgradPArgs& a, dim3 grid, size_t lds, hipStream_t st, hipEvent_t done) {
+    const dim3 block((8 + NLW) * 64);
+#define WS_CASE(O)                                                                                            \
+    case O:                                                                                                   \
+        if (a.rowscale) LAUNCH_EV(done, (wgradws_kernel<true, BJ, NLW, AI, O>), grid, block, lds, st, a);     \
+        else LAUNCH_EV(done, (wgradws_kernel<false, BJ, NLW, AI, O>), grid, block, lds, st, a);               \
+        break;
+    switch (a.opt & (WGO_EPI16 | WGO_BIAS_SPLIT)) {
+        WS_CASE(0) WS_CASE(1) WS_CASE(2) WS_CASE(3)
+    }
+#undef WS_CASE
+}
 void launch_wgradp(const WgradPArgs& a, int nsplit, int shape, hipStream_t st, hipEvent_t done) {
     dim3 grid((a.JT + wgradp_strip(shape) - 1) / wgradp_strip(shape), (a.IT + 15) / 16, nsplit);
     const size_t sc = a.rowscale ? 1024 : 0;
     if (shape == 7) {
-        const size_t lds = WG_NST * (WG_SR * 512 + WG_SR * 512);
-        if (a.rowscale) LAUNCH_EV(done, (wgradws_kernel<true, 4, 4>), grid, dim3(768), lds, st, a);
-        else LAUNCH_EV(done, (wgradws_kernel<false, 4, 4>), grid, dim3(768), lds, st, a);
+        launch_wgradws<4, 4, 7>(a, grid, WG_NST * (WG_SR * 512 + WG_SR * 512), st, done);
+    } else if (shape == 4) {
+        launch_wgradws<4, 4, 4>(a, grid, WG_NST * (WG_SR * 256 + WG_SR * 512), st, done);
     } else if (shape == 9) {
-        const size_t lds = WG_NST * (WG_SR * 512 + WG_SR * 256);
-        if (a.rowscale) LAUNCH_EV(done, (wgradws_kernel<true, 2, 8>), grid, dim3(1024), lds, st, a);
-        else LAUNCH_EV(done, (wgradws_kernel<false, 2, 8>), grid, dim3(1024), lds, st, a);
+        launch_wgradws<2, 8, 7>(a, grid, WG_NST * (WG_SR * 512 + WG_SR * 256), st, done);
     } else if (shape == 16) {
         const size_t lds = WG_NST * (WG_SR * 512 + WG_SR * 512 + sc);
         if (a.rowscale) LAUNCH_EV(done, (wgradp_kernel<16, 2, 8, 2, true>), grid, dim3(1024), lds, st, a);
```

Result: no change. 5.277 million images/s (median of 2 runs) (+0.4%).
